# rtqichen/torchdiffeq

Measured on NVIDIA H100. Metric: trajectories/sec (dopri5, batch=65536 dim=128), higher is better.
Workload: dtype f32

## Files before the change

include/tdq.h:

```cpp
#ifndef TDQ_H_
#define TDQ_H_

#include <stddef.h>
#include <stdint.h>

#ifdef __cplusplus
extern "C" {
#endif

#define TDQ_ABI_VERSION 2

#define TDQ_MAX_STAGES 16
#define TDQ_MAX_K      (TDQ_MAX_STAGES + 1)
#define TDQ_MAX_SEGS   64
#define TDQ_MAX_RANKS  16

typedef enum {
    TDQ_OK = 0,
    TDQ_ERR_INVALID = 1,
    TDQ_ERR_CUDA = 2,
    TDQ_ERR_UNSUPPORTED = 3
} tdq_status;

typedef enum { TDQ_F32 = 0, TDQ_F64 = 1 } tdq_dtype;

typedef enum {
    TDQ_RUN_OK = 0,
    TDQ_RUN_DT_UNDERFLOW = 1,
    TDQ_RUN_NONFINITE = 2,
    TDQ_RUN_MAX_STEPS = 3,
    TDQ_RUN_EXCHANGE_TIMEOUT = 4
} tdq_run_status;

typedef struct {
    int32_t n_stages;
    int32_t order;
    int32_t fsal;
    int32_t reserved;
    double alpha[TDQ_MAX_STAGES];
    double beta[TDQ_MAX_STAGES][TDQ_MAX_K];
    double c_sol[TDQ_MAX_K];
    double c_err[TDQ_MAX_K];
    double c_mid[TDQ_MAX_K];
} tdq_tableau;

typedef struct {
    int32_t dtype;
    int32_t ratio_f64;
    double rtol, atol;
    double min_step, max_step;
    double safety, ifactor, dfactor;
    double t_sign;
    int64_t max_num_steps;
    int64_t n_global;
    void *ybuf[2];
    void *kbuf[2];
    int32_t always_fit;
    int32_t reserved;
    uint64_t loop_handle;
} tdq_options;

typedef struct {
    volatile uint64_t seq;
    volatile int32_t status;
    volatile int32_t accept;
    volatile int32_t done;
    volatile int32_t out_cursor;
    volatile int64_t n_accept, n_reject;
    volatile double t0, t1, dt;
    volatile double ratio;
    volatile double att_t0, att_dt;
    volatile double next_t0, next_dt;
    volatile int32_t on_jump_t;
    volatile int32_t par;
} tdq_mailbox;

int tdq_abi_version(void);
size_t tdq_sizeof(int32_t which);
const char *tdq_last_error(void);
int tdq_device_sm_count(int *out);

int tdq_tableau_get(const char *name, tdq_tableau *out);

int tdq_mailbox_create(tdq_mailbox **host_ptr, void **dev_ptr);
int tdq_mailbox_destroy(tdq_mailbox *host_ptr);

size_t tdq_ctrl_size(void);
size_t tdq_ctrl_tstage_offset(void);
size_t tdq_ctrl_taux_offset(void);

int tdq_ctrl_init(void *ctrl_dev, const tdq_tableau *tab, const tdq_options *opt, const double *t_out_dev,
                  double t_start, int32_t n_out, void *mailbox_dev, void *stream);

int tdq_ctrl_set_step_t(void *ctrl_dev, const double *step_t_dev, int32_t n, void *stream);
int tdq_ctrl_set_jump_t(void *ctrl_dev, const double *jump_t_dev, int32_t n, void *stream);

int64_t tdq_norm_table_fill(const int64_t *seg_offsets, const int64_t *seg_lens, int32_t n_seg, int64_t n,
                            int32_t dtype, int64_t *table_host, int64_t capacity_words);
size_t tdq_norm_partials_len(size_t n, int64_t n_chunks);

int tdq_scaled_sumsq(void *ctrl_dev, int32_t dtype, const void *x, const void *x2, const void *y0,
                     const double *rtol_vec, const double *atol_vec, const int64_t *table_dev, int64_t n_chunks,
                     int32_t table_aligned, int32_t n_seg, size_t n, double *partials, double *out, void *stream);
int tdq_initial_step_h0(void *ctrl_dev, int32_t dtype, const double *d0_sumsq, const double *d1_sumsq,
                        const int64_t *seg_counts_dev, int32_t n_seg, void *stream);
int tdq_initial_step_probe(void *ctrl_dev, int32_t dtype, void *y_probe, const void *y0, const void *f0,
                           size_t n, void *stream);
int tdq_initial_step_finish(void *ctrl_dev, int32_t dtype, const double *d2_sumsq,
                            const int64_t *seg_counts_dev, int32_t n_seg, void *stream);
int tdq_set_first_step(void *ctrl_dev, double first_step, void *stream);

int tdq_prepare_attempt(void *ctrl_dev, int32_t dtype, const double *y0_nonfinite_count_dev, void *stream);

int tdq_stage_combine(void *ctrl_dev, const tdq_tableau *tab, int32_t dtype, int32_t row, void *y_out,
                      const void *y0, const void *const *k, size_t n, void *stream);

int tdq_stage_combine_final(void *ctrl_dev, const tdq_tableau *tab, int32_t dtype, void *y1_out, void *err_out,
                            const void *y0, const void *const *k, size_t n, void *stream);

int tdq_error_norm_commit(void *ctrl_dev, int32_t dtype, const void *err_pre, const void *k_last, const void *y0,
                          const void *y1, const double *rtol_vec, const double *atol_vec, const int64_t *table_dev,
                          int64_t n_chunks, int32_t table_aligned, int32_t n_seg, size_t n, double *partials,
                          double *out, void *err_over_tol_out, void *stream);
int tdq_commit_candidates(void *ctrl_dev, int32_t dtype, const void *y1, const void *k_last, size_t n, void *stream);

int tdq_controller(void *ctrl_dev, int32_t dtype, const double *norm_in, const int64_t *seg_counts_dev,
                   int32_t n_seg, const void *ratio_dev, void *stream);

int tdq_interp_fit_eval(void *ctrl_dev, const tdq_tableau *tab, int32_t dtype, const void *y1, const void *const *k,
                        void *const *coeff, void *solution, size_t n, void *stream);
int tdq_interp_eval_at(void *ctrl_dev, int32_t dtype, const void *const *coeff, const double *t_dev, void *out,
                       size_t n, void *stream);
int tdq_poly_eval(int32_t dtype, const void *const *coeff, double x, void *out, size_t n, void *stream);
int tdq_ctrl_reset_interval(void *ctrl_dev, void *stream);

int tdq_loop_create(void *body_graph, void **loop_out, uint64_t *handle_out);
int tdq_loop_launch(void *loop, void *stream);
int tdq_loop_destroy(void *loop);
int tdq_ctrl_set_loop(void *ctrl_dev, uint64_t loop_handle, void *stream);

int tdq_rk4_stage(int32_t dtype, int32_t which, void *y_out, const void *y0, const void *k1,
                  const void *k2, const void *k3, const void *k4, const void *dt_dev,
                  const int64_t *step_dev, size_t n, void *stream);
int tdq_fixed_emit(int32_t dtype, void *y0, const void *y1, void *solution,
                   const int32_t *rec_begin_dev, const int32_t *out_idx_dev, const int32_t *mode_dev,
                   const void *slope_dev, int64_t *step_dev, const void *tstage_all_dev,
                   void *tstage_cur_dev, int64_t n_steps, size_t n, void *stream);

int tdq_fixed_final_emit(int32_t dtype, int32_t which, void *y0, const void *k1, const void *k2, const void *k3,
                         const void *k4, const void *dt_dev, void *solution, const int32_t *rec_begin_dev,
                         const int32_t *out_idx_dev, const int32_t *mode_dev, const void *slope_dev, int64_t *step_dev,
                         const void *tstage_all_dev, void *tstage_cur_dev, int64_t n_steps, size_t n, void *stream);

int tdq_lincomb(int32_t dtype, void *out, const void *base, const void *const *x, const double *coefs, int32_t n_terms,
                size_t n, void *stream);

int tdq_linear_supported(int32_t dtype, int32_t width);
size_t tdq_linear_weights_bytes(int32_t width);
int tdq_linear_prepare(int32_t dtype, const void *weight, int32_t width, void *planes, void *stream);
int tdq_linear_apply(int32_t dtype, const void *y, const void *planes, int32_t width, size_t n_rows, void *k_out,
                     void *stream);
int tdq_linear_stage(void *ctrl_dev, const tdq_tableau *tab, int32_t dtype, int32_t row, void *k_out, void *y1_out,
                     void *err_out, const void *y0, const void *const *k, const void *planes, int32_t width, size_t n,
                     void *stream);

int tdq_linear_attempt_supported(const tdq_tableau *tab, int32_t dtype, int32_t width);
int tdq_linear_attempt(void *ctrl_dev, const tdq_tableau *tab, int32_t dtype, void *const *k_out, void *y1_out, void *err_out,
                       const void *y0, const void *k0, const void *planes, int32_t width, size_t n, double *partials,
                       double *norm_out, const int64_t *seg_counts_dev, int32_t store_always, void *stream);

int tdq_fixed_emit_cubic(int32_t dtype, const void *y0, const void *y1, const void *f0, const void *f1, void *solution,
                         const int32_t *out_idx_dev, const void *coef_dev, int32_t rec_lo, int32_t rec_hi, size_t n,
                         void *stream);

#define TDQ_IMPL_MAX_STAGES 4
#define TDQ_IMPL_MAX_CHUNKS 64
typedef enum {
    TDQ_IMPL_CONTINUE = 0, TDQ_IMPL_CONVERGED = 1, TDQ_IMPL_SINGULAR = 2, TDQ_IMPL_EXHAUSTED = 3
} tdq_impl_status;
size_t tdq_implicit_partials_len(int32_t max_vectors);
size_t tdq_implicit_state_len(int32_t max_iters);
int tdq_implicit_residual(int32_t dtype, const void *x, const void *const *f, int32_t n_stages, size_t n,
                          const void *const *u_chunks, const void *const *s_chunks, int32_t n_chunks, int64_t per_chunk,
                          int32_t slot, int32_t n_dots, double *partials, double *out, void *stream);
int tdq_implicit_solve(int32_t dtype, const double *res_out, const double *upd_out, double *state, int32_t *status,
                       int32_t m, int32_t max_iters, double tol, void *stream);
int tdq_implicit_update(int32_t dtype, void *x, int32_t n_stages, size_t n, const void *const *u_chunks,
                        const void *const *s_chunks, int32_t n_chunks, int64_t per_chunk, int32_t m, const double *w_dev,
                        const void *f0, void *y_out, const void *y0, const void *const *k, const double *coefs,
                        int32_t n_terms, double *partials, double *out, void *stream);

typedef struct { unsigned char bytes[64]; } tdq_ipc_handle;
int tdq_xchg_create(void **dev_ptr, tdq_ipc_handle *handle_out);
int tdq_xchg_open(const tdq_ipc_handle *handle, void **peer_ptr);
int tdq_xchg_close(void *peer_ptr);
int tdq_xchg_destroy(void *dev_ptr);
int tdq_ctrl_set_exchange(void *ctrl_dev, const void *const *peer_ptrs, int32_t rank, int32_t world,
                          uint64_t epoch, void *stream);

typedef enum {
    TDQ_ROWS_T0 = 0, TDQ_ROWS_T1, TDQ_ROWS_DT, TDQ_ROWS_RATIO,
    TDQ_ROWS_ATT_T0, TDQ_ROWS_ATT_DT, TDQ_ROWS_ATT_T1, TDQ_ROWS_FIT_DT,
    TDQ_ROWS_H0, TDQ_ROWS_D1,
    TDQ_ROWS_PAR, TDQ_ROWS_ACCEPT, TDQ_ROWS_FIT, TDQ_ROWS_DONE,
    TDQ_ROWS_STATUS, TDQ_ROWS_CURSOR, TDQ_ROWS_EMIT_LO, TDQ_ROWS_EMIT_HI,
    TDQ_ROWS_N_STEPS, TDQ_ROWS_N_ACCEPT, TDQ_ROWS_N_REJECT,
    TDQ_ROWS_T_FIRST, TDQ_ROWS_T_PROBE, TDQ_ROWS_T_STAGE,
    TDQ_ROWS_N_FIELDS = TDQ_ROWS_T_STAGE + TDQ_MAX_STAGES,
    TDQ_ROWS_HEADER = 255
} tdq_rows_field;
size_t tdq_rows_size(size_t n_rows);
size_t tdq_rows_offset(int32_t field, size_t n_rows);
size_t tdq_rows_partials_len(size_t n_rows, size_t row_len);
int tdq_rows_init(void *ctrl_dev, void *rows_dev, int32_t dtype, size_t n_rows, double t_start, void *stream);
int tdq_rows_init_grid(void *ctrl_dev, void *rows_dev, int32_t dtype, size_t n_rows, const double *t_grid, int32_t n_out,
                       void *stream);
int tdq_rows_sumsq(void *ctrl_dev, void *rows_dev, int32_t dtype, const void *x, const void *x2, const double *rtol_vec,
                   const double *atol_vec, size_t n_rows, size_t row_len, double *partials, double *out, void *stream);
int tdq_rows_initial_h0(void *ctrl_dev, void *rows_dev, int32_t dtype, const double *d0_sumsq, const double *d1_sumsq,
                        size_t n_rows, size_t row_len, void *stream);
int tdq_rows_initial_probe(void *ctrl_dev, void *rows_dev, int32_t dtype, void *y_probe, size_t n_rows, size_t row_len,
                           void *stream);
int tdq_rows_initial_finish(void *ctrl_dev, void *rows_dev, int32_t dtype, const double *d2_sumsq, size_t n_rows,
                            size_t row_len, void *stream);
int tdq_rows_set_first_step(void *rows_dev, size_t n_rows, double first_step, void *stream);
int tdq_rows_prepare(void *ctrl_dev, void *rows_dev, int32_t dtype, const double *y0_nonfinite_dev, size_t n_rows,
                     void *stream);
int tdq_rows_combine(void *ctrl_dev, void *rows_dev, const tdq_tableau *tab, int32_t dtype, int32_t row, void *y_out,
                     const void *const *k, size_t n_rows, size_t row_len, void *stream);
int tdq_rows_combine_final(void *ctrl_dev, void *rows_dev, const tdq_tableau *tab, int32_t dtype, void *y1_out,
                           void *err_out, const void *const *k, size_t n_rows, size_t row_len, void *stream);
int tdq_rows_error_norm_commit(void *ctrl_dev, void *rows_dev, int32_t dtype, const void *err_pre, const void *k_last,
                               const void *y1, const double *rtol_vec, const double *atol_vec, size_t n_rows,
                               size_t row_len, double *partials, double *out, void *stream);
int tdq_rows_controller(void *ctrl_dev, void *rows_dev, int32_t dtype, const double *norm_in, size_t n_rows,
                        size_t row_len, void *stream);
int tdq_rows_fit_eval(void *ctrl_dev, void *rows_dev, const tdq_tableau *tab, int32_t dtype, const void *y1,
                      const void *const *k, void *solution, size_t n_rows, size_t row_len, void *stream);
int tdq_rows_controller_grid(void *ctrl_dev, void *rows_dev, int32_t dtype, const double *norm_in, size_t n_rows,
                             size_t row_len, void *stream);
int tdq_rows_fit_eval_grid(void *ctrl_dev, void *rows_dev, const tdq_tableau *tab, int32_t dtype, const void *y1,
                           const void *const *k, void *solution, size_t n_rows, size_t row_len, void *stream);

int tdq_rows_event_init(void *rows_dev, const double *ev_val, double *init_sign, double *sign0, int32_t *flag,
                        size_t n_rows, int32_t K, void *stream);
int tdq_rows_controller_event(void *ctrl_dev, void *rows_dev, int32_t dtype, const double *norm_in, const double *ev_val,
                              const double *init_sign, const double *sign0, int32_t *flag, size_t n_rows, size_t row_len,
                              int32_t K, void *stream);
int tdq_rows_controller_event_grid(void *ctrl_dev, void *rows_dev, int32_t dtype, const double *norm_in,
                                   const double *ev_val, const double *init_sign, const double *sign0, int32_t *flag,
                                   size_t n_rows, size_t row_len, int32_t K, void *stream);
int tdq_rows_fit_store(void *ctrl_dev, void *rows_dev, const tdq_tableau *tab, int32_t dtype, const void *y1,
                       const void *const *k, const int32_t *flag, void *coeff, size_t n_rows, size_t row_len,
                       void *stream);
int tdq_rows_event_bisect(void *ctrl_dev, void *rows_dev, int32_t dtype, int32_t iter, const double *ev_val,
                          const double *init_sign, const double *sign0, const int32_t *nitrs, double *lo, double *hi,
                          const void *coeff, const void *y_start, void *y_mid, double *t_ev, double *event_t,
                          void *y_event, size_t n_rows, size_t row_len, int32_t K, void *stream);

int tdq_pack_segments(int32_t dtype, void *dst, const void *const *src, const int64_t *offsets,
                      const int64_t *lens, const double *scales, int32_t n_src, void *stream);

#ifdef __cplusplus
}
#endif
#endif
```

torchdiffeq_b200/_engine.py:

```python
import ctypes as C
import math
import time

import torch

from . import _lib

_DTYPES = {torch.float32: _lib.TDQ_F32, torch.float64: _lib.TDQ_F64}


def _stream():
    return torch.cuda.current_stream().cuda_stream


_SOLVER_STREAMS = {}


def solver_stream(device):
    idx = device.index if device.index is not None else torch.cuda.current_device()
    st = _SOLVER_STREAMS.get(idx)
    if st is None:
        st = _SOLVER_STREAMS[idx] = torch.cuda.Stream(device=idx)
    return st


class on_solver_stream:

    def __init__(self, device):
        self.device = device

    def __enter__(self):
        self.cur = torch.cuda.current_stream(self.device)
        self.s = solver_stream(self.device)
        if self.cur == self.s:
            self.ctx = None
            return self
        self.s.wait_stream(self.cur)
        self.ctx = torch.cuda.stream(self.s)
        self.ctx.__enter__()
        return self

    def __exit__(self, *exc):
        if self.ctx is not None:
            self.ctx.__exit__(*exc)
            self.cur.wait_stream(self.s)
        return False

    def publish(self, *tensors):
        if self.ctx is not None:
            for t in tensors:
                if isinstance(t, torch.Tensor) and t.is_cuda:
                    t.record_stream(self.cur)


class _RetryWithCopies(Exception):
    """func handed back a buffer it had already returned for an earlier stage of the same attempt."""


class SolverFailure(AssertionError):
    """Raised for the reference's in-loop assertions (rk_common.py:247, :286, :287)."""


class Layout:

    def __init__(self, shapes, dtype):
        self.shapes = [torch.Size(s) for s in shapes]
        self.dtype = dtype
        vec = 16 // torch.empty((), dtype=dtype).element_size()
        self.offsets, self.lens = [], []
        off = 0
        for s in self.shapes:
            n = s.numel()
            self.offsets.append(off)
            self.lens.append(n)
            off += (n + vec - 1) // vec * vec
        self.n = off
        self.n_real = sum(self.lens)

    def flatten(self, tensors, out=None):
        flat = out if out is not None else torch.zeros(self.n, dtype=self.dtype, device=tensors[0].device)
        for t, o, l in zip(tensors, self.offsets, self.lens):
            flat[o:o + l].copy_(t.reshape(-1))
        return flat

    def views(self, flat, lead=()):
        return tuple(flat[..., o:o + l].view((*lead, *s)) for o, l, s in zip(self.offsets, self.lens, self.shapes))


def pack_pieces(lib, dt_code, dtype, buf, f, pieces):
    offs, lens, scales = pieces
    srcs, keep = [], []
    for p_, l in zip(f, lens):
        if p_ is None:
            srcs.append(None)
            continue
        if p_.dtype != dtype:
            p_ = p_.to(dtype)
        p_ = p_.reshape(-1)
        if not p_.is_contiguous():
            p_ = p_.contiguous()
        if p_.numel() != l:
            raise ValueError("func returned a piece of %d elements, expected %d" % (p_.numel(), l))
        keep.append(p_)
        srcs.append(p_.data_ptr())
    n_launch = 0
    for lo in range(0, len(srcs), _lib.TDQ_MAX_SEGS):
        hi = min(lo + _lib.TDQ_MAX_SEGS, len(srcs))
        _lib.check(lib.tdq_pack_segments(
            dt_code, buf.data_ptr(), _lib.ptr_array(srcs[lo:hi]), _lib.i64_array(offs[lo:hi]),
            _lib.i64_array(lens[lo:hi]), _lib.dbl_array(scales[lo:hi]), hi - lo, _stream()))
        n_launch += 1
    return n_launch


def find_event(interp_fn, sign0, t0, t1, event_fn, tol):
    nitrs = torch.ceil(torch.log((t1 - t0) / tol) / math.log(2.0))
    for _ in range(int(nitrs.long())):
        t_mid = (t1 + t0) / 2.0
        if bool(sign0 == torch.sign(event_fn(t_mid, interp_fn(t_mid)))):
            t0 = t_mid
        else:
            t1 = t_mid
    event_t = (t0 + t1) / 2.0
    return event_t, interp_fn(event_t)


class AdaptiveEngine:

    def __init__(self, fn, n, dtype, device, method, *, rtol, atol, segs=None, t_sign=1.0,
                 pieces=None, min_step=0.0, max_step=float("inf"), first_step=None, step_t=None, jump_t=None,
                 safety=0.9, ifactor=10.0, dfactor=0.2, max_num_steps=2 ** 31 - 1,
                 rtol_vec=None, atol_vec=None, norm_fn=None, q_view=None,
                 graph="auto", run_ahead=2, reduce_fn=None, n_global=None, seg_counts_global=None,
                 agree_fn=None, exchange=None, callbacks=None, keep_interp=False, device_loop="auto", post_fn=None):
        if device.type != "cuda":
            raise _lib.TdqError("torchdiffeq_b200 runs on CUDA devices only (got %s); there is no CPU path" % device)
        if dtype not in _DTYPES:
            raise _lib.TdqError("unsupported state dtype %s (float32 and float64 are implemented)" % dtype)
        self.lib = _lib.load()
        self.fn = fn
        self.n = int(n)
        self.dtype = dtype
        self.device = device
        self.dt_code = _DTYPES[dtype]
        self.tab = _lib.tableau(method)
        self.S = self.tab.n_stages
        self.fsal = bool(self.tab.fsal)
        self.pieces = pieces
        self.first_step = first_step
        self.norm_fn = norm_fn
        self.q_view = q_view
        self.reduce_fn = reduce_fn
        self.agree_fn = agree_fn
        self.exchange = exchange
        self.post_fn = post_fn
        if exchange is not None and post_fn is None:
            self.agree_fn = None
        self.callbacks = callbacks or {}
        self.graph_opt = graph
        self.run_ahead = int(run_ahead)
        self.device_loop = device_loop
        self.keep_interp = bool(keep_interp)
        self.jump_t = jump_t
        if self.callbacks or (jump_t is not None and jump_t.numel() > 0):
            self.graph_opt = False
            self.run_ahead = 0

        segs = segs if segs is not None else [(0, self.n)]
        self.n_seg = len(segs)
        n_real = sum(int(l) for _, l in segs)
        counts = seg_counts_global if seg_counts_global is not None else [int(l) for _, l in segs]
        self.seg_counts = torch.tensor(counts, dtype=torch.int64, device=device)
        if len(segs) == 1 and int(segs[0][0]) == 0 and int(segs[0][1]) == self.n:
            self.norm_table, self.n_chunks, self.table_aligned = None, 0, 0
        else:
            words = _lib.norm_table(segs, self.n, _DTYPES[dtype])
            self.norm_table = torch.tensor(words, dtype=torch.int64, device=device)
            self.n_chunks, self.table_aligned = int(words[1]), int(words[3])

        if (rtol_vec is None) != (atol_vec is None):
            if rtol_vec is None:
                rtol_vec = torch.full_like(atol_vec, rtol)
            else:
                atol_vec = torch.full_like(rtol_vec, atol)
        self.rtol_vec = rtol_vec
        self.atol_vec = atol_vec
        vtol = rtol_vec is not None
        self.ratio_f64 = vtol or dtype == torch.float64
        self.opt = _lib.Options(
            dtype=self.dt_code, ratio_f64=1 if vtol else 0,
            rtol=float(rtol) if not vtol else 0.0, atol=float(atol) if not vtol else 0.0,
            min_step=float(min_step), max_step=float(max_step), safety=float(safety),
            ifactor=float(ifactor), dfactor=float(dfactor), t_sign=float(t_sign),
            max_num_steps=int(max_num_steps), n_global=int(n_global if n_global is not None else n_real))
        self.step_t = step_t

        kw = dict(dtype=dtype, device=device)
        self.ctrl = torch.zeros(self.lib.tdq_ctrl_size(), dtype=torch.uint8, device=device)
        o = self.lib.tdq_ctrl_tstage_offset()
        self.tstage = self.ctrl[o:o + 8 * _lib.TDQ_MAX_K].view(dtype)
        o = self.lib.tdq_ctrl_taux_offset()
        self.taux = self.ctrl[o:o + 32].view(dtype)
        self.ybuf = [torch.zeros(self.n, **kw) for _ in range(2)]
        self.kbuf = [torch.zeros(self.n, **kw) for _ in range(2)]
        self.opt.ybuf[0], self.opt.ybuf[1] = self.ybuf[0].data_ptr(), self.ybuf[1].data_ptr()
        self.opt.kbuf[0], self.opt.kbuf[1] = self.kbuf[0].data_ptr(), self.kbuf[1].data_ptr()
        self.opt.always_fit = 1 if self.keep_interp else 0
        self.ytmp = torch.zeros(self.n, **kw)
        self.y1 = torch.zeros(self.n, **kw)
        self.errp = torch.zeros(self.n, **kw)
        if self.keep_interp:
            self.coeff = [torch.zeros(self.n, **kw) for _ in range(5)]
            self.coeff_ptrs = _lib.ptr_array([c.data_ptr() for c in self.coeff])
        else:
            self.coeff, self.coeff_ptrs = [], None
        self.partials = torch.zeros(self.lib.tdq_norm_partials_len(self.n, self.n_chunks), dtype=torch.float64,
                                    device=device)
        self.norm_out = torch.zeros(self.n_seg + 1, dtype=torch.float64, device=device)
        self.dsum = [torch.zeros(self.n_seg + 1, dtype=torch.float64, device=device) for _ in range(3)]
        self.kslots = {}
        self.qbuf = None
        self.ratio_buf = None
        if norm_fn is not None:
            self.qbuf = torch.zeros(self.n, dtype=torch.float64 if vtol else dtype, device=device)
            self.ratio_buf = torch.zeros((), dtype=torch.float64 if self.ratio_f64 else dtype, device=device)
        self._own_ptrs = None
        self.mbox_host = C.POINTER(_lib.Mailbox)()
        mdev = C.c_void_p()
        _lib.check(self.lib.tdq_mailbox_create(C.byref(self.mbox_host), C.byref(mdev)))
        self.mbox_dev = mdev.value
        self.solution = None
        self._graph = None
        self._graph_failed = False
        self._graph_keep = None
        self._loop = None
        self._loop_handle = 0
        self._loop_failed = False
        self._always_copy = False
        self.linear = None
        self.capture_in_solve = True
        self.n_attempts = 0
        self.nfe = 0
        self.nfe_total = 0
        self.launches = 0
        self._graph_launches = 0

    def __del__(self):
        try:
            if self.mbox_host:
                torch.cuda.synchronize(self.device)
                self._drop_graph()
                self.lib.tdq_mailbox_destroy(self.mbox_host)
                self.mbox_host = None
        except Exception:
            pass

    def _call_fn(self, t, y, slot, taken=(), dst=None):
        self.nfe += 1
        f = self.fn(t, y)
        if isinstance(f, torch.Tensor):
            if f.dtype != self.dtype:
                f = f.to(self.dtype)
            f = f.reshape(-1)
            if f.numel() != self.n:
                raise ValueError("func returned %d elements for a state of %d" % (f.numel(), self.n))
            if f.data_ptr() in taken and not self._always_copy:
                self._always_copy = True
                raise _RetryWithCopies()
            if (self._always_copy or not f.is_contiguous() or (f.data_ptr() % 16) != 0 or self._aliases(f)
                    or f.data_ptr() in taken):
                buf = self._slot(slot)
                buf.copy_(f)
                f = buf
            return f
        buf = dst if dst is not None else self._slot(slot)
        self.launches += pack_pieces(self.lib, self.dt_code, self.dtype, buf, f, self.pieces)
        if self.post_fn is not None:
            self.post_fn(buf)
        return buf

    def set_linear(self, weight, whole_attempt=True):
        width, S = int(weight.shape[0]), self.S
        if self.pieces is not None or self.post_fn is not None or self.n % width:
            return False
        beta, c_err = self.tab.beta, self.tab.c_err
        for i in range(S):
            used = {j for j in range(i + 1) if beta[i][j] != 0.0}
            if self.fsal and i == S - 1:
                used |= {j for j in range(S) if c_err[j] != 0.0}
            if not 1 <= len(used) <= 8:
                return False
        planes = torch.empty(int(self.lib.tdq_linear_weights_bytes(width)), dtype=torch.uint8, device=self.device)
        whole = bool(whole_attempt) and bool(self.lib.tdq_linear_attempt_supported(C.byref(self.tab), self.dt_code, width))
        fold = (whole and self.norm_table is None and self.n_seg == 1 and self.rtol_vec is None and self.norm_fn is None)
        self.linear = dict(weight=weight, width=width, planes=planes, whole=whole, fold=fold,
                           k=[torch.zeros(self.n, dtype=self.dtype, device=self.device) for _ in range(S)])
        self._drop_graph()
        return True

    def _eval(self, t, y, slot, dst=None):
        if self.linear is None:
            return self._call_fn(t, y, slot, dst=dst)
        self.nfe += 1
        out = dst if dst is not None else self._slot(slot)
        L = self.linear
        self._launch(self.lib.tdq_linear_apply(self.dt_code, y.data_ptr(), L["planes"].data_ptr(), L["width"],
                                               self.n // L["width"], out.data_ptr(), _stream()))
        return out

    @property
    def y0w(self):
        return self.ybuf[self.mbox_host.contents.par & 1]

    @property
    def k0(self):
        return self.kbuf[self.mbox_host.contents.par & 1]

    def _drop_graph(self):
        if self._loop is not None:
            try:
                self.lib.tdq_loop_destroy(self._loop)
            except Exception:
                pass
        self._loop, self._loop_handle = None, 0
        self._graph, self._graph_keep = None, None

    def _launch(self, rc):
        _lib.check(rc)
        self.launches += 1

    def _slot(self, i):
        if i not in self.kslots:
            self.kslots[i] = torch.zeros(self.n, dtype=self.dtype, device=self.device)
        return self.kslots[i]

    def _aliases(self, f):
        if self._own_ptrs is None:
            own = self.ybuf + self.kbuf + [self.ytmp, self.y1, self.errp, self.solution] + self.coeff
            self._own_ptrs = {t.untyped_storage().data_ptr() for t in own}
        return f.untyped_storage().data_ptr() in self._own_ptrs

    def _reduce(self, buf):
        if self.reduce_fn is not None:
            self.reduce_fn(buf)

    def _sumsq(self, x, x2, out):
        self._launch(self.lib.tdq_scaled_sumsq(
            self.ctrl.data_ptr(), self.dt_code, x.data_ptr(), x2.data_ptr() if x2 is not None else None,
            None,
            self.rtol_vec.data_ptr() if self.rtol_vec is not None else None,
            self.atol_vec.data_ptr() if self.atol_vec is not None else None,
            self.norm_table.data_ptr() if self.norm_table is not None else None, self.n_chunks, self.table_aligned,
            self.n_seg, self.n, self.partials.data_ptr(), out.data_ptr(), _stream()))
        self._reduce(out)

    def _attempt_front(self):
        try:
            return self._attempt_front_once()
        except _RetryWithCopies:
            return self._attempt_front_once()

    def _attempt_front_once(self):
        lib, ctrl, tab, dc, st = self.lib, self.ctrl.data_ptr(), C.byref(self.tab), self.dt_code, _stream()
        S = self.S
        k = [None] * (S + 1)
        keep = []
        folded = False
        if self.linear is not None and self.linear["whole"]:
            L = self.linear
            for i in range(S):
                k[i + 1] = L["k"][i].data_ptr()
            folded = L["fold"]
            self._launch(lib.tdq_linear_attempt(ctrl, tab, dc, _lib.ptr_array(k), self.y1.data_ptr(), self.errp.data_ptr(),
                                                None, None, L["planes"].data_ptr(), L["width"], self.n,
                                                self.partials.data_ptr() if folded else None,
                                                self.norm_out.data_ptr() if folded else None,
                                                None, 0 if folded else 1, st))
            self.nfe += S
        elif self.linear is not None:
            L = self.linear
            for i in range(S):
                last = i == S - 1 and self.fsal
                out = L["k"][i]
                self._launch(lib.tdq_linear_stage(ctrl, tab, dc, i, out.data_ptr(),
                                                  self.y1.data_ptr() if last else None,
                                                  self.errp.data_ptr() if last else None, None, _lib.ptr_array(k),
                                                  L["planes"].data_ptr(), L["width"], self.n, st))
                self.nfe += 1
                k[i + 1] = out.data_ptr()
        for i in range(S if self.linear is None else 0):
            if i == S - 1 and self.fsal:
                out = self.y1
                self._launch(lib.tdq_stage_combine_final(ctrl, tab, dc, out.data_ptr(), self.errp.data_ptr(), None,
                                                         _lib.ptr_array(k), self.n, st))
            else:
                out = self.ytmp
                self._launch(lib.tdq_stage_combine(ctrl, tab, dc, i, out.data_ptr(), None, _lib.ptr_array(k), self.n,
                                                   st))
            f = self._call_fn(self.tstage[i], out, i + 1, taken=k)
            keep.append(f)
            k[i + 1] = f.data_ptr()
        if not self.fsal:
            self._launch(lib.tdq_stage_combine_final(ctrl, tab, dc, self.y1.data_ptr(), self.errp.data_ptr(), None,
                                                     _lib.ptr_array(k), self.n, st))
        kp = _lib.ptr_array(k)
        if not folded:
            self._launch(lib.tdq_error_norm_commit(
                ctrl, dc, self.errp.data_ptr(), k[S], None, self.y1.data_ptr(),
                self.rtol_vec.data_ptr() if self.rtol_vec is not None else None,
                self.atol_vec.data_ptr() if self.atol_vec is not None else None,
                self.norm_table.data_ptr() if self.norm_table is not None else None, self.n_chunks, self.table_aligned,
                self.n_seg, self.n, self.partials.data_ptr(), self.norm_out.data_ptr(),
                self.qbuf.data_ptr() if self.qbuf is not None else None, st))
        ratio_ptr = None
        if self.norm_fn is not None:
            r = self.norm_fn(self.q_view(self.qbuf))
            r = torch.as_tensor(r, device=self.device)
            self.ratio_buf.copy_(r.to(self.ratio_buf.dtype).reshape(()))
            ratio_ptr = self.ratio_buf.data_ptr()
        elif self.exchange is None:
            self._reduce(self.norm_out)
        self._launch(lib.tdq_controller(ctrl, dc, self.norm_out.data_ptr(), self.seg_counts.data_ptr(), self.n_seg,
                                      ratio_ptr, st))
        return k, kp, keep

    def _attempt_back(self, kp):
        self._launch(self.lib.tdq_interp_fit_eval(self.ctrl.data_ptr(), C.byref(self.tab), self.dt_code,
                                                  self.y1.data_ptr(), kp, self.coeff_ptrs, self.solution.data_ptr(),
                                                  self.n, _stream()))

    def _attempt(self):
        k, kp, keep = self._attempt_front()
        self._attempt_back(kp)
        return keep

    def _wait_seq(self, target):
        mb = self.mbox_host.contents
        spins = 0
        while mb.seq < target:
            spins += 1
            if spins > 2000:
                time.sleep(0)
                if spins % 20000 == 0 and torch.cuda.current_stream().query() and mb.seq < target:
                    raise _lib.TdqError("the device finished the queued attempts without reporting attempt %d (mailbox at %d)"
                                        % (target, mb.seq))
        return mb

    def _raise_if_failed(self, mb):
        if mb.status != _lib.RUN_OK:
            torch.cuda.current_stream().synchronize()
            self._raise_status(mb.status, mb.next_dt, self.y0w)

    def _raise_status(self, s, dt, y, where=""):
        if s == _lib.RUN_DT_UNDERFLOW:
            raise SolverFailure("underflow in dt {}".format(dt) + where)
        if s == _lib.RUN_NONFINITE:
            raise SolverFailure("non-finite values in state `y`: {}".format(y) + where)
        if s == _lib.RUN_EXCHANGE_TIMEOUT:
            raise _lib.TdqError("a peer rank did not deliver its norm partials within 10 s (sharded solve)")
        if s == _lib.RUN_MAX_STEPS:
            m = self.opt.max_num_steps
            raise SolverFailure("max_num_steps exceeded ({}>={})".format(m, m) + where)
        raise SolverFailure("solver failed with status %d" % s + where)

    def _lockstep_mode(self):
        return bool(self.callbacks) or self.run_ahead == 0

    def _use_loop(self):
        return (self._loop is not None and not self._lockstep_mode() and self.agree_fn is None
                and self.norm_fn is None)

    def solve(self, y0_flat, t64, t_start=None):
        try:
            if self._lockstep_mode():
                for _ in self._lockstep(y0_flat, t64, t_start):
                    pass
            else:
                if self._begin(y0_flat, t64, t_start, loop=self._use_loop()) > 1:
                    self._loop_run_ahead()
                self._read_counters()
        except BaseException:
            self.poisoned = True
            try:
                torch.cuda.current_stream().synchronize()
            except Exception:
                pass
            raise
        return self.solution

    def _read_counters(self):
        mb = self.mbox_host.contents
        self.n_accept, self.n_reject = int(mb.n_accept), int(mb.n_reject)
        self.n_attempts = self.n_accept + self.n_reject

    def prime(self, y0_flat, t64, t_start=None):
        if self.graph_opt not in (True, "auto") or self._lockstep_mode():
            return False
        n_out = self._begin(y0_flat, t64, t_start)
        if n_out <= 1:
            return False
        self._warm_attempt()
        self._capture()
        torch.cuda.current_stream().synchronize()
        return self._graph is not None

    def _begin(self, y0_flat, t64, t_start=None, loop=False):
        lib = self.lib
        self.nfe_total += self.nfe
        self.nfe, self.launches = 0, 0
        n_out = int(t64.numel())
        self.t_out = t64.contiguous()
        if getattr(self, "solution", None) is None or self.solution.shape[0] != n_out:
            self.solution = torch.empty(n_out, self.n, dtype=self.dtype, device=self.device)
            self._drop_graph()
            self._own_ptrs = None
            loop = False
        self.solution[0].copy_(y0_flat)
        self.ybuf[0].copy_(y0_flat)
        st = _stream()
        mb = self.mbox_host.contents
        mb.seq, mb.status, mb.done, mb.par, mb.accept = 0, 0, 0, 0, 0
        mb.n_accept, mb.n_reject = 0, 0
        if t_start is None:
            t_start = float(t64[0])
        self.opt.loop_handle = self._loop_handle if loop else 0
        _lib.check(lib.tdq_ctrl_init(self.ctrl.data_ptr(), C.byref(self.tab), C.byref(self.opt),
                                     self.t_out.data_ptr(), float(t_start), n_out, self.mbox_dev, st))
        self._start(float(t_start), n_out)
        return n_out

    def _start(self, t_start, n_out):
        lib = self.lib
        st = _stream()
        if self.exchange is not None:
            self.exchange.arm(self.ctrl.data_ptr(), st)
        if self.jump_t is not None and self.jump_t.numel() > 0:
            self._launch(lib.tdq_ctrl_set_jump_t(self.ctrl.data_ptr(), self.jump_t.data_ptr(),
                                                 int(self.jump_t.numel()), st))
        if self.step_t is not None and self.step_t.numel() > 0:
            self._launch(lib.tdq_ctrl_set_step_t(self.ctrl.data_ptr(), self.step_t.data_ptr(),
                                               int(self.step_t.numel()), st))
        dc, ctrl = self.dt_code, self.ctrl.data_ptr()
        if self.linear is not None:
            L = self.linear
            self._launch(lib.tdq_linear_prepare(dc, L["weight"].data_ptr(), L["width"], L["planes"].data_ptr(), st))

        f0 = self._eval(self.taux[0], self.ybuf[0], 0, dst=self.kbuf[0])
        if f0.data_ptr() != self.kbuf[0].data_ptr():
            self.kbuf[0].copy_(f0)
        del f0
        self._sumsq(self.ybuf[0], None, self.dsum[0])
        if self.first_step is None:
            if self.norm_fn is not None:
                self._initial_step_custom_norm()
            else:
                self._sumsq(self.kbuf[0], None, self.dsum[1])
                self._launch(lib.tdq_initial_step_h0(ctrl, dc, self.dsum[0].data_ptr(), self.dsum[1].data_ptr(),
                                                   self.seg_counts.data_ptr(), self.n_seg, st))
                self._launch(lib.tdq_initial_step_probe(ctrl, dc, self.ytmp.data_ptr(), None, None, self.n, st))
                f1 = self._eval(self.taux[1], self.ytmp, 1)
                self._sumsq(f1, self.kbuf[0], self.dsum[2])
                del f1
                self._launch(lib.tdq_initial_step_finish(ctrl, dc, self.dsum[2].data_ptr(),
                                                       self.seg_counts.data_ptr(), self.n_seg, st))
        else:
            self._launch(lib.tdq_set_first_step(ctrl, float(self.first_step), st))
        bad_ptr = self.dsum[0].data_ptr() + 8 * self.n_seg if n_out > 1 else None
        self._launch(lib.tdq_prepare_attempt(ctrl, dc, bad_ptr, st))

    def _lockstep_attempt(self, issued, mb):
        cb = self.callbacks
        if cb.get("callback_step") is not None:
            cb["callback_step"](*self._with_y(mb.next_t0, mb.next_dt))
        k, kp, keep = self._attempt_front()
        issued += 1
        mb = self._wait_seq(issued)
        self._raise_if_failed(mb)
        if cb:
            name = "callback_accept_step" if mb.accept else "callback_reject_step"
            if cb.get(name) is not None:
                cb[name](*self._with_y(mb.att_t0, mb.att_dt))
        jumped = bool(mb.accept) and bool(mb.on_jump_t)
        self._attempt_back(kp)
        del k, kp, keep
        if jumped:
            k0 = self.k0
            f = self._call_fn(self.taux[2], self.y0w, 0, dst=k0)
            if f.data_ptr() != k0.data_ptr():
                k0.copy_(f)
            del f
        return issued, mb

    def _lockstep(self, y0_flat, t64, t_start=None):
        n_out = self._begin(y0_flat, t64, t_start)
        torch.cuda.current_stream().synchronize()
        mb = self.mbox_host.contents
        self._raise_if_failed(mb)
        issued = 0
        yield mb
        try:
            while n_out > 1:
                issued, mb = self._lockstep_attempt(issued, mb)
                yield mb
                if mb.done:
                    break
        except GeneratorExit:
            pass
        torch.cuda.current_stream().synchronize()
        self._read_counters()

    def solve_dense(self, y0_flat, t64):
        steps = self._lockstep(y0_flat, t64)
        next(steps)
        times, coeffs = [float(t64[0])], []
        for mb in steps:
            if mb.accept:
                times.append(float(mb.t1))
                coeffs.append([c.clone() for c in self.coeff])
        return self.solution, times, coeffs

    def solve_taped(self, y0_flat, t64, t_start=None):
        steps = self._lockstep(y0_flat, t64, t_start)
        next(steps)
        tape, cursor, first, jumped = [], 1, True, None
        for mb in steps:
            if mb.accept:
                prev = (mb.par ^ 1) & 1
                k0 = self.kbuf[prev]
                tape.append(dict(t0=float(mb.att_t0), dt=float(mb.att_dt), y0=self.ybuf[prev].clone(), k0=k0.clone(),
                                 out_lo=cursor, out_hi=int(mb.out_cursor), first=first, jumped_into=jumped))
                cursor, first = int(mb.out_cursor), False
                jumped = True if mb.on_jump_t else None
        return self.solution, tape

    def solve_until_event(self, y0_flat, t0, event_fn, tol):
        t64 = torch.tensor([float(t0), float("inf")], dtype=torch.float64, device=self.device)
        steps = self._lockstep(y0_flat, t64, float(t0))
        mb = next(steps)
        tt = lambda v: torch.tensor(v, dtype=torch.float64, device=self.device)
        t_cur = float(t0)
        if bool(event_fn(tt(t_cur), self.y0w) == 0):
            return t_cur, self.y0w.clone()
        sign0 = torch.sign(event_fn(tt(t_cur), self.y0w))
        while bool(sign0 == torch.sign(event_fn(tt(t_cur), self.y0w))):
            mb = next(steps)
            t_cur = mb.t1
        steps.close()
        y_mid = torch.empty(self.n, dtype=self.dtype, device=self.device)

        def interp(t_eval):
            self._launch(self.lib.tdq_interp_eval_at(self.ctrl.data_ptr(), self.dt_code, self.coeff_ptrs,
                                                     t_eval.to(self.device).data_ptr(), y_mid.data_ptr(), self.n,
                                                     _stream()))
            return y_mid
        bound = lambda v: torch.tensor(float(v), dtype=torch.float64)
        event_t, y_event = find_event(interp, sign0, bound(mb.t0), bound(mb.t1),
                                      lambda t_, y_: event_fn(t_.to(self.device), y_), tol)
        return float(event_t), y_event.clone()

    def _with_y(self, t0, dt):
        t0, dt = self._scalars(t0, dt)
        return t0, self.y0w, dt

    def _scalars(self, t0, dt):
        kw = dict(dtype=torch.float64, device=self.device)
        return torch.tensor(t0, **kw), torch.tensor(dt, **kw)

    def _loop_run_ahead(self):
        D = max(1, self.run_ahead)
        mb = self.mbox_host.contents
        issued = 0
        use_graph = self.graph_opt in (True, "auto") and not self._graph_failed and self.capture_in_solve
        if self._use_loop() and self.opt.loop_handle != 0:
            self._launch_loop()
            return
        if self._graph is None:
            if use_graph:
                self._warm_attempt()
                self._capture()
            else:
                self._attempt()
            issued += 1
            if self._use_loop():
                _lib.check(self.lib.tdq_ctrl_set_loop(self.ctrl.data_ptr(), self._loop_handle, _stream()))
                self._launch_loop(first=1)
                return
        while True:
            seen = mb.seq
            if mb.status != _lib.RUN_OK or mb.done:
                break
            if issued - seen > D:
                time.sleep(0)
                continue
            if self._graph is not None:
                self._graph.replay()
                self.nfe += self.S
                self.launches += self._graph_launches
            else:
                self._attempt()
            issued += 1
        if self.agree_fn is not None:
            target = self.agree_fn(issued)
            while issued < target:
                if self._graph is not None:
                    self._graph.replay()
                    self.nfe += self.S
                    self.launches += self._graph_launches
                else:
                    self._attempt()
                issued += 1
        mb = self._wait_seq(issued)
        self._raise_if_failed(mb)
        torch.cuda.current_stream().synchronize()

    def _launch_loop(self, first=0):
        _lib.check(self.lib.tdq_loop_launch(self._loop, _stream()))
        torch.cuda.current_stream().synchronize()
        mb = self.mbox_host.contents
        ran = int(mb.seq) - first
        self.nfe += self.S * ran
        self.launches += self._graph_launches * ran
        self._raise_if_failed(mb)

    def _warm_attempt(self):
        self._attempt()

    def _capture(self):
        last = None
        for _try in range(2):
            try:
                want_loop = (self.device_loop in (True, "auto") and not self._loop_failed and self.agree_fn is None
                             and self.norm_fn is None)
                g = torch.cuda.CUDAGraph(keep_graph=True) if want_loop else torch.cuda.CUDAGraph()
                nfe, launches = self.nfe, self.launches
                try:
                    with torch.cuda.graph(g, stream=solver_stream(self.device)):
                        keep = self._attempt()
                finally:
                    self._graph_launches = self.launches - launches
                    self.nfe, self.launches = nfe, launches
                self._graph, self._graph_keep = g, keep
                if want_loop:
                    self._make_loop(g)
                return
            except Exception as e:
                last = e
                self._graph = None
                torch.cuda.synchronize(self.device)
        self._graph_failed = True
        if self.graph_opt is True:
            raise last
        import warnings
        warnings.warn("torchdiffeq_b200: CUDA graph capture of the step body failed (%s: %s); "
                      "continuing with eager launches" % (type(last).__name__, last))

    def _make_loop(self, g):
        loop, handle = C.c_void_p(), C.c_uint64()
        try:
            _lib.check(self.lib.tdq_loop_create(C.c_void_p(g.raw_cuda_graph()), C.byref(loop), C.byref(handle)))
            self._loop, self._loop_handle = loop.value, int(handle.value)
        except Exception as e:
            self._loop, self._loop_handle, self._loop_failed = None, 0, True
            if self.device_loop is True:
                raise
            import warnings
            warnings.warn("torchdiffeq_b200: the captured step could not be wrapped into a device-side loop "
                          "(%s: %s); the host replays it instead" % (type(e).__name__, e))

    def _initial_step_custom_norm(self):
        T = self.dtype
        y0, f0 = self.ybuf[0], self.kbuf[0] * self.opt.t_sign
        if self.rtol_vec is not None:
            scale = self.atol_vec + torch.abs(y0) * self.rtol_vec
        else:
            scale = float(self.opt.atol) + torch.abs(y0) * float(self.opt.rtol)
        nf = lambda v: torch.as_tensor(self.norm_fn(self.q_view(v)), device=self.device).abs()
        d0, d1 = nf(y0 / scale), nf(f0 / scale)
        if d0 < 1e-5 or d1 < 1e-5:
            h0 = torch.tensor(1e-6, dtype=T, device=self.device)
        else:
            h0 = 0.01 * d0 / d1
        h0 = h0.abs()
        self.ytmp.copy_(y0 + h0 * f0)
        t0 = float(self.t_out[0])
        self.taux[1] = (torch.tensor(t0, dtype=torch.float64, device=self.device) + h0.double()).to(T) * self.opt.t_sign
        f1 = self._call_fn(self.taux[1], self.ytmp, 1) * self.opt.t_sign
        d2 = torch.abs(nf((f1 - f0) / scale) / h0)
        order = self.tab.order - 1
        if d1 <= 1e-15 and d2 <= 1e-15:
            h1 = torch.max(torch.tensor(1e-6, dtype=T, device=self.device), h0 * 1e-3)
        else:
            h1 = (0.01 / max(d1, d2)) ** (1. / float(order + 1))
        h1 = h1.abs()
        dt = float(torch.min(100 * h0, h1).to(torch.float64))
        self._launch(self.lib.tdq_set_first_step(self.ctrl.data_ptr(), dt, _stream()))


def bisect_iterations(lo, hi, tol):
    v = torch.log((hi - lo) / tol) / math.log(2.0)
    for r in ((v - v.round()).abs() < 1e-6).nonzero().view(-1).tolist():
        v[r] = torch.log((hi[r] - lo[r]) / tol[r]) / math.log(2.0)
    n = torch.ceil(v)
    return torch.where(torch.isfinite(n) & (n > 0), n, torch.zeros_like(n)).to(torch.int32)


class RowsEngine(AdaptiveEngine):

    def __init__(self, fn, shape, dtype, device, method, **kw):
        shape = torch.Size(shape)
        self.B = int(shape[0])
        self.D = int(shape[1:].numel())
        self.row_shape = shape[1:]
        super().__init__(fn, self.B * self.D, dtype, device, method, **kw)
        lib, B = self.lib, self.B
        self.rows = torch.zeros(lib.tdq_rows_size(B), dtype=torch.uint8, device=device)
        es = torch.empty((), dtype=dtype).element_size()
        tshape = (B,) + (1,) * (len(shape) - 1)

        def field(which, dt, size):
            o = lib.tdq_rows_offset(which, B)
            return self.rows[o:o + B * size].view(dt)
        self._field = field
        self.t_first = field(_lib.ROWS_T_FIRST, dtype, es).view(tshape)
        self.t_probe = field(_lib.ROWS_T_PROBE, dtype, es).view(tshape)
        self.t_stage = [field(_lib.ROWS_T_STAGE + i, dtype, es).view(tshape) for i in range(self.S)]
        f64 = dict(dtype=torch.float64, device=device)
        self.row_partials = torch.zeros(lib.tdq_rows_partials_len(B, self.D), **f64)
        self.row_norm = torch.zeros(2 * B, **f64)
        self.row_dsum = [torch.zeros(2 * B, **f64) for _ in range(3)]
        self.row_n_accept = self.row_n_reject = None
        self.ev_fn = None
        self.grid = None
        self._next_grid = None
        self._graph_grid = False

    def solve(self, y0_flat, t64, t_start=None, grid=None):
        if grid is not None:
            if grid.dim() != 2 or grid.shape[0] != self.B or grid.dtype != torch.float64 or grid.device != self.device:
                raise ValueError("grid must be a float64 [%d, T] tensor on %s, got %s %s on %s"
                                 % (self.B, self.device, grid.dtype, tuple(grid.shape), grid.device))
            grid = grid.contiguous()
            t64 = grid[0]
        self._next_grid = grid
        try:
            return super().solve(y0_flat, t64, t_start)
        finally:
            self._next_grid = None

    def _begin(self, y0_flat, t64, t_start=None, loop=False):
        self.grid = self._next_grid
        if (self.grid is not None) != self._graph_grid:
            self._drop_graph()
            self._graph_grid = self.grid is not None
            loop = False
        return super()._begin(y0_flat, t64, t_start, loop)

    def _rows_sumsq(self, x, x2, out):
        self._launch(self.lib.tdq_rows_sumsq(
            self.ctrl.data_ptr(), self.rows.data_ptr(), self.dt_code, x.data_ptr(),
            x2.data_ptr() if x2 is not None else None,
            self.rtol_vec.data_ptr() if self.rtol_vec is not None else None,
            self.atol_vec.data_ptr() if self.atol_vec is not None else None,
            self.B, self.D, self.row_partials.data_ptr(), out.data_ptr(), _stream()))

    def _attempt_front_once(self):
        lib, ctrl, rows, tab, dc, st = (self.lib, self.ctrl.data_ptr(), self.rows.data_ptr(), C.byref(self.tab),
                                        self.dt_code, _stream())
        S, B, D = self.S, self.B, self.D
        k = [None] * (S + 1)
        keep = []
        for i in range(S):
            if i == S - 1 and self.fsal:
                out = self.y1
                self._launch(lib.tdq_rows_combine_final(ctrl, rows, tab, dc, out.data_ptr(), self.errp.data_ptr(),
                                                        _lib.ptr_array(k), B, D, st))
            else:
                out = self.ytmp
                self._launch(lib.tdq_rows_combine(ctrl, rows, tab, dc, i, out.data_ptr(), _lib.ptr_array(k), B, D, st))
            f = self._call_fn(self.t_stage[i], out, i + 1, taken=k)
            keep.append(f)
            k[i + 1] = f.data_ptr()
        if not self.fsal:
            self._launch(lib.tdq_rows_combine_final(ctrl, rows, tab, dc, self.y1.data_ptr(), self.errp.data_ptr(),
                                                    _lib.ptr_array(k), B, D, st))
        kp = _lib.ptr_array(k)
        self._launch(lib.tdq_rows_error_norm_commit(
            ctrl, rows, dc, self.errp.data_ptr(), k[S], self.y1.data_ptr(),
            self.rtol_vec.data_ptr() if self.rtol_vec is not None else None,
            self.atol_vec.data_ptr() if self.atol_vec is not None else None,
            B, D, self.row_partials.data_ptr(), self.row_norm.data_ptr(), st))
        grid = self.grid is not None
        if self.ev_fn is None:
            controller = lib.tdq_rows_controller_grid if grid else lib.tdq_rows_controller
            self._launch(controller(ctrl, rows, dc, self.row_norm.data_ptr(), B, D, st))
        else:
            torch.mul(self.row_field(_lib.ROWS_ATT_T1, torch.float64), self.opt.t_sign, out=self.ev_t)
            self._ev_call(self.y1)
            controller = lib.tdq_rows_controller_event_grid if grid else lib.tdq_rows_controller_event
            self._launch(controller(ctrl, rows, dc, self.row_norm.data_ptr(), self.ev_val.data_ptr(),
                                    self.ev_init.data_ptr(), self.ev_sign0.data_ptr(), self.ev_flag.data_ptr(), B, D,
                                    self.K, st))
        return k, kp, keep

    def _attempt_back(self, kp):
        if self.ev_fn is not None:
            self._launch(self.lib.tdq_rows_fit_store(self.ctrl.data_ptr(), self.rows.data_ptr(), C.byref(self.tab),
                                                     self.dt_code, self.y1.data_ptr(), kp, self.ev_flag.data_ptr(),
                                                     self.ev_coeff.data_ptr(), self.B, self.D, _stream()))
            return
        fit_eval = self.lib.tdq_rows_fit_eval_grid if self.grid is not None else self.lib.tdq_rows_fit_eval
        self._launch(fit_eval(self.ctrl.data_ptr(), self.rows.data_ptr(), C.byref(self.tab), self.dt_code,
                              self.y1.data_ptr(), kp, self.solution.data_ptr(), self.B, self.D, _stream()))

    def _ev_call(self, y_flat):
        self.n_ev += 1
        v = self.ev_fn(self.ev_t_view, y_flat.view(self.B, *self.row_shape))
        if not isinstance(v, torch.Tensor) or v.dim() == 0 or v.shape[0] != self.B or v.numel() != self.B * self.K:
            raise ValueError("event_fn returned %s; with independent rows it must keep the shape of its first result, "
                             "[B, K...] with B = %d and K = %d" % (tuple(getattr(v, "shape", ())), self.B, self.K))
        self.ev_val.copy_(v.reshape(self.B, self.K))

    def solve_until_event(self, y0_flat, t_start, ev, ev0, tol, t_starts=None):
        B, dev = self.B, self.device
        K = int(ev0.numel()) // B
        f64 = dict(dtype=torch.float64, device=dev)
        self.ev_fn, self.K = ev, K
        self.ev_val = torch.zeros(B, K, **f64)
        self.ev_init = torch.zeros(B, K, **f64)
        self.ev_sign0 = torch.zeros(B, **f64)
        self.ev_flag = torch.zeros(B, dtype=torch.int32, device=dev)
        self.ev_lo = torch.zeros(2 * B, **f64)
        self.ev_hi = torch.zeros(2 * B, **f64)
        self.ev_nitrs = torch.zeros(B, dtype=torch.int32, device=dev)
        self.ev_coeff = torch.zeros(5, self.n, dtype=self.dtype, device=dev)
        sign = self.opt.t_sign
        self.ev_t = torch.full((B,), t_start * sign, **f64) if t_starts is None else t_starts * sign
        self.ev_t_view = self.ev_t.view(B, *([1] * len(self.row_shape)))
        self.ev_event_t = torch.zeros(B, **f64)
        self.ev_val.copy_(ev0.reshape(B, K))
        self.n_ev = 1
        t64 = torch.tensor([t_start, float("inf")], **f64)
        grid = None if t_starts is None else torch.stack([t_starts, torch.full_like(t_starts, float("inf"))], dim=1)
        self.solve(y0_flat, t64, t_start, grid=grid)
        o0, o1 = self.lib.tdq_rows_offset(_lib.ROWS_T0, B), self.lib.tdq_rows_offset(_lib.ROWS_T1, B)
        tt = self.rows[o0:o1 + 8 * B].view(torch.float64).cpu()
        nitrs = bisect_iterations(tt[:B], tt[(o1 - o0) // 8:], tol)
        self.ev_nitrs.copy_(nitrs)
        self.bisect_iters = int(nitrs.max())
        lib, ctrl, rows, dc, st = self.lib, self.ctrl.data_ptr(), self.rows.data_ptr(), self.dt_code, _stream()
        for it in range(self.bisect_iters + 1):
            self._launch(lib.tdq_rows_event_bisect(
                ctrl, rows, dc, it, self.ev_val.data_ptr(), self.ev_init.data_ptr(), self.ev_sign0.data_ptr(),
                self.ev_nitrs.data_ptr(), self.ev_lo.data_ptr(), self.ev_hi.data_ptr(), self.ev_coeff.data_ptr(),
                self.solution[0].data_ptr(), self.ytmp.data_ptr(), self.ev_t.data_ptr(), self.ev_event_t.data_ptr(),
                self.solution[1].data_ptr(), B, self.D, K, st))
            if it < self.bisect_iters:
                self._ev_call(self.ytmp)
        return self.ev_event_t, self.solution

    def _start(self, t_start, n_out):
        lib, st = self.lib, _stream()
        ctrl, rows, dc, B, D = self.ctrl.data_ptr(), self.rows.data_ptr(), self.dt_code, self.B, self.D
        if self.grid is not None:
            self._launch(lib.tdq_rows_init_grid(ctrl, rows, dc, B, self.grid.data_ptr(), n_out, st))
        else:
            self._launch(lib.tdq_rows_init(ctrl, rows, dc, B, t_start, st))
        f0 = self._call_fn(self.t_first, self.ybuf[0], 0, dst=self.kbuf[0])
        if f0.data_ptr() != self.kbuf[0].data_ptr():
            self.kbuf[0].copy_(f0)
        del f0
        d = self.row_dsum
        self._rows_sumsq(self.ybuf[0], None, d[0])
        if self.first_step is None:
            self._rows_sumsq(self.kbuf[0], None, d[1])
            self._launch(lib.tdq_rows_initial_h0(ctrl, rows, dc, d[0].data_ptr(), d[1].data_ptr(), B, D, st))
            self._launch(lib.tdq_rows_initial_probe(ctrl, rows, dc, self.ytmp.data_ptr(), B, D, st))
            f1 = self._call_fn(self.t_probe, self.ytmp, 1)
            self._rows_sumsq(f1, self.kbuf[0], d[2])
            del f1
            self._launch(lib.tdq_rows_initial_finish(ctrl, rows, dc, d[2].data_ptr(), B, D, st))
        else:
            self._launch(lib.tdq_rows_set_first_step(rows, B, float(self.first_step), st))
        if self.ev_fn is not None:
            self._launch(lib.tdq_rows_event_init(rows, self.ev_val.data_ptr(), self.ev_init.data_ptr(),
                                                 self.ev_sign0.data_ptr(), self.ev_flag.data_ptr(), B, self.K, st))
        self._launch(lib.tdq_rows_prepare(ctrl, rows, dc, d[0].data_ptr() if n_out > 1 else None, B, st))

    def row_field(self, which, dtype):
        return self._field(which, dtype, torch.empty((), dtype=dtype).element_size())

    def _raise_if_failed(self, mb):
        if mb.status == _lib.RUN_OK:
            return
        torch.cuda.current_stream().synchronize()
        r = int(self.rows[:16].view(torch.int32)[3])
        par = int(self.row_field(_lib.ROWS_PAR, torch.int32)[r])
        y = self.ybuf[par][r * self.D:(r + 1) * self.D].view(1, *self.row_shape)
        self._raise_status(mb.status, float(self.row_field(_lib.ROWS_ATT_DT, torch.float64)[r]), y, " (row %d)" % r)

    def _read_counters(self):
        self.row_n_accept = self.row_field(_lib.ROWS_N_ACCEPT, torch.int64).cpu()
        self.row_n_reject = self.row_field(_lib.ROWS_N_REJECT, torch.int64).cpu()
        self.n_accept, self.n_reject = int(self.row_n_accept.sum()), int(self.row_n_reject.sum())
        self.n_attempts = int((self.row_n_accept + self.row_n_reject).max())
```

torchdiffeq_b200/_lib.py:

```python
import ctypes as C
import os

_HERE = os.path.dirname(os.path.abspath(__file__))
LIB_PATH = os.path.join(_HERE, "csrc", "libtdq.so")

TDQ_MAX_STAGES = 16
TDQ_MAX_K = TDQ_MAX_STAGES + 1
TDQ_MAX_SEGS = 64
TDQ_F32, TDQ_F64 = 0, 1
RUN_OK, RUN_DT_UNDERFLOW, RUN_NONFINITE, RUN_MAX_STEPS, RUN_EXCHANGE_TIMEOUT = 0, 1, 2, 3, 4
TDQ_MAX_RANKS = 16
(ROWS_T0, ROWS_T1, ROWS_DT, ROWS_RATIO, ROWS_ATT_T0, ROWS_ATT_DT, ROWS_ATT_T1, ROWS_FIT_DT, ROWS_H0, ROWS_D1, ROWS_PAR,
 ROWS_ACCEPT, ROWS_FIT, ROWS_DONE, ROWS_STATUS, ROWS_CURSOR, ROWS_EMIT_LO, ROWS_EMIT_HI, ROWS_N_STEPS, ROWS_N_ACCEPT,
 ROWS_N_REJECT, ROWS_T_FIRST, ROWS_T_PROBE, ROWS_T_STAGE) = range(24)
ROWS_HEADER = 255
ABI_VERSION = 2


class IpcHandle(C.Structure):
    _fields_ = [("bytes", C.c_ubyte * 64)]


class Tableau(C.Structure):
    _fields_ = [
        ("n_stages", C.c_int32), ("order", C.c_int32), ("fsal", C.c_int32), ("reserved", C.c_int32),
        ("alpha", C.c_double * TDQ_MAX_STAGES),
        ("beta", (C.c_double * TDQ_MAX_K) * TDQ_MAX_STAGES),
        ("c_sol", C.c_double * TDQ_MAX_K),
        ("c_err", C.c_double * TDQ_MAX_K),
        ("c_mid", C.c_double * TDQ_MAX_K),
    ]


class Options(C.Structure):
    _fields_ = [
        ("dtype", C.c_int32), ("ratio_f64", C.c_int32),
        ("rtol", C.c_double), ("atol", C.c_double),
        ("min_step", C.c_double), ("max_step", C.c_double),
        ("safety", C.c_double), ("ifactor", C.c_double), ("dfactor", C.c_double),
        ("t_sign", C.c_double),
        ("max_num_steps", C.c_int64), ("n_global", C.c_int64),
        ("ybuf", C.c_void_p * 2), ("kbuf", C.c_void_p * 2),
        ("always_fit", C.c_int32), ("reserved", C.c_int32),
        ("loop_handle", C.c_uint64),
    ]


class Mailbox(C.Structure):
    _fields_ = [
        ("seq", C.c_uint64),
        ("status", C.c_int32), ("accept", C.c_int32), ("done", C.c_int32), ("out_cursor", C.c_int32),
        ("n_accept", C.c_int64), ("n_reject", C.c_int64),
        ("t0", C.c_double), ("t1", C.c_double), ("dt", C.c_double),
        ("ratio", C.c_double), ("att_t0", C.c_double), ("att_dt", C.c_double),
        ("next_t0", C.c_double), ("next_dt", C.c_double),
        ("on_jump_t", C.c_int32), ("par", C.c_int32),
    ]


class TdqError(RuntimeError):
    pass


_vp, _i32, _i64, _sz, _dbl = C.c_void_p, C.c_int32, C.c_int64, C.c_size_t, C.c_double
_pp = C.POINTER(C.c_void_p)
_pi64 = C.POINTER(C.c_int64)
_pdbl = C.POINTER(C.c_double)
_ptab = C.POINTER(Tableau)

_SIGNATURES = {
    "tdq_abi_version": (C.c_int, []),
    "tdq_sizeof": (_sz, [_i32]),
    "tdq_last_error": (C.c_char_p, []),
    "tdq_device_sm_count": (C.c_int, [C.POINTER(C.c_int)]),
    "tdq_tableau_get": (C.c_int, [C.c_char_p, _ptab]),
    "tdq_mailbox_create": (C.c_int, [C.POINTER(C.POINTER(Mailbox)), _pp]),
    "tdq_mailbox_destroy": (C.c_int, [C.POINTER(Mailbox)]),
    "tdq_ctrl_size": (_sz, []),
    "tdq_ctrl_tstage_offset": (_sz, []),
    "tdq_ctrl_taux_offset": (_sz, []),
    "tdq_ctrl_init": (C.c_int, [_vp, _ptab, C.POINTER(Options), _vp, _dbl, _i32, _vp, _vp]),
    "tdq_ctrl_set_step_t": (C.c_int, [_vp, _vp, _i32, _vp]),
    "tdq_ctrl_set_jump_t": (C.c_int, [_vp, _vp, _i32, _vp]),
    "tdq_norm_table_fill": (_i64, [_pi64, _pi64, _i32, _i64, _i32, _pi64, _i64]),
    "tdq_norm_partials_len": (_sz, [_sz, _i64]),
    "tdq_scaled_sumsq": (C.c_int, [_vp, _i32, _vp, _vp, _vp, _vp, _vp, _vp, _i64, _i32, _i32, _sz, _vp, _vp, _vp]),
    "tdq_initial_step_h0": (C.c_int, [_vp, _i32, _vp, _vp, _vp, _i32, _vp]),
    "tdq_initial_step_probe": (C.c_int, [_vp, _i32, _vp, _vp, _vp, _sz, _vp]),
    "tdq_initial_step_finish": (C.c_int, [_vp, _i32, _vp, _vp, _i32, _vp]),
    "tdq_set_first_step": (C.c_int, [_vp, _dbl, _vp]),
    "tdq_prepare_attempt": (C.c_int, [_vp, _i32, _vp, _vp]),
    "tdq_stage_combine": (C.c_int, [_vp, _ptab, _i32, _i32, _vp, _vp, _pp, _sz, _vp]),
    "tdq_stage_combine_final": (C.c_int, [_vp, _ptab, _i32, _vp, _vp, _vp, _pp, _sz, _vp]),
    "tdq_error_norm_commit": (C.c_int, [_vp, _i32, _vp, _vp, _vp, _vp, _vp, _vp, _vp, _i64, _i32, _i32, _sz, _vp, _vp,
                                        _vp, _vp]),
    "tdq_commit_candidates": (C.c_int, [_vp, _i32, _vp, _vp, _sz, _vp]),
    "tdq_controller": (C.c_int, [_vp, _i32, _vp, _vp, _i32, _vp, _vp]),
    "tdq_interp_fit_eval": (C.c_int, [_vp, _ptab, _i32, _vp, _pp, _pp, _vp, _sz, _vp]),
    "tdq_interp_eval_at": (C.c_int, [_vp, _i32, _pp, _vp, _vp, _sz, _vp]),
    "tdq_poly_eval": (C.c_int, [_i32, _pp, _dbl, _vp, _sz, _vp]),
    "tdq_ctrl_reset_interval": (C.c_int, [_vp, _vp]),
    "tdq_loop_create": (C.c_int, [_vp, _pp, C.POINTER(C.c_uint64)]),
    "tdq_loop_launch": (C.c_int, [_vp, _vp]),
    "tdq_loop_destroy": (C.c_int, [_vp]),
    "tdq_ctrl_set_loop": (C.c_int, [_vp, C.c_uint64, _vp]),
    "tdq_rk4_stage": (C.c_int, [_i32, _i32, _vp, _vp, _vp, _vp, _vp, _vp, _vp, _vp, _sz, _vp]),
    "tdq_fixed_emit": (C.c_int, [_i32, _vp, _vp, _vp, _vp, _vp, _vp, _vp, _vp, _vp, _vp, _i64, _sz, _vp]),
    "tdq_fixed_final_emit": (C.c_int, [_i32, _i32, _vp, _vp, _vp, _vp, _vp, _vp, _vp, _vp, _vp, _vp, _vp, _vp, _vp, _vp,
                                       _i64, _sz, _vp]),
    "tdq_lincomb": (C.c_int, [_i32, _vp, _vp, _pp, _pdbl, _i32, _sz, _vp]),
    "tdq_linear_supported": (C.c_int, [_i32, _i32]),
    "tdq_linear_weights_bytes": (_sz, [_i32]),
    "tdq_linear_prepare": (C.c_int, [_i32, _vp, _i32, _vp, _vp]),
    "tdq_linear_apply": (C.c_int, [_i32, _vp, _vp, _i32, _sz, _vp, _vp]),
    "tdq_linear_stage": (C.c_int, [_vp, _ptab, _i32, _i32, _vp, _vp, _vp, _vp, _pp, _vp, _i32, _sz, _vp]),
    "tdq_linear_attempt_supported": (C.c_int, [_ptab, _i32, _i32]),
    "tdq_linear_attempt": (C.c_int, [_vp, _ptab, _i32, _pp, _vp, _vp, _vp, _vp, _vp, _i32, _sz, _vp, _vp, _vp, _i32, _vp]),
    "tdq_fixed_emit_cubic": (C.c_int, [_i32, _vp, _vp, _vp, _vp, _vp, _vp, _vp, _i32, _i32, _sz, _vp]),
    "tdq_pack_segments": (C.c_int, [_i32, _vp, _pp, _pi64, _pi64, _pdbl, _i32, _vp]),
    "tdq_implicit_partials_len": (_sz, [_i32]),
    "tdq_implicit_state_len": (_sz, [_i32]),
    "tdq_implicit_residual": (C.c_int, [_i32, _vp, _pp, _i32, _sz, _pp, _pp, _i32, _i64, _i32, _i32, _vp, _vp, _vp]),
    "tdq_implicit_solve": (C.c_int, [_i32, _vp, _vp, _vp, _vp, _i32, _i32, _dbl, _vp]),
    "tdq_implicit_update": (C.c_int, [_i32, _vp, _i32, _sz, _pp, _pp, _i32, _i64, _i32, _vp, _vp, _vp, _vp, _pp, _pdbl,
                                      _i32, _vp, _vp, _vp]),
    "tdq_rows_size": (_sz, [_sz]),
    "tdq_rows_offset": (_sz, [_i32, _sz]),
    "tdq_rows_partials_len": (_sz, [_sz, _sz]),
    "tdq_rows_init": (C.c_int, [_vp, _vp, _i32, _sz, _dbl, _vp]),
    "tdq_rows_init_grid": (C.c_int, [_vp, _vp, _i32, _sz, _vp, _i32, _vp]),
    "tdq_rows_sumsq": (C.c_int, [_vp, _vp, _i32, _vp, _vp, _vp, _vp, _sz, _sz, _vp, _vp, _vp]),
    "tdq_rows_initial_h0": (C.c_int, [_vp, _vp, _i32, _vp, _vp, _sz, _sz, _vp]),
    "tdq_rows_initial_probe": (C.c_int, [_vp, _vp, _i32, _vp, _sz, _sz, _vp]),
    "tdq_rows_initial_finish": (C.c_int, [_vp, _vp, _i32, _vp, _sz, _sz, _vp]),
    "tdq_rows_set_first_step": (C.c_int, [_vp, _sz, _dbl, _vp]),
    "tdq_rows_prepare": (C.c_int, [_vp, _vp, _i32, _vp, _sz, _vp]),
    "tdq_rows_combine": (C.c_int, [_vp, _vp, _ptab, _i32, _i32, _vp, _pp, _sz, _sz, _vp]),
    "tdq_rows_combine_final": (C.c_int, [_vp, _vp, _ptab, _i32, _vp, _vp, _pp, _sz, _sz, _vp]),
    "tdq_rows_error_norm_commit": (C.c_int, [_vp, _vp, _i32, _vp, _vp, _vp, _vp, _vp, _sz, _sz, _vp, _vp, _vp]),
    "tdq_rows_controller": (C.c_int, [_vp, _vp, _i32, _vp, _sz, _sz, _vp]),
    "tdq_rows_controller_grid": (C.c_int, [_vp, _vp, _i32, _vp, _sz, _sz, _vp]),
    "tdq_rows_fit_eval": (C.c_int, [_vp, _vp, _ptab, _i32, _vp, _pp, _vp, _sz, _sz, _vp]),
    "tdq_rows_fit_eval_grid": (C.c_int, [_vp, _vp, _ptab, _i32, _vp, _pp, _vp, _sz, _sz, _vp]),
    "tdq_rows_event_init": (C.c_int, [_vp, _vp, _vp, _vp, _vp, _sz, _i32, _vp]),
    "tdq_rows_controller_event": (C.c_int, [_vp, _vp, _i32, _vp, _vp, _vp, _vp, _vp, _sz, _sz, _i32, _vp]),
    "tdq_rows_controller_event_grid": (C.c_int, [_vp, _vp, _i32, _vp, _vp, _vp, _vp, _vp, _sz, _sz, _i32, _vp]),
    "tdq_rows_fit_store": (C.c_int, [_vp, _vp, _ptab, _i32, _vp, _pp, _vp, _vp, _sz, _sz, _vp]),
    "tdq_rows_event_bisect": (C.c_int, [_vp, _vp, _i32, _i32, _vp, _vp, _vp, _vp, _vp, _vp, _vp, _vp, _vp, _vp, _vp, _vp,
                                        _sz, _sz, _i32, _vp]),
    "tdq_xchg_create": (C.c_int, [_pp, C.POINTER(IpcHandle)]),
    "tdq_xchg_open": (C.c_int, [C.POINTER(IpcHandle), _pp]),
    "tdq_xchg_close": (C.c_int, [_vp]),
    "tdq_xchg_destroy": (C.c_int, [_vp]),
    "tdq_ctrl_set_exchange": (C.c_int, [_vp, _pp, _i32, _i32, C.c_uint64, _vp]),
}

EXPORTED_SYMBOLS = tuple(_SIGNATURES)

_lib = None


def load():
    global _lib
    if _lib is not None:
        return _lib
    if not os.path.exists(LIB_PATH):
        raise TdqError(
            "libtdq.so is not built (%s). Run `python -m torchdiffeq_b200.csrc.build` "
            "(or __graft_entry__.build()); there is no fallback path." % LIB_PATH)
    lib = C.CDLL(LIB_PATH)
    for name, (res, args) in _SIGNATURES.items():
        try:
            fn = getattr(lib, name)
        except AttributeError as e:
            raise TdqError("libtdq.so does not export %s; rebuild it" % name) from e
        fn.restype = res
        fn.argtypes = args
    if lib.tdq_abi_version() != ABI_VERSION:
        raise TdqError("libtdq.so ABI version mismatch")
    for which, st in ((0, Tableau), (1, Options), (2, Mailbox)):
        if lib.tdq_sizeof(which) != C.sizeof(st):
            raise TdqError("libtdq.so struct layout mismatch for %s; rebuild it" % st.__name__)
    _lib = lib
    return lib


def check(rc):
    if rc != 0:
        msg = load().tdq_last_error()
        raise TdqError("libtdq call failed (%d): %s" % (rc, msg.decode() if msg else "?"))


def tableau(name):
    t = Tableau()
    check(load().tdq_tableau_get(name.encode(), C.byref(t)))
    return t


def tableau_as_dict(name):
    t = tableau(name)
    S = t.n_stages
    return {
        "n_stages": S, "order": t.order, "fsal": bool(t.fsal),
        "alpha": [t.alpha[i] for i in range(S)],
        "beta": [[t.beta[i][j] for j in range(i + 1)] for i in range(S)],
        "c_sol": [t.c_sol[j] for j in range(S + 1)],
        "c_err": [t.c_err[j] for j in range(S + 1)],
        "c_mid": [t.c_mid[j] for j in range(S + 1)],
    }


def norm_table(segs, n, dt_code):
    lib = load()
    offs = i64_array([int(o) for o, _ in segs])
    lens = i64_array([int(l) for _, l in segs])
    words = lib.tdq_norm_table_fill(offs, lens, len(segs), int(n), dt_code, None, 0)
    if words < 0:
        check(1)
    buf = (C.c_int64 * words)()
    if lib.tdq_norm_table_fill(offs, lens, len(segs), int(n), dt_code, buf, words) != words:
        check(1)
    return list(buf)


def ptr_array(ptrs):
    arr = (C.c_void_p * len(ptrs))()
    for i, p in enumerate(ptrs):
        arr[i] = p
    return arr


def i64_array(vals):
    return (C.c_int64 * len(vals))(*vals)


def dbl_array(vals):
    return (C.c_double * len(vals))(*vals)
```

torchdiffeq_b200/csrc/build.py:

```python
import hashlib
import os
import shutil
import subprocess
import sys

HERE = os.path.dirname(os.path.abspath(__file__))
ROOT = os.path.dirname(os.path.dirname(HERE))
INCLUDE = os.path.join(ROOT, "include")
SOURCES = ["tdq_api.cu", "tdq_ctrl.cu", "tdq_stream.cu", "tdq_norm.cu", "tdq_interp.cu", "tdq_fixed.cu", "tdq_graph.cu", "tdq_linear.cu", "tdq_attempt.cu", "tdq_implicit.cu", "tdq_rows.cu"]
HEADERS = [os.path.join(HERE, "tdq_common.cuh"), os.path.join(HERE, "tdq_shape.cuh"), os.path.join(HERE, "tdq_step.cuh"), os.path.join(HERE, "tdq_tc.cuh"), os.path.join(HERE, "tdq_tableau_tsit5.inc"), os.path.join(INCLUDE, "tdq.h")]
LIB = os.path.join(HERE, "libtdq.so")
STAMP = os.path.join(HERE, "libtdq.stamp")

NVCC_FLAGS = [
    "-gencode", "arch=compute_90a,code=sm_90a",
    "-O3", "-lineinfo", "-std=c++17",
    "--fmad=false",
    "-Xcompiler", "-fPIC,-O2,-ffp-contract=off,-fvisibility=default",
    "-I", INCLUDE, "-I", HERE,
]


def _nvcc():
    exe = shutil.which("nvcc") or "/usr/local/cuda/bin/nvcc"
    if not os.path.exists(exe):
        raise RuntimeError("nvcc not found; libtdq cannot be built")
    return exe


def _digest():
    h = hashlib.sha256()
    for p in [os.path.join(HERE, s) for s in SOURCES] + HEADERS + [os.path.abspath(__file__)]:
        with open(p, "rb") as f:
            h.update(f.read())
    return h.hexdigest()


def build(force=False, verbose=False):
    want = _digest()
    if not force and os.path.exists(LIB) and os.path.exists(STAMP):
        with open(STAMP) as f:
            if f.read().strip() == want:
                return LIB
    nvcc = _nvcc()
    objs = []
    procs = []
    for src in SOURCES:
        obj = os.path.join(HERE, src.replace(".cu", ".o"))
        cmd = [nvcc] + NVCC_FLAGS + (["-Xptxas", "-v"] if verbose else []) + ["-c", os.path.join(HERE, src), "-o", obj]
        procs.append((src, subprocess.Popen(cmd, stdout=subprocess.PIPE, stderr=subprocess.STDOUT, text=True)))
        objs.append(obj)
    failed = False
    for src, p in procs:
        out, _ = p.communicate()
        if p.returncode != 0:
            failed = True
            sys.stderr.write("nvcc failed on %s:\n%s\n" % (src, out))
        elif verbose:
            sys.stderr.write(out)
    if failed:
        raise RuntimeError("libtdq build failed")
    cmd = [nvcc, "-shared", "-o", LIB] + objs + ["-gencode", "arch=compute_90a,code=sm_90a", "-lcudart_static",
                                                 "-Xcompiler", "-fPIC"]
    subprocess.run(cmd, check=True)
    with open(STAMP, "w") as f:
        f.write(want)
    return LIB


if __name__ == "__main__":
    print(build(force="--force" in sys.argv, verbose="--verbose" in sys.argv))
```

torchdiffeq_b200/csrc/tdq_attempt.cu:

```cuda
#include "tdq_shape.cuh"
#include "tdq_tc.cuh"

#include <cstddef>
#include <type_traits>

namespace {

using namespace tdq_tc;

constexpr int AT_ROWS = 32;
constexpr int AT_THREADS = 256;
constexpr int AT_STAGE = 3 * y_plane<AT_ROWS>();
constexpr int AT_Y0 = AT_ROWS * LD * 4;
constexpr int AT_AUX = 2048;
constexpr int AT_SMEM = W_BYTES + AT_STAGE + AT_Y0 + AT_AUX + 128;
constexpr int AT_MAX_S = 7;

__device__ __forceinline__ void sts_f32(uint32_t addr, float v) { asm volatile("st.shared.f32 [%0], %1;" :: "r"(addr), "f"(v) : "memory"); }
__device__ __forceinline__ float lds_f32(uint32_t addr) {
    float v;
    asm volatile("ld.shared.f32 %0, [%1];" : "=f"(v) : "r"(addr) : "memory");
    return v;
}

__device__ __forceinline__ uint64_t lds_u64(uint32_t addr) {
    uint64_t v;
    asm volatile("ld.shared.u64 %0, [%1];" : "=l"(v) : "r"(addr) : "memory");
    return v;
}
__device__ __forceinline__ float lds_pinned_f32(uint32_t addr) {
    float v;
    asm volatile("ld.volatile.shared.f32 %0, [%1];" : "=f"(v) : "r"(addr) : "memory");
    return v;
}

struct AttOut {
    float *k[AT_MAX_S + 1];
    float *y1, *err;
};

template <int S, unsigned long long RM, unsigned EM>
__global__ void __launch_bounds__(AT_THREADS, 1)
k_linear_attempt(TdqCtrl *c, const float *y0, const float *k0, AttOut out, const uint32_t *__restrict__ wt,
                 double *partials, double *norm_out, int store_always, size_t n_rows_sz) {
    if (c->halt) return;
    extern __shared__ uint8_t smem_raw[];
    uint8_t *smem = reinterpret_cast<uint8_t *>((reinterpret_cast<uintptr_t>(smem_raw) + 127) & ~(uintptr_t)127);
    uint8_t *aux = smem + W_BYTES + AT_STAGE + AT_Y0;
    int *s_flag = reinterpret_cast<int *>(aux);
    struct Scalars {
        const float *y0, *k0;
        float *ycand, *kcand;
        AttOut out;
        float rtol, atol;
    };
    Scalars *s_sc = reinterpret_cast<Scalars *>(aux + 320);
    static_assert(320 + sizeof(Scalars) <= 512, "aux layout");
    float *s_cr = reinterpret_cast<float *>(aux + 64);
    float *s_ce = s_cr + AT_MAX_S * 8;
    double *s_red = reinterpret_cast<double *>(aux + 512);
    const int tid = threadIdx.x, lane = tid & 31;
    const int warp = __shfl_sync(0xffffffffu, tid >> 5, 0);
    const int n_rows = (int)n_rows_sz;

    if (tid < AT_MAX_S * 8) {
        const int i = tid >> 3, j = tid & 7;
        const unsigned mask = i < S ? (unsigned)((RM >> (8 * i)) & 0xffull) : 0u, below = (1u << j) - 1u;
        s_cr[i * 8 + j] = ((mask >> j) & 1u) ? (float)c->coef[i][__popc(mask & below)] : 0.f;
        if (i == 0) s_ce[j] = j == S ? (float)c->ecoef[__popc(EM)] : ((EM >> j) & 1u) ? (float)c->ecoef[__popc(EM & below)] : 0.f;
    }
    const bool fold = partials != nullptr;
    if (tid == 0) {
        Scalars sc;
        sc.y0 = tdq_detach(y0 != nullptr ? y0 : reinterpret_cast<const float *>(c->y0_cur), n_rows_sz);
        sc.k0 = tdq_detach(k0 != nullptr ? k0 : reinterpret_cast<const float *>(c->k0_cur), n_rows_sz);
        sc.ycand = sc.kcand = nullptr;
        if (fold && c->ybuf[0] != nullptr) {
            sc.ycand = tdq_detach(reinterpret_cast<float *>(c->ybuf[c->par ^ 1]), n_rows_sz);
            sc.kcand = tdq_detach(reinterpret_cast<float *>(c->kbuf[c->par ^ 1]), n_rows_sz);
        }
        sc.out = out;
        sc.rtol = (float)c->rtol;
        sc.atol = (float)c->atol;
        *s_sc = sc;
    }
    load_weights(smem, wt, tid, AT_THREADS);
    fence_async_smem();
    __syncthreads();

    bool store = store_always != 0 || c->always_fit != 0;
    if (!store) {
        const int cur = c->out_cursor;
        store = cur < c->n_out && !(c->t_out[cur] > c->att_t1);
    }
    const int h = warp >> 2, w = warp & 3;
    const uint32_t wsm = smem_u32(smem);
    const uint32_t ssc = wsm + (uint32_t)(reinterpret_cast<uint8_t *>(s_sc) - smem);
    const uint32_t scoef = wsm + (uint32_t)(reinterpret_cast<uint8_t *>(s_cr) - smem);
    auto coef = [scoef](int i, int j) { return lds_pinned_f32(scoef + 4 * (8 * i + j)); };
    const uint32_t wsm_h = wsm + h * 8 * SBO;
    const uint32_t stage = wsm + W_BYTES;
    const uint32_t sy0 = stage + AT_STAGE + tid * 4;
    const uint64_t dw = make_desc(wsm_h), dy = make_desc(stage);
    uint32_t ahi[LD / 16][4];
#pragma unroll
    for (int ks = 0; ks < LD / 16; ++ks) {
#pragma unroll
        for (int r = 0; r < 4; ++r) {
            const int f = 16 * w + (lane >> 2) + 8 * (r & 1), k = 16 * ks + 2 * (lane & 3) + 8 * (r >> 1);
            asm volatile("ld.shared.b32 %0, [%1];" : "=r"(ahi[ks][r])
                         : "r"(wsm_h + (f >> 3) * SBO + (k >> 3) * LBO + (f & 7) * 16 + (k & 7) * 2));
        }
    }
    const int toff = thread_offset(w, lane) + 64 * h;

    const int tiles = (n_rows + AT_ROWS - 1) / AT_ROWS;
    double acc = 0.0;
    int nbad = 0;

    constexpr int KEEP = S < 4 ? S : 4;
    constexpr int NACC = S - KEEP;
    auto row_mask = [](int i) -> unsigned { return (unsigned)((RM >> (8 * i)) & 0xffull); };
    auto do_tile = [&](auto full_tag, const int t) {
        constexpr bool FULL = decltype(full_tag)::value;
        const int row0 = t * AT_ROWS;
        const int rows_here = n_rows - row0;
        const size_t base = (size_t)row0 * LD + toff;
        float K[KEEP][16];
        float A[NACC > 0 ? NACC : 1][16];
        float AE[16], PRE[16], KN[16], Y1[16];
        {
            const float *y0 = reinterpret_cast<const float *>(lds_u64(ssc + offsetof(Scalars, y0)));
            const float *k0 = reinterpret_cast<const float *>(lds_u64(ssc + offsetof(Scalars, k0)));
            float Y0[16];
#pragma unroll
            for (int e = 0; e < 16; ++e) {
                Y0[e] = 0.f;
                KN[e] = 0.f;
                if (FULL || elem_row<AT_ROWS>(e, lane) < rows_here) {
                    Y0[e] = __ldcs(y0 + base + elem_offset<AT_ROWS>(e));
                    KN[e] = __ldcs(k0 + base + elem_offset<AT_ROWS>(e));
                }
            }
#pragma unroll
            for (int e = 0; e < 16; ++e) sts_f32(sy0 + e * 1024, Y0[e]);
        }
#pragma unroll
        for (int i = 0; i < S; ++i) {
            const unsigned mask = row_mask(i);
            const bool last = i == S - 1;
            const bool has_prefix = (mask & ((1u << i) - 1u)) != 0u, has_new = ((mask >> i) & 1u) != 0u;
            const float c_new = has_new ? coef(i, i) : 0.f;
            if (i < KEEP) {
#pragma unroll
                for (int e = 0; e < 16; ++e) K[i < KEEP ? i : 0][e] = KN[e];
            }
            {
                float yv[16];
#pragma unroll
                for (int e = 0; e < 16; ++e) {
                    const float pre = i < KEEP ? PRE[e] : A[i >= KEEP ? i - KEEP : 0][e];
                    float sum;
                    if (has_prefix && has_new) sum = pre + KN[e] * c_new;
                    else if (has_prefix) sum = pre;
                    else sum = KN[e] * c_new;
                    yv[e] = lds_f32(sy0 + e * 1024) + sum;
                    if (last) Y1[e] = yv[e];
                }
                __syncthreads();
                store_planes<AT_ROWS>(stage, yv, h, w, lane);
            }
            fence_async_smem();
            __syncthreads();
            TileAcc<AT_ROWS> tacc;
            tile_product(dw, dy, tacc, ahi);
            if (i + 1 < KEEP && i + 1 < S) {
                const unsigned mn = row_mask(i + 1);
                bool first = true;
#pragma unroll
                for (int j = 0; j <= i; ++j) {
                    if ((mn >> j) & 1u) {
                        const float cj = coef(i + 1, j);
#pragma unroll
                        for (int e = 0; e < 16; ++e) {
                            const float p = K[j < KEEP ? j : 0][e] * cj;
                            PRE[e] = first ? p : PRE[e] + p;
                        }
                        first = false;
                    }
                }
                reg_fence(PRE);
            }
            if (i == KEEP - 1) {
                float cq[NACC > 0 ? NACC : 1][KEEP], ce[KEEP];
#pragma unroll
                for (int j = 0; j < KEEP; ++j) {
#pragma unroll
                    for (int qrow = KEEP; qrow < S; ++qrow)
                        if ((row_mask(qrow) >> j) & 1u) cq[qrow - KEEP][j] = coef(qrow, j);
                    if ((EM >> j) & 1u) ce[j] = coef(AT_MAX_S, j);
                }
#pragma unroll
                for (int e = 0; e < 16; ++e) {
#pragma unroll
                    for (int qrow = KEEP; qrow < S; ++qrow) {
                        const unsigned mq = row_mask(qrow);
                        float a_ = 0.f;
                        bool first = true;
#pragma unroll
                        for (int j = 0; j <= i; ++j) {
                            if ((mq >> j) & 1u) {
                                const float p = K[j < KEEP ? j : 0][e] * cq[qrow - KEEP][j];
                                a_ = first ? p : a_ + p;
                                first = false;
                            }
                        }
                        A[qrow - KEEP][e] = a_;
                    }
                    float e_ = 0.f;
                    bool first = true;
#pragma unroll
                    for (int j = 0; j <= i; ++j) {
                        if ((EM >> j) & 1u) {
                            const float p = K[j < KEEP ? j : 0][e] * ce[j];
                            e_ = first ? p : e_ + p;
                            first = false;
                        }
                    }
                    AE[e] = e_;
                }
#pragma unroll
                for (int qrow = KEEP; qrow < S; ++qrow) reg_fence(A[qrow - KEEP]);
                reg_fence(AE);
            }
            if (i >= KEEP) {
#pragma unroll
                for (int qrow = i + 1; qrow < S; ++qrow) {
                    const unsigned mq = row_mask(qrow);
                    if ((mq >> i) & 1u) {
                        const float cj = coef(qrow, i);
                        const bool started = (mq & ((1u << i) - 1u)) != 0u;
#pragma unroll
                        for (int e = 0; e < 16; ++e) {
                            const float p = KN[e] * cj;
                            A[qrow - KEEP][e] = started ? A[qrow - KEEP][e] + p : p;
                        }
                    }
                }
                if ((EM >> i) & 1u) {
                    const float cj = coef(AT_MAX_S, i);
                    const bool started = (EM & ((1u << i) - 1u)) != 0u;
#pragma unroll
                    for (int e = 0; e < 16; ++e) {
                        const float p = KN[e] * cj;
                        AE[e] = started ? AE[e] + p : p;
                    }
                }
#pragma unroll
                for (int qrow = i + 1; qrow < S; ++qrow) reg_fence(A[qrow - KEEP]);
                reg_fence(AE);
            }
            if (last) {
                float *ycand = reinterpret_cast<float *>(lds_u64(ssc + offsetof(Scalars, ycand)));
                const float rtolT = lds_f32(ssc + offsetof(Scalars, rtol)), atolT = lds_f32(ssc + offsetof(Scalars, atol));
#pragma unroll
                for (int e = 0; e < 16; ++e) {
                    const float y1v = Y1[e];
                    if (FULL || elem_row<AT_ROWS>(e, lane) < rows_here) {
                        if (!isfinite(y1v)) nbad += 1;
                        const size_t o = base + elem_offset<AT_ROWS>(e);
                        if (ycand) ycand[o] = y1v;
                        if (store) {
                            reinterpret_cast<float *>(lds_u64(ssc + offsetof(Scalars, out.y1)))[o] = y1v;
                            reinterpret_cast<float *>(lds_u64(ssc + offsetof(Scalars, out.err)))[o] = AE[e];
                        }
                    }
                    Y1[e] = Ar<float>::add(atolT, Ar<float>::mul(rtolT, Ar<float>::max_nan(fabsf(lds_f32(sy0 + e * 1024)), fabsf(y1v))));
                }
                reg_fence(Y1);
            }
            wgmma_wait();
            tile_result(tacc, KN);
            if (store) {
                float *ko = reinterpret_cast<float *>(lds_u64(ssc + offsetof(Scalars, out.k) + 8 * (i + 1)));
#pragma unroll
                for (int e = 0; e < 16; ++e)
                    if (FULL || elem_row<AT_ROWS>(e, lane) < rows_here) ko[base + elem_offset<AT_ROWS>(e)] = KN[e];
            }
            if (last) {
                float *kcand = reinterpret_cast<float *>(lds_u64(ssc + offsetof(Scalars, kcand)));
                const float ecS = coef(AT_MAX_S, S);
#pragma unroll
                for (int e = 0; e < 16; ++e) {
                    if (FULL || elem_row<AT_ROWS>(e, lane) < rows_here) {
                        if (kcand) kcand[base + elem_offset<AT_ROWS>(e)] = KN[e];
                        if (fold) {
                            const float num = Ar<float>::add(AE[e], Ar<float>::mul(KN[e], ecS));
                            const float q = Ar<float>::div(num, Y1[e]);
                            acc += (double)Ar<float>::mul(q, q);
                        }
                    }
                }
            }
        }
    };
#pragma unroll 1
    for (int t = (int)blockIdx.x; t < tiles; t += (int)gridDim.x) {
        {
            const int tn = t + (int)gridDim.x;
            const long long prow = (long long)tn * AT_ROWS + lane;
            if (tn < tiles && prow < (long long)n_rows) {
                const float *y0 = reinterpret_cast<const float *>(lds_u64(ssc + offsetof(Scalars, y0)));
                const float *k0 = reinterpret_cast<const float *>(lds_u64(ssc + offsetof(Scalars, k0)));
                const size_t o = (size_t)prow * LD + 64 * h + 16 * w;
                asm volatile("prefetch.global.L2 [%0];" :: "l"(y0 + o));
                asm volatile("prefetch.global.L2 [%0];" :: "l"(k0 + o));
            }
        }
        if (n_rows - t * AT_ROWS >= AT_ROWS) do_tile(std::true_type{}, t);
        else do_tile(std::false_type{}, t);
    }
    const double bad = (double)nbad;

    if (!fold) return;
    {
        const double wa = warp_sum(acc), wb = warp_sum(bad);
        if (lane == 0) {
            s_red[warp] = wa;
            s_red[32 + warp] = wb;
        }
    }
    __syncthreads();
    const int P = (int)gridDim.x;
    double *p_sum = partials + 2, *p_bad = p_sum + P;
    unsigned int *ticket = reinterpret_cast<unsigned int *>(partials);
    if (tid == 0) {
        double a = 0.0, b = 0.0;
        for (int w_ = 0; w_ < AT_THREADS / 32; ++w_) {
            a += s_red[w_];
            b += s_red[32 + w_];
        }
        p_sum[blockIdx.x] = a;
        p_bad[blockIdx.x] = b;
        __threadfence();
        const unsigned int tk = atomicAdd(ticket, 1u);
        *s_flag = (tk == gridDim.x - 1) ? 1 : 0;
    }
    __syncthreads();
    if (!*s_flag) return;
    __threadfence();
    if (warp == 0) {
        double a = 0.0, b = 0.0;
        for (int i = lane; i < P; i += 32) {
            a += __ldcg(&p_sum[i]);
            b += __ldcg(&p_bad[i]);
        }
        a = warp_sum(a);
        b = warp_sum(b);
        if (lane == 0) {
            norm_out[0] = a;
            norm_out[1] = b;
            *ticket = 0;
        }
    }
}

constexpr unsigned long long RM_DOPRI5 = 0x01ull | (0x03ull << 8) | (0x07ull << 16) | (0x0full << 24) | (0x1full << 32) | (0x3dull << 40);
constexpr unsigned long long RM_BOSH3 = 0x01ull | (0x02ull << 8) | (0x07ull << 16);

template <int S, unsigned long long RM, unsigned EM>
int launch_attempt(TdqCtrl *c, const float *y0, const float *k0, const AttOut &out, const uint32_t *wt, double *partials,
                   double *norm_out, int store_always, size_t n_rows, cudaStream_t st) {
    auto kern = k_linear_attempt<S, RM, EM>;
    if (cudaFuncSetAttribute(kern, cudaFuncAttributeMaxDynamicSharedMemorySize, AT_SMEM) != cudaSuccess) return -2;
    kern<<<tdq_grid(n_rows, AT_ROWS, 1), AT_THREADS, AT_SMEM, st>>>(c, y0, k0, out, wt, partials, norm_out, store_always, n_rows);
    return 0;
}

bool attempt_masks(const TdqHostShape &hs, unsigned long long *rm, unsigned *em) {
    const int S = hs.n_stages;
    if (!hs.fsal || S < 2 || S > AT_MAX_S) return false;
    *rm = 0;
    *em = 0;
    for (int i = 0; i < S; ++i) {
        unsigned m = 0;
        for (int q = 0; q < hs.row_nnz[i]; ++q) {
            if (hs.row_idx[i][q] > i) return false;
            m |= 1u << hs.row_idx[i][q];
        }
        if (m == 0) return false;
        *rm |= (unsigned long long)m << (8 * i);
    }
    bool has_S = false;
    for (int q = 0; q < hs.err_nnz; ++q) {
        if (hs.err_idx[q] == S) has_S = true;
        else *em |= 1u << hs.err_idx[q];
    }
    return has_S && hs.err_idx[hs.err_nnz - 1] == S;
}

}

extern "C" {

int tdq_linear_attempt_supported(const tdq_tableau *tab, int32_t dtype, int32_t width) {
    if (!tab || dtype != TDQ_F32 || width != LD) return 0;
    TdqHostShape hs;
    tdq_shape_from_tableau(tab, &hs);
    unsigned long long rm;
    unsigned em;
    if (!attempt_masks(hs, &rm, &em)) return 0;
    const int S = hs.n_stages;
    return ((S == 6 && rm == RM_DOPRI5 && em == 0x3du) || (S == 3 && rm == RM_BOSH3 && em == 0x07u)) ? 1 : 0;
}

int tdq_linear_attempt(void *ctrl_dev, const tdq_tableau *tab, int32_t dtype, void *const *k_out, void *y1_out, void *err_out,
                       const void *y0, const void *k0, const void *planes, int32_t width, size_t n, double *partials,
                       double *norm_out, const int64_t *seg_counts_dev, int32_t store_always, void *stream) {
    TDQ_REQUIRE(ctrl_dev && tab && k_out && y1_out && err_out && planes, "null argument");
    TDQ_REQUIRE(dtype == TDQ_F32 && width == LD, "the fused linear field is float32, width 128");
    TDQ_REQUIRE(n % (size_t)width == 0, "state size is not a multiple of the field width");
    TDQ_REQUIRE((partials == nullptr) == (norm_out == nullptr), "partials and norm_out go together");
    TDQ_REQUIRE(seg_counts_dev == nullptr, "seg_counts_dev is reserved and must be NULL");
    const size_t n_rows = n / (size_t)width;
    TDQ_REQUIRE(n_rows < ((size_t)1 << 31) - 64, "too many rows");
    TdqHostShape hs;
    tdq_shape_from_tableau(tab, &hs);
    unsigned long long rm = 0;
    unsigned em = 0;
    TDQ_REQUIRE(attempt_masks(hs, &rm, &em), "the whole-attempt kernel takes FSAL tableaus of at most 7 stages");
    const int S = hs.n_stages;
    AttOut out;
    memset(&out, 0, sizeof(out));
    for (int i = 1; i <= S; ++i) {
        TDQ_REQUIRE(k_out[i] != nullptr, "missing stage slot");
        out.k[i] = (float *)k_out[i];
    }
    out.y1 = (float *)y1_out;
    out.err = (float *)err_out;
    if (n_rows == 0) return TDQ_OK;
    TdqCtrl *c = (TdqCtrl *)ctrl_dev;
    const uint32_t *wt = (const uint32_t *)planes;
    cudaStream_t st = (cudaStream_t)stream;
    int rc = -1;
    if (S == 6 && rm == RM_DOPRI5 && em == 0x3du)
        rc = launch_attempt<6, RM_DOPRI5, 0x3du>(c, (const float *)y0, (const float *)k0, out, wt, partials, norm_out, store_always, n_rows, st);
    else if (S == 3 && rm == RM_BOSH3 && em == 0x07u)
        rc = launch_attempt<3, RM_BOSH3, 0x07u>(c, (const float *)y0, (const float *)k0, out, wt, partials, norm_out, store_always, n_rows, st);
    TDQ_REQUIRE(rc != -1, "no whole-attempt kernel for this tableau (tdq_linear_attempt_supported)");
    TDQ_REQUIRE(rc == 0, "launch configuration failed");
    TDQ_CHECK_CUDA(cudaGetLastError());
    return TDQ_OK;
}

}
```

torchdiffeq_b200/csrc/tdq_ctrl.cu:

```cuda
#include "tdq_common.cuh"
#include "tdq_shape.cuh"
#include "tdq_step.cuh"

namespace {

template <typename T> __device__ __forceinline__ void store_T(unsigned char *raw, int i, T v) {
    reinterpret_cast<T *>(raw)[i] = v;
}

template <typename T> __device__ void prepare_scalar(TdqCtrl &c) {
    if (c.halt) return;
    if (c.n_steps_interval >= c.max_num_steps) {
        c.status = TDQ_RUN_MAX_STEPS;
        c.halt = 1;
        return;
    }
    double dt = tdq_clamp_dt(c.dt, c.min_step, c.max_step);
    const double t0 = c.t1;
    double t1 = t0 + dt;
    c.att_t0 = t0;
    c.att_dt = dt;
    if (!(t0 + dt > t0)) {
        c.status = TDQ_RUN_DT_UNDERFLOW;
        c.halt = 1;
        return;
    }
    if (c.y0_bad) {
        c.status = TDQ_RUN_NONFINITE;
        c.halt = 1;
        return;
    }
    c.on_step_t = 0;
    if (c.n_step_t > 0) {
        const double nxt = c.step_t[c.next_step_index];
        if (t0 < nxt && nxt < t0 + dt) {
            c.on_step_t = 1;
            t1 = nxt;
            dt = t1 - t0;
        }
    }
    c.on_jump_t = 0;
    if (c.n_jump_t > 0) {
        const double nxt = c.jump_t[c.next_jump_index];
        if (t0 < nxt && nxt < t0 + dt) {
            c.on_jump_t = 1;
            c.on_step_t = 0;
            t1 = nxt;
            dt = t1 - t0;
        }
    }
    c.att_dt = dt;
    c.att_t1 = t1;
    c.att_dtT = (double)(T)dt;
}

template <typename T> __device__ void prepare_tables(TdqCtrl &c, int tid, int nthreads) {
    if (c.halt) return;
    const T t0T = (T)c.att_t0, dtT = (T)c.att_dt, t1T = (T)c.att_t1;
    const T sgn = (T)c.t_sign;
    const int S = c.n_stages;
    for (int i = tid; i < S; i += nthreads)
        store_T<T>(c.tstage, i, tdq_stage_time<T>((T)c.alpha[i], t0T, dtT, t1T, sgn));
    const int rows = c.fsal ? S : S + 1;
    for (int e = tid; e < rows * TDQ_MAX_K; e += nthreads) {
        const int r = e / TDQ_MAX_K, m = e % TDQ_MAX_K;
        if (m < c.row_nnz[r]) c.coef[r][m] = (double)tdq_coef<T>(sgn, (T)c.beta[r][m], dtT);
    }
    for (int m = tid; m < c.err_nnz; m += nthreads)
        c.ecoef[m] = (double)tdq_coef<T>(sgn, (T)c.c_err[m], dtT);
}

template <typename T> __device__ void prepare_attempt(TdqCtrl &c) {
    prepare_scalar<T>(c);
    prepare_tables<T>(c, 0, 1);
}

template <typename T, int THREADS>
__device__ double block_norm_from_sums(const TdqCtrl &c, const double *sums, const int64_t *counts, int n_seg,
                                       double *smem ) {
    double best = 0.0;
    int nan = 0;
    for (int s = threadIdx.x; s < n_seg; s += THREADS) {
        const double cnt = counts ? (double)counts[s] : (double)c.n_global;
        if (cnt <= 0.0) continue;
        const double r = tdq_rms<T>(sums[s], cnt, c.ratio_f64);
        if (r != r) nan = 1;
        if (r > best) best = r;
    }
#pragma unroll
    for (int o = 16; o > 0; o >>= 1) {
        const double ob = __shfl_down_sync(0xffffffffu, best, o);
        const int on = __shfl_down_sync(0xffffffffu, nan, o);
        if (ob > best) best = ob;
        nan |= on;
    }
    const int lane = threadIdx.x & 31, w = threadIdx.x >> 5;
    __syncthreads();
    if (lane == 0) smem[w] = nan ? CUDART_NAN : best;
    __syncthreads();
    if (threadIdx.x == 0) {
        double b = 0.0;
        bool bn = false;
        for (int i = 0; i < THREADS / 32; ++i) {
            const double v = smem[i];
            if (v != v) bn = true;
            else if (v > b) b = v;
        }
        smem[THREADS / 32] = bn ? CUDART_NAN : b;
    }
    __syncthreads();
    return smem[THREADS / 32];
}

static __device__ void write_mailbox(TdqCtrl &c, double fin_t0, double fin_dt, int jumped = 0) {
    c.seq += 1;
    tdq_mailbox *m = c.mbox;
    if (!m) return;
    if (c.loop_handle != 0ull && !c.halt) return;
    m->status = c.status;
    m->accept = c.accept;
    m->done = c.done;
    m->out_cursor = c.out_cursor;
    m->n_accept = c.n_accept;
    m->n_reject = c.n_reject;
    m->t0 = c.t0;
    m->t1 = c.t1;
    m->dt = c.dt;
    m->ratio = c.ratio;
    m->att_t0 = fin_t0;
    m->att_dt = fin_dt;
    m->next_t0 = c.att_t0;
    m->next_dt = c.att_dt;
    m->on_jump_t = jumped;
    m->par = c.par;
    __threadfence_system();
    m->seq = c.seq;
}

template <typename T>
__device__ void controller(TdqCtrl &c, const double *norm_in, int n_seg, const void *ratio_dev, double ratio_pre) {
    if (c.halt) {
        c.accept = 0;
        c.fit_now = 0;
        c.emit_lo = c.emit_hi;
        write_mailbox(c, c.att_t0, c.att_dt);
        return;
    }
    using A = Ar<T>;
    double ratio;
    if (ratio_dev) {
        ratio = c.ratio_f64 ? *reinterpret_cast<const double *>(ratio_dev)
                            : (double)*reinterpret_cast<const T *>(ratio_dev);
        ratio = fabs(ratio);
    } else {
        ratio = ratio_pre;
    }
    const bool y1_nonfinite = norm_in && norm_in[n_seg] > 0.0;
    if (y1_nonfinite && !ratio_dev) ratio = CUDART_NAN;
    c.ratio = ratio;

    const double dt = c.att_dt;
    const bool accept = tdq_accept(ratio, dt, c.min_step, c.max_step);
    c.accept = accept ? 1 : 0;

    if (accept) {
        c.t0 = c.att_t0;
        c.t1 = c.att_t1;
        c.n_accept += 1;
        c.y0_prev = c.y0_cur;
        c.k0_prev = c.k0_cur;
        c.par ^= 1;
        c.y0_cur = c.ybuf[c.par];
        c.k0_cur = c.kbuf[c.par];
        if (c.on_step_t && c.next_step_index != c.n_step_t - 1) c.next_step_index += 1;
        if (c.on_jump_t) {
            if (c.next_jump_index != c.n_jump_t - 1) c.next_jump_index += 1;
            store_T<T>(c.taux, 2, A::mul((T)c.t_sign, next_repr<T>((T)c.att_t1)));
        }
        const T dtT = (T)c.att_dtT, sgn = (T)c.t_sign;
        c.fit_sdt = (double)A::mul(sgn, dtT);
        for (int m = 0; m < c.mid_nnz; ++m)
            c.fit_mcoef[m] = (double)tdq_coef<T>(sgn, (T)c.c_mid[m], dtT);
        if (y1_nonfinite) {
            c.status = TDQ_RUN_NONFINITE;
            c.halt = 1;
        }
    } else {
        c.t0 = c.att_t0;
        c.t1 = c.att_t0;
        c.n_reject += 1;
    }

    const double dt_next = tdq_next_dt(ratio, dt, c.safety, c.ifactor, c.dfactor, c.order, c.min_step, c.max_step);
    c.dt = dt_next;

    c.emit_lo = c.out_cursor;
    c.n_steps_interval += 1;
    if (accept) {
        const int cur = tdq_cursor_after(c.t_out, c.n_out, c.out_cursor, c.t1);
        if (cur != c.out_cursor) c.n_steps_interval = 0;
        c.out_cursor = cur;
    }
    c.emit_hi = c.out_cursor;
    c.fit_now = (accept && (c.always_fit || c.emit_hi > c.emit_lo)) ? 1 : 0;
    if (c.out_cursor >= c.n_out) {
        c.done = 1;
        c.halt = 1;
    }
    const double fin_t0 = c.att_t0, fin_dt = c.att_dt;
    const int jumped = (accept && c.on_jump_t) ? 1 : 0;
    prepare_scalar<T>(c);
    write_mailbox(c, fin_t0, fin_dt, jumped);
}

constexpr int kCtrlThreads = 256;
static_assert(sizeof(TdqCtrl) % 8 == 0, "control block must be a whole number of 8-byte words");
static_assert(sizeof(TdqCtrl) <= 40 * 1024, "control block must fit static shared memory");

template <typename T>
__global__ void __launch_bounds__(kCtrlThreads)
k_controller(TdqCtrl *c, const double *norm_in, const int64_t *cnt, int n_seg, const void *ratio_dev) {
    __shared__ __align__(16) unsigned char raw[sizeof(TdqCtrl)];
    constexpr int kWords = (int)(sizeof(TdqCtrl) / 8);
    unsigned long long *sw = reinterpret_cast<unsigned long long *>(raw);
    const unsigned long long *gw = reinterpret_cast<const unsigned long long *>(c);
    for (int i = threadIdx.x; i < kWords; i += kCtrlThreads) sw[i] = gw[i];
    __syncthreads();
    TdqCtrl &sc = *reinterpret_cast<TdqCtrl *>(raw);
    __shared__ double xsum[TDQ_MAX_SEGS + 2];
    __shared__ int xfail;
    if (sc.xworld > 1 && !sc.halt && norm_in != nullptr && ratio_dev == nullptr && n_seg <= TDQ_MAX_SEGS) {
        const int R = sc.xworld, me = sc.xrank, nv = n_seg + 1;
        const int par = (int)(((sc.xepoch & 1ull) << 1) | (sc.seq & 1ull));
        const unsigned long long want = (sc.xepoch << 32) | (sc.seq + 1ull);
        if (threadIdx.x == 0) xfail = 0;
        __syncthreads();
        if ((int)threadIdx.x < R) {
            const int t = threadIdx.x;
            TdqXBuf *peer = reinterpret_cast<TdqXBuf *>(sc.xpeer[t]);
            for (int i = 0; i < nv; ++i) peer->vals[par][me][i] = norm_in[i];
            __threadfence_system();
            asm volatile("st.release.sys.global.u64 [%0], %1;" :: "l"(&peer->flags[par][me]), "l"(want) : "memory");
            TdqXBuf *mine = reinterpret_cast<TdqXBuf *>(sc.xpeer[me]);
            unsigned long long seen = 0, t0 = 0, now = 0;
            asm volatile("mov.u64 %0, %%globaltimer;" : "=l"(t0));
            do {
                asm volatile("ld.acquire.sys.global.u64 %0, [%1];" : "=l"(seen) : "l"(&mine->flags[par][t]) : "memory");
                if (seen == want) break;
                asm volatile("mov.u64 %0, %%globaltimer;" : "=l"(now));
            } while (now - t0 < 10000000000ull);
            if (seen != want) atomicExch(&xfail, 1);
        }
        __syncthreads();
        if (threadIdx.x == 0) {
            if (xfail) {
                sc.status = TDQ_RUN_EXCHANGE_TIMEOUT;
                sc.halt = 1;
            } else {
                const TdqXBuf *mine = reinterpret_cast<const TdqXBuf *>(sc.xpeer[me]);
                for (int i = 0; i < nv; ++i) {
                    double a = 0.0;
                    for (int r = 0; r < R; ++r) a += __ldcg(&mine->vals[par][r][i]);
                    xsum[i] = a;
                }
            }
        }
        __syncthreads();
        norm_in = xsum;
    }
    __shared__ double nsm[kCtrlThreads / 32 + 1];
    double ratio_pre = 0.0;
    if (!sc.halt && ratio_dev == nullptr)
        ratio_pre = block_norm_from_sums<T, kCtrlThreads>(sc, norm_in, cnt, n_seg, nsm);
    __shared__ int was_halted;
    if (threadIdx.x == 0) {
        was_halted = sc.halt;
        controller<T>(sc, norm_in, n_seg, ratio_dev, ratio_pre);
    }
    __syncthreads();
    if (!was_halted) prepare_tables<T>(sc, threadIdx.x, kCtrlThreads);
    __syncthreads();
    unsigned long long *go = reinterpret_cast<unsigned long long *>(c);
    for (int i = threadIdx.x; i < kWords; i += kCtrlThreads) go[i] = sw[i];
    if (threadIdx.x == 0 && sc.loop_handle != 0ull)
        cudaGraphSetConditional((cudaGraphConditionalHandle)sc.loop_handle, sc.halt ? 0u : 1u);
}

template <typename T>
__device__ void initial_h0(TdqCtrl &c, double d0d, double d1d) {
    using A = Ar<T>;
    const double h0 = tdq_initial_h0<T>(c.ratio_f64 != 0, d0d, d1d);
    c.h0 = h0;
    c.ratio = d1d;
    const T tp = (T)(c.t1 + h0);
    store_T<T>(c.taux, 1, A::mul((T)c.t_sign, tp));
}

template <typename T>
__device__ void initial_finish(TdqCtrl &c, double nd) {
    const double dt = tdq_initial_finish<T>(c.ratio_f64 != 0, c.order, c.ratio, c.h0, nd);
    c.dt = dt;
}

template <typename T> __global__ void k_prepare(TdqCtrl *c, const double *y0_bad) {
    if (y0_bad && *y0_bad > 0.0) c->y0_bad = 1;
    prepare_attempt<T>(*c);
    c->y0_bad = 0;
    if (c->mbox) {
        c->mbox->status = c->status;
        c->mbox->next_t0 = c->att_t0;
        c->mbox->next_dt = c->att_dt;
        __threadfence_system();
    }
}
constexpr int kInitThreads = 128;
template <typename T>
__global__ void __launch_bounds__(kInitThreads)
k_initial_h0(TdqCtrl *c, const double *s0, const double *s1, const int64_t *cnt, int n_seg) {
    __shared__ double nsm[kInitThreads / 32 + 1];
    const double d0 = block_norm_from_sums<T, kInitThreads>(*c, s0, cnt, n_seg, nsm);
    const double d1 = block_norm_from_sums<T, kInitThreads>(*c, s1, cnt, n_seg, nsm);
    if (threadIdx.x == 0) initial_h0<T>(*c, d0, d1);
}
template <typename T>
__global__ void __launch_bounds__(kInitThreads)
k_initial_finish(TdqCtrl *c, const double *s2, const int64_t *cnt, int n_seg) {
    __shared__ double nsm[kInitThreads / 32 + 1];
    const double nd = block_norm_from_sums<T, kInitThreads>(*c, s2, cnt, n_seg, nsm);
    if (threadIdx.x == 0) initial_finish<T>(*c, nd);
}
__global__ void k_set_loop(TdqCtrl *c, unsigned long long h) { c->loop_handle = h; }
__global__ void k_set_first_step(TdqCtrl *c, double dt) { c->dt = dt; }
struct XPtrs { const void *p[TDQ_MAX_RANKS]; };
__global__ void k_set_exchange(TdqCtrl *c, XPtrs xp, int rank, int world, unsigned long long epoch) {
    for (int r = 0; r < TDQ_MAX_RANKS; ++r) c->xpeer[r] = const_cast<void *>(xp.p[r]);
    c->xrank = rank;
    c->xworld = world;
    c->xepoch = epoch;
}
__global__ void k_reset_interval(TdqCtrl *c) { c->n_steps_interval = 0; }
__global__ void k_set_jump_t(TdqCtrl *c, const double *jt, int n) {
    c->jump_t = jt;
    c->n_jump_t = n;
    int idx = 0;
    while (idx < n && !(jt[idx] > c->t1)) ++idx;
    c->next_jump_index = (idx < n - 1) ? idx : (n - 1);
    if (n <= 0) c->next_jump_index = 0;
}
__global__ void k_set_step_t(TdqCtrl *c, const double *st, int n) {
    c->step_t = st;
    c->n_step_t = n;
    int idx = 0;
    while (idx < n && !(st[idx] > c->t1)) ++idx;
    c->next_step_index = (idx < n - 1) ? idx : (n - 1);
    if (n <= 0) c->next_step_index = 0;
}

}

extern "C" {

size_t tdq_ctrl_size(void) { return (sizeof(TdqCtrl) + 255) & ~size_t(255); }
size_t tdq_ctrl_tstage_offset(void) { return offsetof(TdqCtrl, tstage); }
size_t tdq_ctrl_taux_offset(void) { return offsetof(TdqCtrl, taux); }

static float round_f32(double x) { return (float)x; }

int tdq_ctrl_init(void *ctrl_dev, const tdq_tableau *tab, const tdq_options *opt, const double *t_out_dev,
                  double t_start, int32_t n_out, void *mailbox_dev, void *stream) {
    TDQ_REQUIRE(ctrl_dev && tab && opt, "null argument");
    TDQ_REQUIRE(tab->n_stages >= 1 && tab->n_stages <= TDQ_MAX_STAGES, "n_stages out of range");
    TDQ_REQUIRE(opt->dtype == TDQ_F32 || opt->dtype == TDQ_F64, "unsupported dtype");
    TDQ_REQUIRE(n_out >= 1, "need at least one output time");
    static thread_local TdqCtrl h;
    memset(&h, 0, sizeof(h));
    const bool f32 = opt->dtype == TDQ_F32;
    auto rT = [&](double x) { return f32 ? (double)round_f32(x) : x; };
    const int S = tab->n_stages;
    h.dtype = opt->dtype;
    h.n_stages = S;
    h.order = tab->order;
    h.fsal = tab->fsal ? 1 : 0;
    h.ratio_f64 = (opt->ratio_f64 || !f32) ? 1 : 0;
    h.n_out = n_out;
    TdqHostShape hs;
    tdq_shape_from_tableau(tab, &hs);
    static_assert(sizeof(h.row_idx) == sizeof(hs.row_idx) && sizeof(h.err_idx) == sizeof(hs.err_idx), "index layouts");
    memcpy(h.row_nnz, hs.row_nnz, sizeof(h.row_nnz));
    memcpy(h.row_idx, hs.row_idx, sizeof(h.row_idx));
    memcpy(h.err_idx, hs.err_idx, sizeof(h.err_idx));
    memcpy(h.mid_idx, hs.mid_idx, sizeof(h.mid_idx));
    h.err_nnz = hs.err_nnz;
    h.mid_nnz = hs.mid_nnz;
    for (int i = 0; i < S; ++i) h.alpha[i] = rT(tab->alpha[i]);
    for (int i = 0; i <= S; ++i) {
        const double *w = i < S ? tab->beta[i] : tab->c_sol;
        for (int m = 0; m < hs.row_nnz[i]; ++m) h.beta[i][m] = rT(w[hs.row_idx[i][m]]);
    }
    for (int m = 0; m < hs.err_nnz; ++m) h.c_err[m] = rT(tab->c_err[hs.err_idx[m]]);
    for (int m = 0; m < hs.mid_nnz; ++m) h.c_mid[m] = rT(tab->c_mid[hs.mid_idx[m]]);
    h.rtol = opt->rtol;
    h.atol = opt->atol;
    h.min_step = opt->min_step;
    h.max_step = opt->max_step;
    h.safety = opt->safety;
    h.ifactor = opt->ifactor;
    h.dfactor = opt->dfactor;
    h.t_sign = (opt->t_sign < 0) ? -1.0 : 1.0;
    h.max_num_steps = opt->max_num_steps;
    h.n_global = opt->n_global;
    h.t_out = t_out_dev;
    h.mbox = reinterpret_cast<tdq_mailbox *>(mailbox_dev);
    h.t0 = h.t1 = t_start;
    h.dt = 0.0;
    TDQ_REQUIRE((opt->ybuf[0] == nullptr) == (opt->ybuf[1] == nullptr) &&
                    (opt->ybuf[0] == nullptr) == (opt->kbuf[0] == nullptr) &&
                    (opt->ybuf[0] == nullptr) == (opt->kbuf[1] == nullptr),
                "ybuf/kbuf: give all four state buffers or none");
    for (int i = 0; i < 2; ++i) {
        TDQ_REQUIRE(tdq_aligned16(opt->ybuf[i]) && tdq_aligned16(opt->kbuf[i]), "state buffers must be 16-byte aligned");
        h.ybuf[i] = opt->ybuf[i];
        h.kbuf[i] = opt->kbuf[i];
    }
    h.par = 0;
    h.y0_cur = h.y0_prev = h.ybuf[0];
    h.k0_cur = h.k0_prev = h.kbuf[0];
    h.always_fit = opt->always_fit ? 1 : 0;
    h.loop_handle = opt->loop_handle;
    h.out_cursor = 1;
    h.emit_lo = h.emit_hi = 1;
    if (n_out <= 1) { h.done = 1; h.halt = 1; }
    if (f32) {
        float v = (float)h.t_sign * (float)t_start;
        memcpy(h.taux, &v, sizeof(v));
    } else {
        double v = h.t_sign * t_start;
        memcpy(h.taux, &v, sizeof(v));
    }
    TDQ_CHECK_CUDA(cudaMemcpyAsync(ctrl_dev, &h, sizeof(h), cudaMemcpyHostToDevice, (cudaStream_t)stream));
    return TDQ_OK;
}

int tdq_ctrl_set_step_t(void *ctrl_dev, const double *step_t_dev, int32_t n, void *stream) {
    TDQ_REQUIRE(ctrl_dev, "null ctrl");
    k_set_step_t<<<1, 1, 0, (cudaStream_t)stream>>>((TdqCtrl *)ctrl_dev, step_t_dev, n);
    TDQ_CHECK_CUDA(cudaGetLastError());
    return TDQ_OK;
}

int tdq_ctrl_set_jump_t(void *ctrl_dev, const double *jump_t_dev, int32_t n, void *stream) {
    TDQ_REQUIRE(ctrl_dev, "null ctrl");
    k_set_jump_t<<<1, 1, 0, (cudaStream_t)stream>>>((TdqCtrl *)ctrl_dev, jump_t_dev, n);
    TDQ_CHECK_CUDA(cudaGetLastError());
    return TDQ_OK;
}

int tdq_prepare_attempt(void *ctrl_dev, int32_t dtype, const double *y0_nonfinite_count_dev, void *stream) {
    TDQ_REQUIRE(ctrl_dev, "null ctrl");
    TDQ_DISPATCH_T(dtype, (k_prepare<T><<<1, 1, 0, (cudaStream_t)stream>>>((TdqCtrl *)ctrl_dev, y0_nonfinite_count_dev)));
    TDQ_CHECK_CUDA(cudaGetLastError());
    return TDQ_OK;
}

int tdq_controller(void *ctrl_dev, int32_t dtype, const double *norm_in, const int64_t *seg_counts_dev,
                   int32_t n_seg, const void *ratio_dev, void *stream) {
    TDQ_REQUIRE(ctrl_dev, "null ctrl");
    TDQ_REQUIRE(norm_in || ratio_dev, "need norm sums or an explicit ratio");
    TDQ_REQUIRE(n_seg >= 1, "n_seg out of range");
    TDQ_DISPATCH_T(dtype, (k_controller<T><<<1, kCtrlThreads, 0, (cudaStream_t)stream>>>(
                               (TdqCtrl *)ctrl_dev, norm_in, seg_counts_dev, n_seg, ratio_dev)));
    TDQ_CHECK_CUDA(cudaGetLastError());
    return TDQ_OK;
}

int tdq_initial_step_h0(void *ctrl_dev, int32_t dtype, const double *d0_sumsq, const double *d1_sumsq,
                        const int64_t *seg_counts_dev, int32_t n_seg, void *stream) {
    TDQ_REQUIRE(ctrl_dev && d0_sumsq && d1_sumsq, "null argument");
    TDQ_DISPATCH_T(dtype, (k_initial_h0<T><<<1, kInitThreads, 0, (cudaStream_t)stream>>>(
                               (TdqCtrl *)ctrl_dev, d0_sumsq, d1_sumsq, seg_counts_dev, n_seg)));
    TDQ_CHECK_CUDA(cudaGetLastError());
    return TDQ_OK;
}

int tdq_initial_step_finish(void *ctrl_dev, int32_t dtype, const double *d2_sumsq,
                            const int64_t *seg_counts_dev, int32_t n_seg, void *stream) {
    TDQ_REQUIRE(ctrl_dev && d2_sumsq, "null argument");
    TDQ_DISPATCH_T(dtype, (k_initial_finish<T><<<1, kInitThreads, 0, (cudaStream_t)stream>>>(
                               (TdqCtrl *)ctrl_dev, d2_sumsq, seg_counts_dev, n_seg)));
    TDQ_CHECK_CUDA(cudaGetLastError());
    return TDQ_OK;
}

int tdq_set_first_step(void *ctrl_dev, double first_step, void *stream) {
    TDQ_REQUIRE(ctrl_dev, "null ctrl");
    k_set_first_step<<<1, 1, 0, (cudaStream_t)stream>>>((TdqCtrl *)ctrl_dev, first_step);
    TDQ_CHECK_CUDA(cudaGetLastError());
    return TDQ_OK;
}

int tdq_ctrl_set_exchange(void *ctrl_dev, const void *const *peer_ptrs, int32_t rank, int32_t world, uint64_t epoch,
                          void *stream) {
    TDQ_REQUIRE(ctrl_dev && peer_ptrs, "null argument");
    TDQ_REQUIRE(world >= 1 && world <= TDQ_MAX_RANKS && rank >= 0 && rank < world, "rank/world out of range");
    XPtrs xp;
    memset(&xp, 0, sizeof(xp));
    for (int r = 0; r < world; ++r) {
        TDQ_REQUIRE(peer_ptrs[r] != nullptr, "missing peer buffer");
        xp.p[r] = peer_ptrs[r];
    }
    k_set_exchange<<<1, 1, 0, (cudaStream_t)stream>>>((TdqCtrl *)ctrl_dev, xp, rank, world, (unsigned long long)epoch);
    TDQ_CHECK_CUDA(cudaGetLastError());
    return TDQ_OK;
}

int tdq_xchg_create(void **dev_ptr, tdq_ipc_handle *handle_out) {
    TDQ_REQUIRE(dev_ptr && handle_out, "null argument");
    static_assert(sizeof(cudaIpcMemHandle_t) <= sizeof(tdq_ipc_handle), "IPC handle does not fit");
    void *p = nullptr;
    TDQ_CHECK_CUDA(cudaMalloc(&p, sizeof(TdqXBuf)));
    TDQ_CHECK_CUDA(cudaMemset(p, 0, sizeof(TdqXBuf)));
    TDQ_CHECK_CUDA(cudaDeviceSynchronize());
    cudaIpcMemHandle_t h;
    cudaError_t e = cudaIpcGetMemHandle(&h, p);
    if (e != cudaSuccess) {
        cudaFree(p);
        tdq_set_error("cudaIpcGetMemHandle failed: %s", cudaGetErrorString(e));
        return TDQ_ERR_CUDA;
    }
    memset(handle_out, 0, sizeof(*handle_out));
    memcpy(handle_out->bytes, &h, sizeof(h));
    *dev_ptr = p;
    return TDQ_OK;
}

int tdq_xchg_open(const tdq_ipc_handle *handle, void **peer_ptr) {
    TDQ_REQUIRE(handle && peer_ptr, "null argument");
    cudaIpcMemHandle_t h;
    memcpy(&h, handle->bytes, sizeof(h));
    TDQ_CHECK_CUDA(cudaIpcOpenMemHandle(peer_ptr, h, cudaIpcMemLazyEnablePeerAccess));
    return TDQ_OK;
}

int tdq_xchg_close(void *peer_ptr) {
    if (peer_ptr) TDQ_CHECK_CUDA(cudaIpcCloseMemHandle(peer_ptr));
    return TDQ_OK;
}

int tdq_xchg_destroy(void *dev_ptr) {
    if (dev_ptr) TDQ_CHECK_CUDA(cudaFree(dev_ptr));
    return TDQ_OK;
}

int tdq_ctrl_set_loop(void *ctrl_dev, uint64_t loop_handle, void *stream) {
    TDQ_REQUIRE(ctrl_dev, "null ctrl");
    k_set_loop<<<1, 1, 0, (cudaStream_t)stream>>>((TdqCtrl *)ctrl_dev, (unsigned long long)loop_handle);
    TDQ_CHECK_CUDA(cudaGetLastError());
    return TDQ_OK;
}

int tdq_ctrl_reset_interval(void *ctrl_dev, void *stream) {
    TDQ_REQUIRE(ctrl_dev, "null ctrl");
    k_reset_interval<<<1, 1, 0, (cudaStream_t)stream>>>((TdqCtrl *)ctrl_dev);
    TDQ_CHECK_CUDA(cudaGetLastError());
    return TDQ_OK;
}

}
```

torchdiffeq_b200/csrc/tdq_interp.cu:

```cuda
#include "tdq_common.cuh"
#include "tdq_shape.cuh"
#include "tdq_step.cuh"

namespace {

constexpr int kThreads = 256;

template <typename T, int NK, bool VECTOR, bool STORE>
__global__ void __launch_bounds__(kThreads)
k_fit_eval(const TdqCtrl *__restrict__ c, const T *__restrict__ y1p, const T *__restrict__ kSp, KPtrs kmid,
           T *__restrict__ ce, T *__restrict__ cd, T *__restrict__ cc, T *__restrict__ cb, T *__restrict__ ca,
           T *__restrict__ solution, size_t n) {
    if (!c->fit_now) return;
    using A = Ar<T>;
    const T *y0p = reinterpret_cast<const T *>(c->y0_prev);
    const T *k0p = reinterpret_cast<const T *>(c->k0_prev);
    T mf[NK];
    const T *km[NK];
#pragma unroll
    for (int m = 0; m < NK; ++m) {
        mf[m] = (T)c->fit_mcoef[m];
        km[m] = reinterpret_cast<const T *>(kmid.p[m] ? kmid.p[m] : (const void *)k0p);
    }
    const T sdt = (T)c->fit_sdt;
    const T two_sdt = A::mul((T)2, sdt);
    const int lo = c->emit_lo, hi = c->emit_hi;
    const double t0 = c->t0, t1 = c->t1;

    auto fit = [&](T y0v, T y1v, T f0, T f1, const T *kv, T &e, T &d, T &cq, T &b, T &a) {
        tdq_quartic<T>(y0v, y1v, f0, f1, tdq_combine<T, NK>(y0v, kv, mf), sdt, two_sdt, e, d, cq, b, a);
    };
    auto xof = [&](int j) -> T { return (T)((c->t_out[j] - t0) / (t1 - t0)); };

    if (VECTOR) {
        using V = Vec<T>;
        const size_t nvec = n / V::N;
        for (size_t v = (size_t)blockIdx.x * kThreads + threadIdx.x; v < nvec; v += (size_t)gridDim.x * kThreads) {
            const size_t i0 = v * V::N;
            V a0 = ld_stream<T>(y0p + i0), a1 = ld_stream<T>(y1p + i0);
            V f0 = ld_stream<T>(k0p + i0), f1 = ld_stream<T>(kSp + i0);
            V kv[NK];
#pragma unroll
            for (int m = 0; m < NK; ++m) kv[m] = ld_stream<T>(km[m] + i0);
            V re, rd, rc, rb, ra;
#pragma unroll
            for (int e = 0; e < V::N; ++e) {
                T ke[NK];
#pragma unroll
                for (int m = 0; m < NK; ++m) ke[m] = kv[m].v[e];
                fit(a0.v[e], a1.v[e], f0.v[e], f1.v[e], ke, re.v[e], rd.v[e], rc.v[e], rb.v[e], ra.v[e]);
            }
            if (STORE) {
                st_vec<T>(ce + i0, re); st_vec<T>(cd + i0, rd); st_vec<T>(cc + i0, rc);
                st_vec<T>(cb + i0, rb); st_vec<T>(ca + i0, ra);
            }
            for (int j = lo; j < hi; ++j) {
                const T x = xof(j);
                V r;
#pragma unroll
                for (int l = 0; l < V::N; ++l) r.v[l] = tdq_eval_poly<T>(re.v[l], rd.v[l], rc.v[l], rb.v[l], ra.v[l], x);
                st_vec<T>(solution + (size_t)j * n + i0, r);
            }
        }
        if (blockIdx.x == gridDim.x - 1) {
            const size_t i = nvec * V::N + threadIdx.x;
            if (i < n) {
                T ke[NK];
#pragma unroll
                for (int m = 0; m < NK; ++m) ke[m] = km[m][i];
                T e, d, cq, b, a;
                fit(y0p[i], y1p[i], k0p[i], kSp[i], ke, e, d, cq, b, a);
                if (STORE) { ce[i] = e; cd[i] = d; cc[i] = cq; cb[i] = b; ca[i] = a; }
                for (int j = lo; j < hi; ++j) solution[(size_t)j * n + i] = tdq_eval_poly<T>(e, d, cq, b, a, xof(j));
            }
        }
    } else {
        for (size_t i = (size_t)blockIdx.x * kThreads + threadIdx.x; i < n; i += (size_t)gridDim.x * kThreads) {
            T ke[NK];
#pragma unroll
            for (int m = 0; m < NK; ++m) ke[m] = km[m][i];
            T e, d, cq, b, a;
            fit(y0p[i], y1p[i], k0p[i], kSp[i], ke, e, d, cq, b, a);
            if (STORE) { ce[i] = e; cd[i] = d; cc[i] = cq; cb[i] = b; ca[i] = a; }
            for (int j = lo; j < hi; ++j) solution[(size_t)j * n + i] = tdq_eval_poly<T>(e, d, cq, b, a, xof(j));
        }
    }
}

template <typename T, int NK>
int launch_fit(const TdqCtrl *c, const void *y1, const void *kS, const KPtrs &kmid, void *const *coeff, void *solution,
               size_t n, bool vec, cudaStream_t st) {
    const unsigned blocks = tdq_grid(vec ? n / Vec<T>::N : n, kThreads, 2);
    T *co[5] = {nullptr, nullptr, nullptr, nullptr, nullptr};
    if (coeff) for (int i = 0; i < 5; ++i) co[i] = (T *)coeff[i];
    return tdq_dispatch(TdqBool{}, vec, [&](auto V) {
        return tdq_dispatch(TdqBool{}, coeff != nullptr, [&](auto S) {
            k_fit_eval<T, NK, V, S><<<blocks, kThreads, 0, st>>>(c, (const T *)y1, (const T *)kS, kmid, co[0], co[1], co[2],
                                                                 co[3], co[4], (T *)solution, n);
            return 0;
        });
    });
}

template <typename T>
__global__ void __launch_bounds__(kThreads)
k_poly_eval(const T *__restrict__ ce, const T *__restrict__ cd, const T *__restrict__ cc, const T *__restrict__ cb,
            const T *__restrict__ ca, T *__restrict__ out, double x64, size_t n) {
    const T x = (T)x64;
    for (size_t i = (size_t)blockIdx.x * kThreads + threadIdx.x; i < n; i += (size_t)gridDim.x * kThreads)
        out[i] = tdq_eval_poly<T>(ce[i], cd[i], cc[i], cb[i], ca[i], x);
}

template <typename T>
__global__ void __launch_bounds__(kThreads)
k_interp_eval_at(const TdqCtrl *__restrict__ c, const T *__restrict__ ce, const T *__restrict__ cd,
                 const T *__restrict__ cc, const T *__restrict__ cb, const T *__restrict__ ca, T *__restrict__ out,
                 const double *__restrict__ t_at, size_t n) {
    const double t0 = c->t0, t1 = c->t1;
    const T x = (T)((*t_at - t0) / (t1 - t0));
    for (size_t i = (size_t)blockIdx.x * kThreads + threadIdx.x; i < n; i += (size_t)gridDim.x * kThreads)
        out[i] = tdq_eval_poly<T>(ce[i], cd[i], cc[i], cb[i], ca[i], x);
}

template <typename T>
__global__ void __launch_bounds__(kThreads)
k_probe(const TdqCtrl *__restrict__ c, T *__restrict__ out, const T *y0, const T *f0, size_t n) {
    if (y0 == nullptr) y0 = reinterpret_cast<const T *>(c->y0_cur);
    if (f0 == nullptr) f0 = reinterpret_cast<const T *>(c->k0_cur);
    const T h = tdq_probe_h<T>(c->t_sign, c->h0);
    for (size_t i = (size_t)blockIdx.x * kThreads + threadIdx.x; i < n; i += (size_t)gridDim.x * kThreads)
        out[i] = tdq_probe<T>(y0[i], h, f0[i]);
}

}

extern "C" {

int tdq_initial_step_probe(void *ctrl_dev, int32_t dtype, void *y_probe, const void *y0, const void *f0, size_t n,
                           void *stream) {
    TDQ_REQUIRE(ctrl_dev && y_probe, "null argument");
    if (n == 0) return TDQ_OK;
    const unsigned blocks = tdq_grid(n, kThreads, 16);
    TDQ_DISPATCH_T(dtype, (k_probe<T><<<blocks, kThreads, 0, (cudaStream_t)stream>>>(
                               (const TdqCtrl *)ctrl_dev, (T *)y_probe, (const T *)y0, (const T *)f0, n)));
    TDQ_CHECK_CUDA(cudaGetLastError());
    return TDQ_OK;
}

int tdq_interp_fit_eval(void *ctrl_dev, const tdq_tableau *tab, int32_t dtype, const void *y1, const void *const *k,
                        void *const *coeff, void *solution, size_t n, void *stream) {
    TDQ_REQUIRE(ctrl_dev && tab && y1 && k && solution, "null argument");
    TdqHostShape hs;
    tdq_shape_from_tableau(tab, &hs);
    const int S = hs.n_stages;
    const int nk = hs.mid_nnz;
    TDQ_REQUIRE(nk >= 1, "tableau has no mid-point weights");
    TDQ_REQUIRE(k[S] != nullptr, "k_S is required");
    KPtrs kmid;
    bool vec = tdq_aligned16(y1) && tdq_aligned16(k[S]) && tdq_aligned16(solution) &&
               ((n * (dtype == TDQ_F32 ? 4 : 8)) % 16 == 0);
    TDQ_REQUIRE(tdq_plan_terms(hs.mid_idx, nk, k, kmid.p, vec) == TDQ_PLAN_OK,
                "missing stage slot for a non-zero mid-point weight");
    if (coeff)
        for (int i = 0; i < 5; ++i) {
            TDQ_REQUIRE(coeff[i] != nullptr, "five coefficient buffers are required");
            vec = vec && tdq_aligned16(coeff[i]);
        }
    if (n == 0) return TDQ_OK;
    int rc = -1;
    TDQ_DISPATCH_T(dtype, rc = tdq_dispatch(TdqRange<1, TDQ_MAX_K>{}, nk, [&](auto NK) {
                       return launch_fit<T, NK>((const TdqCtrl *)ctrl_dev, y1, k[S], kmid, coeff, solution, n, vec,
                                                (cudaStream_t)stream);
                   }));
    TDQ_REQUIRE(rc == 0, "unsupported number of mid-point terms");
    TDQ_CHECK_CUDA(cudaGetLastError());
    return TDQ_OK;
}

int tdq_poly_eval(int32_t dtype, const void *const *coeff, double x, void *out, size_t n, void *stream) {
    TDQ_REQUIRE(coeff && out, "null argument");
    for (int i = 0; i < 5; ++i) TDQ_REQUIRE(coeff[i] != nullptr, "five coefficient buffers are required");
    if (n == 0) return TDQ_OK;
    const unsigned blocks = tdq_grid(n, kThreads, 8);
    TDQ_DISPATCH_T(dtype, (k_poly_eval<T><<<blocks, kThreads, 0, (cudaStream_t)stream>>>(
                               (const T *)coeff[0], (const T *)coeff[1], (const T *)coeff[2], (const T *)coeff[3],
                               (const T *)coeff[4], (T *)out, x, n)));
    TDQ_CHECK_CUDA(cudaGetLastError());
    return TDQ_OK;
}

int tdq_interp_eval_at(void *ctrl_dev, int32_t dtype, const void *const *coeff, const double *t_dev, void *out,
                       size_t n, void *stream) {
    TDQ_REQUIRE(ctrl_dev && coeff && out && t_dev, "null argument");
    for (int i = 0; i < 5; ++i) TDQ_REQUIRE(coeff[i] != nullptr, "five coefficient buffers are required");
    if (n == 0) return TDQ_OK;
    const unsigned blocks = tdq_grid(n, kThreads, 8);
    TDQ_DISPATCH_T(dtype, (k_interp_eval_at<T><<<blocks, kThreads, 0, (cudaStream_t)stream>>>(
                               (const TdqCtrl *)ctrl_dev, (const T *)coeff[0], (const T *)coeff[1], (const T *)coeff[2],
                               (const T *)coeff[3], (const T *)coeff[4], (T *)out, t_dev, n)));
    TDQ_CHECK_CUDA(cudaGetLastError());
    return TDQ_OK;
}

}
```

Measured before the change: 3.426 million.

## Run whole linear-ODE solve in one persistent kernel with grid barriers

Adds a persistent cooperative kernel that runs the whole adaptive dopri5 loop for linear vector fields on the device. Stage attempts, the norm reduction, the step controller and dense-output fitting all run inside it, separated by software grid barriers. This removes per-attempt kernel launches, graph or loop dispatch and host mailbox polling. The cost is grid-wide barrier synchronization, a timeout error path, and reliance on all blocks being co-resident.

```diff
diff --git a/include/tdq.h b/include/tdq.h
--- a/include/tdq.h
+++ b/include/tdq.h
@@ -29,7 +29,8 @@
     TDQ_RUN_DT_UNDERFLOW = 1,
     TDQ_RUN_NONFINITE = 2,
     TDQ_RUN_MAX_STEPS = 3,
-    TDQ_RUN_EXCHANGE_TIMEOUT = 4
+    TDQ_RUN_EXCHANGE_TIMEOUT = 4,
+    TDQ_RUN_BARRIER_TIMEOUT = 5
 } tdq_run_status;
 
 typedef struct {
@@ -168,6 +169,11 @@
 int tdq_linear_attempt(void *ctrl_dev, const tdq_tableau *tab, int32_t dtype, void *const *k_out, void *y1_out, void *err_out,
                        const void *y0, const void *k0, const void *planes, int32_t width, size_t n, double *partials,
                        double *norm_out, const int64_t *seg_counts_dev, int32_t store_always, void *stream);
+
+size_t tdq_linear_solve_scratch_len(void);
+int tdq_linear_solve(void *ctrl_dev, const tdq_tableau *tab, int32_t dtype, void *const *k_out, void *y1_out, void *err_out,
+                     const void *planes, int32_t width, size_t n, double *scratch, size_t scratch_len,
+                     const int64_t *seg_counts_dev, void *solution, void *stream);
 
 int tdq_fixed_emit_cubic(int32_t dtype, const void *y0, const void *y1, const void *f0, const void *f1, void *solution,
                          const int32_t *out_idx_dev, const void *coef_dev, int32_t rec_lo, int32_t rec_hi, size_t n,
diff --git a/torchdiffeq_b200/_engine.py b/torchdiffeq_b200/_engine.py
--- a/torchdiffeq_b200/_engine.py
+++ b/torchdiffeq_b200/_engine.py
@@ -236,6 +236,8 @@
         self._loop = None
         self._loop_handle = 0
         self._loop_failed = False
+        self._solve_scratch = None
+        self._solve_refused = False
         self._always_copy = False
         self.linear = None
         self.capture_in_solve = True
@@ -458,6 +460,8 @@
             raise SolverFailure("non-finite values in state `y`: {}".format(y) + where)
         if s == _lib.RUN_EXCHANGE_TIMEOUT:
             raise _lib.TdqError("a peer rank did not deliver its norm partials within 10 s (sharded solve)")
+        if s == _lib.RUN_BARRIER_TIMEOUT:
+            raise _lib.TdqError("a block of the persistent linear solve missed a grid barrier by 10 s")
         if s == _lib.RUN_MAX_STEPS:
             m = self.opt.max_num_steps
             raise SolverFailure("max_num_steps exceeded ({}>={})".format(m, m) + where)
@@ -667,6 +671,8 @@
         return torch.tensor(t0, **kw), torch.tensor(dt, **kw)
 
     def _loop_run_ahead(self):
+        if self._linear_solve_ready() and self._linear_solve():
+            return
         D = max(1, self.run_ahead)
         mb = self.mbox_host.contents
         issued = 0
@@ -713,6 +719,34 @@
         self._raise_if_failed(mb)
         torch.cuda.current_stream().synchronize()
 
+    persistent_linear = True
+
+    def _linear_solve_ready(self):
+        L = self.linear
+        return (L is not None and L["whole"] and L["fold"] and self.persistent_linear and not self._solve_refused
+                and self.device_loop in (True, "auto") and not self._lockstep_mode() and self.agree_fn is None
+                and self.norm_fn is None and self.exchange is None and not self.keep_interp)
+
+    def _linear_solve(self):
+        lib, L = self.lib, self.linear
+        if self._solve_scratch is None:
+            self._solve_scratch = torch.zeros(int(lib.tdq_linear_solve_scratch_len()), dtype=torch.float64,
+                                              device=self.device)
+        k = [None] + [L["k"][i].data_ptr() for i in range(self.S)]
+        rc = lib.tdq_linear_solve(self.ctrl.data_ptr(), C.byref(self.tab), self.dt_code, _lib.ptr_array(k),
+                                  self.y1.data_ptr(), self.errp.data_ptr(), L["planes"].data_ptr(), L["width"], self.n,
+                                  self._solve_scratch.data_ptr(), self._solve_scratch.numel(), self.seg_counts.data_ptr(),
+                                  self.solution.data_ptr(), _stream())
+        if rc == _lib.TDQ_ERR_UNSUPPORTED:
+            self._solve_refused = True
+            return False
+        self._launch(rc)
+        torch.cuda.current_stream().synchronize()
+        mb = self.mbox_host.contents
+        self.nfe += self.S * int(mb.seq)
+        self._raise_if_failed(mb)
+        return True
+
     def _launch_loop(self, first=0):
         _lib.check(self.lib.tdq_loop_launch(self._loop, _stream()))
         torch.cuda.current_stream().synchronize()
@@ -805,6 +839,8 @@
 
 
 class RowsEngine(AdaptiveEngine):
+
+    persistent_linear = False
 
     def __init__(self, fn, shape, dtype, device, method, **kw):
         shape = torch.Size(shape)
diff --git a/torchdiffeq_b200/_lib.py b/torchdiffeq_b200/_lib.py
--- a/torchdiffeq_b200/_lib.py
+++ b/torchdiffeq_b200/_lib.py
@@ -8,7 +8,8 @@
 TDQ_MAX_K = TDQ_MAX_STAGES + 1
 TDQ_MAX_SEGS = 64
 TDQ_F32, TDQ_F64 = 0, 1
-RUN_OK, RUN_DT_UNDERFLOW, RUN_NONFINITE, RUN_MAX_STEPS, RUN_EXCHANGE_TIMEOUT = 0, 1, 2, 3, 4
+TDQ_ERR_UNSUPPORTED = 3
+RUN_OK, RUN_DT_UNDERFLOW, RUN_NONFINITE, RUN_MAX_STEPS, RUN_EXCHANGE_TIMEOUT, RUN_BARRIER_TIMEOUT = 0, 1, 2, 3, 4, 5
 TDQ_MAX_RANKS = 16
 (ROWS_T0, ROWS_T1, ROWS_DT, ROWS_RATIO, ROWS_ATT_T0, ROWS_ATT_DT, ROWS_ATT_T1, ROWS_FIT_DT, ROWS_H0, ROWS_D1, ROWS_PAR,
  ROWS_ACCEPT, ROWS_FIT, ROWS_DONE, ROWS_STATUS, ROWS_CURSOR, ROWS_EMIT_LO, ROWS_EMIT_HI, ROWS_N_STEPS, ROWS_N_ACCEPT,
@@ -116,6 +117,8 @@
     "tdq_linear_stage": (C.c_int, [_vp, _ptab, _i32, _i32, _vp, _vp, _vp, _vp, _pp, _vp, _i32, _sz, _vp]),
     "tdq_linear_attempt_supported": (C.c_int, [_ptab, _i32, _i32]),
     "tdq_linear_attempt": (C.c_int, [_vp, _ptab, _i32, _pp, _vp, _vp, _vp, _vp, _vp, _i32, _sz, _vp, _vp, _vp, _i32, _vp]),
+    "tdq_linear_solve_scratch_len": (_sz, []),
+    "tdq_linear_solve": (C.c_int, [_vp, _ptab, _i32, _pp, _vp, _vp, _vp, _i32, _sz, _vp, _sz, _vp, _vp, _vp]),
     "tdq_fixed_emit_cubic": (C.c_int, [_i32, _vp, _vp, _vp, _vp, _vp, _vp, _vp, _i32, _i32, _sz, _vp]),
     "tdq_pack_segments": (C.c_int, [_i32, _vp, _pp, _pi64, _pi64, _pdbl, _i32, _vp]),
     "tdq_implicit_partials_len": (_sz, [_i32]),
diff --git a/torchdiffeq_b200/csrc/build.py b/torchdiffeq_b200/csrc/build.py
--- a/torchdiffeq_b200/csrc/build.py
+++ b/torchdiffeq_b200/csrc/build.py
@@ -8,7 +8,7 @@
 ROOT = os.path.dirname(os.path.dirname(HERE))
 INCLUDE = os.path.join(ROOT, "include")
 SOURCES = ["tdq_api.cu", "tdq_ctrl.cu", "tdq_stream.cu", "tdq_norm.cu", "tdq_interp.cu", "tdq_fixed.cu", "tdq_graph.cu", "tdq_linear.cu", "tdq_attempt.cu", "tdq_implicit.cu", "tdq_rows.cu"]
-HEADERS = [os.path.join(HERE, "tdq_common.cuh"), os.path.join(HERE, "tdq_shape.cuh"), os.path.join(HERE, "tdq_step.cuh"), os.path.join(HERE, "tdq_tc.cuh"), os.path.join(HERE, "tdq_tableau_tsit5.inc"), os.path.join(INCLUDE, "tdq.h")]
+HEADERS = [os.path.join(HERE, "tdq_common.cuh"), os.path.join(HERE, "tdq_shape.cuh"), os.path.join(HERE, "tdq_step.cuh"), os.path.join(HERE, "tdq_tc.cuh"), os.path.join(HERE, "tdq_ctrl_step.cuh"), os.path.join(HERE, "tdq_fit.cuh"), os.path.join(HERE, "tdq_tableau_tsit5.inc"), os.path.join(INCLUDE, "tdq.h")]
 LIB = os.path.join(HERE, "libtdq.so")
 STAMP = os.path.join(HERE, "libtdq.stamp")
 
diff --git a/torchdiffeq_b200/csrc/tdq_attempt.cu b/torchdiffeq_b200/csrc/tdq_attempt.cu
--- a/torchdiffeq_b200/csrc/tdq_attempt.cu
+++ b/torchdiffeq_b200/csrc/tdq_attempt.cu
@@ -1,5 +1,7 @@
 #include "tdq_shape.cuh"
 #include "tdq_tc.cuh"
+#include "tdq_ctrl_step.cuh"
+#include "tdq_fit.cuh"
 
 #include <cstddef>
 #include <type_traits>
@@ -39,37 +41,36 @@
     float *y1, *err;
 };
 
+struct Scalars {
+    const float *y0, *k0;
+    float *ycand, *kcand;
+    AttOut out;
+    float rtol, atol;
+};
+
+constexpr int AUX_CR = 64;
+constexpr int AUX_SC = 320;
+constexpr int AUX_RED = 512;
+constexpr int AUX_SOLVE = 1024;
+static_assert(AUX_SC + sizeof(Scalars) <= AUX_RED, "aux layout");
+
+__device__ __forceinline__ uint8_t *at_smem() {
+    extern __shared__ uint8_t smem_raw[];
+    return reinterpret_cast<uint8_t *>((reinterpret_cast<uintptr_t>(smem_raw) + 127) & ~(uintptr_t)127);
+}
+__device__ __forceinline__ uint8_t *at_aux(uint8_t *smem) { return smem + W_BYTES + AT_STAGE + AT_Y0; }
+
 template <int S, unsigned long long RM, unsigned EM>
-__global__ void __launch_bounds__(AT_THREADS, 1)
-k_linear_attempt(TdqCtrl *c, const float *y0, const float *k0, AttOut out, const uint32_t *__restrict__ wt,
-                 double *partials, double *norm_out, int store_always, size_t n_rows_sz) {
-    if (c->halt) return;
-    extern __shared__ uint8_t smem_raw[];
-    uint8_t *smem = reinterpret_cast<uint8_t *>((reinterpret_cast<uintptr_t>(smem_raw) + 127) & ~(uintptr_t)127);
-    uint8_t *aux = smem + W_BYTES + AT_STAGE + AT_Y0;
-    int *s_flag = reinterpret_cast<int *>(aux);
-    struct Scalars {
-        const float *y0, *k0;
-        float *ycand, *kcand;
-        AttOut out;
-        float rtol, atol;
-    };
-    Scalars *s_sc = reinterpret_cast<Scalars *>(aux + 320);
-    static_assert(320 + sizeof(Scalars) <= 512, "aux layout");
-    float *s_cr = reinterpret_cast<float *>(aux + 64);
+__device__ __forceinline__ void attempt_prologue(const TdqCtrl *c, const float *y0, const float *k0, const AttOut &out,
+                                                 bool fold, size_t n_rows_sz, uint8_t *aux, int tid) {
+    float *s_cr = reinterpret_cast<float *>(aux + AUX_CR);
     float *s_ce = s_cr + AT_MAX_S * 8;
-    double *s_red = reinterpret_cast<double *>(aux + 512);
-    const int tid = threadIdx.x, lane = tid & 31;
-    const int warp = __shfl_sync(0xffffffffu, tid >> 5, 0);
-    const int n_rows = (int)n_rows_sz;
-
     if (tid < AT_MAX_S * 8) {
         const int i = tid >> 3, j = tid & 7;
         const unsigned mask = i < S ? (unsigned)((RM >> (8 * i)) & 0xffull) : 0u, below = (1u << j) - 1u;
         s_cr[i * 8 + j] = ((mask >> j) & 1u) ? (float)c->coef[i][__popc(mask & below)] : 0.f;
         if (i == 0) s_ce[j] = j == S ? (float)c->ecoef[__popc(EM)] : ((EM >> j) & 1u) ? (float)c->ecoef[__popc(EM & below)] : 0.f;
     }
-    const bool fold = partials != nullptr;
     if (tid == 0) {
         Scalars sc;
         sc.y0 = tdq_detach(y0 != nullptr ? y0 : reinterpret_cast<const float *>(c->y0_cur), n_rows_sz);
@@ -82,41 +83,51 @@
         sc.out = out;
         sc.rtol = (float)c->rtol;
         sc.atol = (float)c->atol;
-        *s_sc = sc;
-    }
-    load_weights(smem, wt, tid, AT_THREADS);
-    fence_async_smem();
-    __syncthreads();
-
+        *reinterpret_cast<Scalars *>(aux + AUX_SC) = sc;
+    }
+}
+
+__device__ __forceinline__ bool attempt_store(const TdqCtrl *c, int store_always) {
     bool store = store_always != 0 || c->always_fit != 0;
     if (!store) {
         const int cur = c->out_cursor;
         store = cur < c->n_out && !(c->t_out[cur] > c->att_t1);
     }
+    return store;
+}
+
+__device__ __forceinline__ void load_ahi(uint32_t (&ahi)[LD / 16][4], const uint8_t *smem) {
+    const int tid = threadIdx.x, lane = tid & 31, warp = tid >> 5;
+    const int h = warp >> 2, w = warp & 3;
+    const uint32_t wsm_h = smem_u32(smem) + h * 8 * SBO;
+#pragma unroll
+    for (int ks = 0; ks < LD / 16; ++ks) {
+#pragma unroll
+        for (int r = 0; r < 4; ++r) {
+            const int f = 16 * w + (lane >> 2) + 8 * (r & 1), k = 16 * ks + 2 * (lane & 3) + 8 * (r >> 1);
+            asm volatile("ld.shared.b32 %0, [%1];" : "=r"(ahi[ks][r])
+                         : "r"(wsm_h + (f >> 3) * SBO + (k >> 3) * LBO + (f & 7) * 16 + (k & 7) * 2));
+        }
+    }
+}
+
+template <int S, unsigned long long RM, unsigned EM>
+__device__ __forceinline__ void attempt_tiles(uint8_t *smem, const uint32_t (&ahi)[LD / 16][4], bool store, bool fold, int n_rows,
+                                              int tid, double &acc, int &nbad) {
+    const int lane = tid & 31;
+    const int warp = __shfl_sync(0xffffffffu, tid >> 5, 0);
     const int h = warp >> 2, w = warp & 3;
     const uint32_t wsm = smem_u32(smem);
-    const uint32_t ssc = wsm + (uint32_t)(reinterpret_cast<uint8_t *>(s_sc) - smem);
-    const uint32_t scoef = wsm + (uint32_t)(reinterpret_cast<uint8_t *>(s_cr) - smem);
+    const uint32_t ssc = wsm + (uint32_t)(at_aux(smem) - smem) + AUX_SC;
+    const uint32_t scoef = wsm + (uint32_t)(at_aux(smem) - smem) + AUX_CR;
     auto coef = [scoef](int i, int j) { return lds_pinned_f32(scoef + 4 * (8 * i + j)); };
     const uint32_t wsm_h = wsm + h * 8 * SBO;
     const uint32_t stage = wsm + W_BYTES;
     const uint32_t sy0 = stage + AT_STAGE + tid * 4;
     const uint64_t dw = make_desc(wsm_h), dy = make_desc(stage);
-    uint32_t ahi[LD / 16][4];
-#pragma unroll
-    for (int ks = 0; ks < LD / 16; ++ks) {
-#pragma unroll
-        for (int r = 0; r < 4; ++r) {
-            const int f = 16 * w + (lane >> 2) + 8 * (r & 1), k = 16 * ks + 2 * (lane & 3) + 8 * (r >> 1);
-            asm volatile("ld.shared.b32 %0, [%1];" : "=r"(ahi[ks][r])
-                         : "r"(wsm_h + (f >> 3) * SBO + (k >> 3) * LBO + (f & 7) * 16 + (k & 7) * 2));
-        }
-    }
     const int toff = thread_offset(w, lane) + 64 * h;
 
     const int tiles = (n_rows + AT_ROWS - 1) / AT_ROWS;
-    double acc = 0.0;
-    int nbad = 0;
 
     constexpr int KEEP = S < 4 ? S : 4;
     constexpr int NACC = S - KEEP;
@@ -320,20 +331,18 @@
         if (n_rows - t * AT_ROWS >= AT_ROWS) do_tile(std::true_type{}, t);
         else do_tile(std::false_type{}, t);
     }
-    const double bad = (double)nbad;
-
-    if (!fold) return;
+}
+
+__device__ __forceinline__ void cta_partial(double acc, int nbad, double *s_red, double *p_sum, double *p_bad) {
+    const int tid = threadIdx.x, lane = tid & 31, warp = tid >> 5;
     {
-        const double wa = warp_sum(acc), wb = warp_sum(bad);
+        const double wa = warp_sum(acc), wb = warp_sum((double)nbad);
         if (lane == 0) {
             s_red[warp] = wa;
             s_red[32 + warp] = wb;
         }
     }
     __syncthreads();
-    const int P = (int)gridDim.x;
-    double *p_sum = partials + 2, *p_bad = p_sum + P;
-    unsigned int *ticket = reinterpret_cast<unsigned int *>(partials);
     if (tid == 0) {
         double a = 0.0, b = 0.0;
         for (int w_ = 0; w_ < AT_THREADS / 32; ++w_) {
@@ -342,6 +351,49 @@
         }
         p_sum[blockIdx.x] = a;
         p_bad[blockIdx.x] = b;
+    }
+}
+
+__device__ __forceinline__ void sum_partials(const double *p_sum, const double *p_bad, int P, double &a, double &b) {
+    const int lane = threadIdx.x & 31;
+    a = 0.0;
+    b = 0.0;
+    for (int i = lane; i < P; i += 32) {
+        a += __ldcg(&p_sum[i]);
+        b += __ldcg(&p_bad[i]);
+    }
+    a = warp_sum(a);
+    b = warp_sum(b);
+}
+
+template <int S, unsigned long long RM, unsigned EM>
+__global__ void __launch_bounds__(AT_THREADS, 1)
+k_linear_attempt(TdqCtrl *c, const float *y0, const float *k0, AttOut out, const uint32_t *__restrict__ wt,
+                 double *partials, double *norm_out, int store_always, size_t n_rows_sz) {
+    if (c->halt) return;
+    uint8_t *smem = at_smem();
+    uint8_t *aux = at_aux(smem);
+    int *s_flag = reinterpret_cast<int *>(aux);
+    double *s_red = reinterpret_cast<double *>(aux + AUX_RED);
+    const int tid = threadIdx.x;
+    const bool fold = partials != nullptr;
+    attempt_prologue<S, RM, EM>(c, y0, k0, out, fold, n_rows_sz, aux, tid);
+    load_weights(smem, wt, tid, AT_THREADS);
+    fence_async_smem();
+    __syncthreads();
+    const bool store = attempt_store(c, store_always);
+    uint32_t ahi[LD / 16][4];
+    load_ahi(ahi, smem);
+    double acc = 0.0;
+    int nbad = 0;
+    attempt_tiles<S, RM, EM>(smem, ahi, store, fold, (int)n_rows_sz, tid, acc, nbad);
+
+    if (!fold) return;
+    const int P = (int)gridDim.x;
+    double *p_sum = partials + 2, *p_bad = p_sum + P;
+    unsigned int *ticket = reinterpret_cast<unsigned int *>(partials);
+    cta_partial(acc, nbad, s_red, p_sum, p_bad);
+    if (tid == 0) {
         __threadfence();
         const unsigned int tk = atomicAdd(ticket, 1u);
         *s_flag = (tk == gridDim.x - 1) ? 1 : 0;
@@ -349,19 +401,168 @@
     __syncthreads();
     if (!*s_flag) return;
     __threadfence();
-    if (warp == 0) {
-        double a = 0.0, b = 0.0;
-        for (int i = lane; i < P; i += 32) {
-            a += __ldcg(&p_sum[i]);
-            b += __ldcg(&p_bad[i]);
-        }
-        a = warp_sum(a);
-        b = warp_sum(b);
-        if (lane == 0) {
+    if ((tid >> 5) == 0) {
+        double a, b;
+        sum_partials(p_sum, p_bad, P, a, b);
+        if (tid == 0) {
             norm_out[0] = a;
             norm_out[1] = b;
             *ticket = 0;
         }
+    }
+}
+
+enum { BAR_ARRIVE = 0, BAR_RELEASE = 1, BAR_FIT = 2, BAR_ABORT = 3, BAR_WORDS = 4 };
+
+struct SolveAux {
+    double norm[2];
+    double nsm[AT_THREADS / 32 + 1];
+    int attempt, fits, fit_now, halt, was_halted, ok;
+    KPtrs kmid;
+    const float *y1s, *kSs;
+    float *solution;
+    unsigned long long n;
+    unsigned block, blocks;
+};
+static_assert(AUX_SOLVE + sizeof(SolveAux) <= AT_AUX, "aux layout");
+constexpr int SV_CTRL = (AT_SMEM + 15) & ~15;
+constexpr int SV_SMEM = SV_CTRL + (int)sizeof(TdqCtrl);
+
+__device__ __forceinline__ int opaque_tid() {
+    int t;
+    asm volatile("mov.u32 %0, %%tid.x;" : "=r"(t));
+    return t;
+}
+
+__device__ __forceinline__ unsigned ld_acquire_u32(const unsigned *p) {
+    unsigned v;
+    asm volatile("ld.acquire.gpu.global.u32 %0, [%1];" : "=r"(v) : "l"(p) : "memory");
+    return v;
+}
+__device__ __forceinline__ unsigned long long global_ns() {
+    unsigned long long t;
+    asm volatile("mov.u64 %0, %%globaltimer;" : "=l"(t));
+    return t;
+}
+
+__device__ __forceinline__ bool bar_wait(TdqCtrl *c, unsigned *bar, int which, unsigned target) {
+    const unsigned long long t0 = global_ns();
+    for (;;) {
+        if ((int)(ld_acquire_u32(bar + which) - target) >= 0) return true;
+        if (ld_acquire_u32(bar + BAR_ABORT) != 0u) return false;
+        if (global_ns() - t0 > 10000000000ull) break;
+    }
+    if (atomicExch(bar + BAR_ABORT, 1u) == 0u) {
+        c->status = TDQ_RUN_BARRIER_TIMEOUT;
+        c->halt = 1;
+        if (c->mbox) {
+            c->mbox->status = TDQ_RUN_BARRIER_TIMEOUT;
+            __threadfence_system();
+        }
+    }
+    return false;
+}
+
+__device__ __forceinline__ void bar_arrive(unsigned *bar, int which) {
+    __threadfence();
+    atomicAdd(bar + which, 1u);
+}
+
+__device__ __forceinline__ void solve_controller_step(TdqCtrl *c, uint8_t *smem, SolveAux *sx, const int64_t *cnt) {
+    unsigned char *raw = smem + SV_CTRL;
+    ctrl_stage_in(c, raw);
+    ctrl_decide<float, AT_THREADS>(*reinterpret_cast<TdqCtrl *>(raw), sx->norm, cnt, 1, nullptr, true, sx->nsm, &sx->was_halted,
+                                    opaque_tid());
+    ctrl_stage_out(c, raw);
+}
+
+template <int S, unsigned long long RM, unsigned EM, int NK>
+__global__ void __launch_bounds__(AT_THREADS, 1)
+k_linear_solve(TdqCtrl *c, AttOut out, const uint32_t *__restrict__ wt, unsigned *bar, double *part, const int64_t *cnt,
+               KPtrs kmid, const float *y1s, const float *kSs, float *solution, size_t n_rows_sz) {
+    uint8_t *smem = at_smem();
+    uint8_t *aux = at_aux(smem);
+    double *s_red = reinterpret_cast<double *>(aux + AUX_RED);
+    volatile SolveAux *sxv = reinterpret_cast<volatile SolveAux *>(aux + AUX_SOLVE);
+    SolveAux *sx = reinterpret_cast<SolveAux *>(aux + AUX_SOLVE);
+    const int tid = threadIdx.x;
+    const unsigned P = gridDim.x;
+    if (c->halt) {
+        if (blockIdx.x == 0) solve_controller_step(c, smem, sx, cnt);
+        return;
+    }
+    load_weights(smem, wt, tid, AT_THREADS);
+    fence_async_smem();
+    if (tid == 0) {
+        sx->attempt = 0;
+        sx->fits = 0;
+        sx->kmid = kmid;
+        sx->y1s = y1s;
+        sx->kSs = kSs;
+        sx->solution = solution;
+        sx->n = n_rows_sz * LD;
+        sx->block = blockIdx.x;
+        sx->blocks = gridDim.x;
+    }
+    __syncthreads();
+    uint32_t ahi[LD / 16][4];
+    load_ahi(ahi, smem);
+    for (;;) {
+        attempt_prologue<S, RM, EM>(c, nullptr, nullptr, out, true, n_rows_sz, aux, opaque_tid());
+        __syncthreads();
+        const bool store = attempt_store(c, 0);
+        double acc = 0.0;
+        int nbad = 0;
+        attempt_tiles<S, RM, EM>(smem, ahi, store, true, (int)n_rows_sz, opaque_tid(), acc, nbad);
+        const unsigned a = (unsigned)sxv->attempt;
+        double *p_sum = part + (a & 1u) * 2 * P, *p_bad = p_sum + P;
+        cta_partial(acc, nbad, s_red, p_sum, p_bad);
+        if (tid == 0) bar_arrive(bar, BAR_ARRIVE);
+        if (blockIdx.x == 0) {
+            if (tid == 0) sxv->ok = bar_wait(c, bar, BAR_ARRIVE, P * (a + 1u));
+            __syncthreads();
+            if (!sxv->ok) return;
+            if ((tid >> 5) == 0) {
+                double sa, sb;
+                sum_partials(p_sum, p_bad, (int)P, sa, sb);
+                if (tid == 0) {
+                    sxv->norm[0] = sa;
+                    sxv->norm[1] = sb;
+                }
+            }
+            __syncthreads();
+            solve_controller_step(c, smem, sx, cnt);
+            __syncthreads();
+            if (tid == 0) {
+                __threadfence();
+                asm volatile("st.release.gpu.global.u32 [%0], %1;" :: "l"(bar + BAR_RELEASE), "r"(a + 1u) : "memory");
+            }
+        } else if (tid == 0) {
+            sxv->ok = bar_wait(c, bar, BAR_RELEASE, a + 1u);
+        }
+        if (tid == 0) {
+            sxv->fit_now = c->fit_now;
+            sxv->halt = c->halt;
+            sxv->attempt = (int)(a + 1u);
+        }
+        __syncthreads();
+        if (!sxv->ok) return;
+        if (sxv->fit_now) {
+            KPtrs km;
+#pragma unroll
+            for (int m = 0; m < NK; ++m) km.p[m] = sxv->kmid.p[m];
+            fit_eval_body<float, NK, true, false>(c, sxv->y1s, sxv->kSs, km, nullptr, nullptr, nullptr, nullptr, nullptr,
+                                                  sxv->solution, (size_t)sxv->n, sxv->block, sxv->blocks);
+            __syncthreads();
+            if (tid == 0) {
+                bar_arrive(bar, BAR_FIT);
+                sxv->fits = sxv->fits + 1;
+                sxv->ok = bar_wait(c, bar, BAR_FIT, P * (unsigned)sxv->fits);
+            }
+            __syncthreads();
+            if (!sxv->ok) return;
+        }
+        if (sxv->halt) return;
     }
 }
 
@@ -374,6 +575,28 @@
     auto kern = k_linear_attempt<S, RM, EM>;
     if (cudaFuncSetAttribute(kern, cudaFuncAttributeMaxDynamicSharedMemorySize, AT_SMEM) != cudaSuccess) return -2;
     kern<<<tdq_grid(n_rows, AT_ROWS, 1), AT_THREADS, AT_SMEM, st>>>(c, y0, k0, out, wt, partials, norm_out, store_always, n_rows);
+    return 0;
+}
+
+template <int S, unsigned long long RM, unsigned EM, int NK>
+int launch_solve(TdqCtrl *c, const AttOut &out, const uint32_t *wt, unsigned *bar, double *part, const int64_t *cnt,
+                 const KPtrs &kmid, const float *y1, const float *kS, float *solution, size_t n_rows, cudaStream_t st) {
+    auto kern = k_linear_solve<S, RM, EM, NK>;
+    if (cudaFuncSetAttribute(kern, cudaFuncAttributeMaxDynamicSharedMemorySize, SV_SMEM) != cudaSuccess) return -2;
+    cudaLaunchConfig_t cfg = {};
+    cfg.gridDim = dim3(tdq_grid(n_rows, AT_ROWS, 1));
+    cfg.blockDim = dim3(AT_THREADS);
+    cfg.dynamicSmemBytes = SV_SMEM;
+    cfg.stream = st;
+    cudaLaunchAttribute attr[1];
+    attr[0].id = cudaLaunchAttributeCooperative;
+    attr[0].val.cooperative = 1;
+    cfg.attrs = attr;
+    cfg.numAttrs = 1;
+    if (cudaLaunchKernelEx(&cfg, kern, c, out, wt, bar, part, cnt, kmid, y1, kS, solution, n_rows) != cudaSuccess) {
+        (void)cudaGetLastError();
+        return -3;
+    }
     return 0;
 }
 
@@ -453,4 +676,61 @@
     return TDQ_OK;
 }
 
-}
+size_t tdq_linear_solve_scratch_len(void) { return (size_t)(2 + 4 * tdq_sm_count()); }
+
+int tdq_linear_solve(void *ctrl_dev, const tdq_tableau *tab, int32_t dtype, void *const *k_out, void *y1_out, void *err_out,
+                     const void *planes, int32_t width, size_t n, double *scratch, size_t scratch_len,
+                     const int64_t *seg_counts_dev, void *solution, void *stream) {
+    TDQ_REQUIRE(ctrl_dev && tab && k_out && y1_out && err_out && planes && scratch && seg_counts_dev && solution, "null argument");
+    TDQ_REQUIRE(dtype == TDQ_F32 && width == LD, "the fused linear field is float32, width 128");
+    TDQ_REQUIRE(n % (size_t)width == 0 && n > 0, "state size is not a positive multiple of the field width");
+    const size_t n_rows = n / (size_t)width;
+    TDQ_REQUIRE(n_rows < ((size_t)1 << 31) - 64, "too many rows");
+    TDQ_REQUIRE(scratch_len >= tdq_linear_solve_scratch_len(), "scratch is shorter than tdq_linear_solve_scratch_len()");
+    TdqHostShape hs;
+    tdq_shape_from_tableau(tab, &hs);
+    unsigned long long rm = 0;
+    unsigned em = 0;
+    TDQ_REQUIRE(attempt_masks(hs, &rm, &em), "the whole-attempt kernel takes FSAL tableaus of at most 7 stages");
+    const int S = hs.n_stages;
+    AttOut out;
+    memset(&out, 0, sizeof(out));
+    const void *k[TDQ_MAX_K] = {nullptr};
+    for (int i = 1; i <= S; ++i) {
+        TDQ_REQUIRE(k_out[i] != nullptr, "missing stage slot");
+        out.k[i] = (float *)k_out[i];
+        k[i] = k_out[i];
+    }
+    out.y1 = (float *)y1_out;
+    out.err = (float *)err_out;
+    KPtrs kmid;
+    bool vec = tdq_aligned16(y1_out) && tdq_aligned16(k_out[S]) && tdq_aligned16(solution) && (n * 4) % 16 == 0;
+    TDQ_REQUIRE(hs.mid_nnz >= 1 && tdq_plan_terms(hs.mid_idx, hs.mid_nnz, k, kmid.p, vec) == TDQ_PLAN_OK,
+                "missing stage slot for a non-zero mid-point weight");
+    if (!vec) {
+        tdq_set_error("tdq_linear_solve: the stage, y1 and solution buffers must be 16-byte aligned");
+        return TDQ_ERR_UNSUPPORTED;
+    }
+    unsigned *bar = reinterpret_cast<unsigned *>(scratch);
+    cudaStream_t st = (cudaStream_t)stream;
+    TDQ_CHECK_CUDA(cudaMemsetAsync(bar, 0, BAR_WORDS * sizeof(unsigned), st));
+    TdqCtrl *c = (TdqCtrl *)ctrl_dev;
+    const uint32_t *wt = (const uint32_t *)planes;
+    int rc = -1;
+    if (S == 6 && rm == RM_DOPRI5 && em == 0x3du && hs.mid_nnz == 6)
+        rc = launch_solve<6, RM_DOPRI5, 0x3du, 6>(c, out, wt, bar, scratch + 2, seg_counts_dev, kmid, (const float *)y1_out,
+                                                 (const float *)k_out[S], (float *)solution, n_rows, st);
+    else if (S == 3 && rm == RM_BOSH3 && em == 0x07u && hs.mid_nnz == 1)
+        rc = launch_solve<3, RM_BOSH3, 0x07u, 1>(c, out, wt, bar, scratch + 2, seg_counts_dev, kmid, (const float *)y1_out,
+                                                (const float *)k_out[S], (float *)solution, n_rows, st);
+    TDQ_REQUIRE(rc != -1, "no persistent solve kernel for this tableau (tdq_linear_attempt_supported)");
+    TDQ_REQUIRE(rc != -2, "launch configuration failed");
+    if (rc == -3) {
+        tdq_set_error("tdq_linear_solve: the cooperative launch was refused (the CTAs cannot all be resident)");
+        return TDQ_ERR_UNSUPPORTED;
+    }
+    TDQ_CHECK_CUDA(cudaGetLastError());
+    return TDQ_OK;
+}
+
+}
diff --git a/torchdiffeq_b200/csrc/tdq_ctrl.cu b/torchdiffeq_b200/csrc/tdq_ctrl.cu
--- a/torchdiffeq_b200/csrc/tdq_ctrl.cu
+++ b/torchdiffeq_b200/csrc/tdq_ctrl.cu
@@ -1,231 +1,23 @@
 #include "tdq_common.cuh"
 #include "tdq_shape.cuh"
 #include "tdq_step.cuh"
+#include "tdq_ctrl_step.cuh"
 
 namespace {
-
-template <typename T> __device__ __forceinline__ void store_T(unsigned char *raw, int i, T v) {
-    reinterpret_cast<T *>(raw)[i] = v;
-}
-
-template <typename T> __device__ void prepare_scalar(TdqCtrl &c) {
-    if (c.halt) return;
-    if (c.n_steps_interval >= c.max_num_steps) {
-        c.status = TDQ_RUN_MAX_STEPS;
-        c.halt = 1;
-        return;
-    }
-    double dt = tdq_clamp_dt(c.dt, c.min_step, c.max_step);
-    const double t0 = c.t1;
-    double t1 = t0 + dt;
-    c.att_t0 = t0;
-    c.att_dt = dt;
-    if (!(t0 + dt > t0)) {
-        c.status = TDQ_RUN_DT_UNDERFLOW;
-        c.halt = 1;
-        return;
-    }
-    if (c.y0_bad) {
-        c.status = TDQ_RUN_NONFINITE;
-        c.halt = 1;
-        return;
-    }
-    c.on_step_t = 0;
-    if (c.n_step_t > 0) {
-        const double nxt = c.step_t[c.next_step_index];
-        if (t0 < nxt && nxt < t0 + dt) {
-            c.on_step_t = 1;
-            t1 = nxt;
-            dt = t1 - t0;
-        }
-    }
-    c.on_jump_t = 0;
-    if (c.n_jump_t > 0) {
-        const double nxt = c.jump_t[c.next_jump_index];
-        if (t0 < nxt && nxt < t0 + dt) {
-            c.on_jump_t = 1;
-            c.on_step_t = 0;
-            t1 = nxt;
-            dt = t1 - t0;
-        }
-    }
-    c.att_dt = dt;
-    c.att_t1 = t1;
-    c.att_dtT = (double)(T)dt;
-}
-
-template <typename T> __device__ void prepare_tables(TdqCtrl &c, int tid, int nthreads) {
-    if (c.halt) return;
-    const T t0T = (T)c.att_t0, dtT = (T)c.att_dt, t1T = (T)c.att_t1;
-    const T sgn = (T)c.t_sign;
-    const int S = c.n_stages;
-    for (int i = tid; i < S; i += nthreads)
-        store_T<T>(c.tstage, i, tdq_stage_time<T>((T)c.alpha[i], t0T, dtT, t1T, sgn));
-    const int rows = c.fsal ? S : S + 1;
-    for (int e = tid; e < rows * TDQ_MAX_K; e += nthreads) {
-        const int r = e / TDQ_MAX_K, m = e % TDQ_MAX_K;
-        if (m < c.row_nnz[r]) c.coef[r][m] = (double)tdq_coef<T>(sgn, (T)c.beta[r][m], dtT);
-    }
-    for (int m = tid; m < c.err_nnz; m += nthreads)
-        c.ecoef[m] = (double)tdq_coef<T>(sgn, (T)c.c_err[m], dtT);
-}
 
 template <typename T> __device__ void prepare_attempt(TdqCtrl &c) {
     prepare_scalar<T>(c);
     prepare_tables<T>(c, 0, 1);
 }
 
-template <typename T, int THREADS>
-__device__ double block_norm_from_sums(const TdqCtrl &c, const double *sums, const int64_t *counts, int n_seg,
-                                       double *smem ) {
-    double best = 0.0;
-    int nan = 0;
-    for (int s = threadIdx.x; s < n_seg; s += THREADS) {
-        const double cnt = counts ? (double)counts[s] : (double)c.n_global;
-        if (cnt <= 0.0) continue;
-        const double r = tdq_rms<T>(sums[s], cnt, c.ratio_f64);
-        if (r != r) nan = 1;
-        if (r > best) best = r;
-    }
-#pragma unroll
-    for (int o = 16; o > 0; o >>= 1) {
-        const double ob = __shfl_down_sync(0xffffffffu, best, o);
-        const int on = __shfl_down_sync(0xffffffffu, nan, o);
-        if (ob > best) best = ob;
-        nan |= on;
-    }
-    const int lane = threadIdx.x & 31, w = threadIdx.x >> 5;
-    __syncthreads();
-    if (lane == 0) smem[w] = nan ? CUDART_NAN : best;
-    __syncthreads();
-    if (threadIdx.x == 0) {
-        double b = 0.0;
-        bool bn = false;
-        for (int i = 0; i < THREADS / 32; ++i) {
-            const double v = smem[i];
-            if (v != v) bn = true;
-            else if (v > b) b = v;
-        }
-        smem[THREADS / 32] = bn ? CUDART_NAN : b;
-    }
-    __syncthreads();
-    return smem[THREADS / 32];
-}
-
-static __device__ void write_mailbox(TdqCtrl &c, double fin_t0, double fin_dt, int jumped = 0) {
-    c.seq += 1;
-    tdq_mailbox *m = c.mbox;
-    if (!m) return;
-    if (c.loop_handle != 0ull && !c.halt) return;
-    m->status = c.status;
-    m->accept = c.accept;
-    m->done = c.done;
-    m->out_cursor = c.out_cursor;
-    m->n_accept = c.n_accept;
-    m->n_reject = c.n_reject;
-    m->t0 = c.t0;
-    m->t1 = c.t1;
-    m->dt = c.dt;
-    m->ratio = c.ratio;
-    m->att_t0 = fin_t0;
-    m->att_dt = fin_dt;
-    m->next_t0 = c.att_t0;
-    m->next_dt = c.att_dt;
-    m->on_jump_t = jumped;
-    m->par = c.par;
-    __threadfence_system();
-    m->seq = c.seq;
-}
-
-template <typename T>
-__device__ void controller(TdqCtrl &c, const double *norm_in, int n_seg, const void *ratio_dev, double ratio_pre) {
-    if (c.halt) {
-        c.accept = 0;
-        c.fit_now = 0;
-        c.emit_lo = c.emit_hi;
-        write_mailbox(c, c.att_t0, c.att_dt);
-        return;
-    }
-    using A = Ar<T>;
-    double ratio;
-    if (ratio_dev) {
-        ratio = c.ratio_f64 ? *reinterpret_cast<const double *>(ratio_dev)
-                            : (double)*reinterpret_cast<const T *>(ratio_dev);
-        ratio = fabs(ratio);
-    } else {
-        ratio = ratio_pre;
-    }
-    const bool y1_nonfinite = norm_in && norm_in[n_seg] > 0.0;
-    if (y1_nonfinite && !ratio_dev) ratio = CUDART_NAN;
-    c.ratio = ratio;
-
-    const double dt = c.att_dt;
-    const bool accept = tdq_accept(ratio, dt, c.min_step, c.max_step);
-    c.accept = accept ? 1 : 0;
-
-    if (accept) {
-        c.t0 = c.att_t0;
-        c.t1 = c.att_t1;
-        c.n_accept += 1;
-        c.y0_prev = c.y0_cur;
-        c.k0_prev = c.k0_cur;
-        c.par ^= 1;
-        c.y0_cur = c.ybuf[c.par];
-        c.k0_cur = c.kbuf[c.par];
-        if (c.on_step_t && c.next_step_index != c.n_step_t - 1) c.next_step_index += 1;
-        if (c.on_jump_t) {
-            if (c.next_jump_index != c.n_jump_t - 1) c.next_jump_index += 1;
-            store_T<T>(c.taux, 2, A::mul((T)c.t_sign, next_repr<T>((T)c.att_t1)));
-        }
-        const T dtT = (T)c.att_dtT, sgn = (T)c.t_sign;
-        c.fit_sdt = (double)A::mul(sgn, dtT);
-        for (int m = 0; m < c.mid_nnz; ++m)
-            c.fit_mcoef[m] = (double)tdq_coef<T>(sgn, (T)c.c_mid[m], dtT);
-        if (y1_nonfinite) {
-            c.status = TDQ_RUN_NONFINITE;
-            c.halt = 1;
-        }
-    } else {
-        c.t0 = c.att_t0;
-        c.t1 = c.att_t0;
-        c.n_reject += 1;
-    }
-
-    const double dt_next = tdq_next_dt(ratio, dt, c.safety, c.ifactor, c.dfactor, c.order, c.min_step, c.max_step);
-    c.dt = dt_next;
-
-    c.emit_lo = c.out_cursor;
-    c.n_steps_interval += 1;
-    if (accept) {
-        const int cur = tdq_cursor_after(c.t_out, c.n_out, c.out_cursor, c.t1);
-        if (cur != c.out_cursor) c.n_steps_interval = 0;
-        c.out_cursor = cur;
-    }
-    c.emit_hi = c.out_cursor;
-    c.fit_now = (accept && (c.always_fit || c.emit_hi > c.emit_lo)) ? 1 : 0;
-    if (c.out_cursor >= c.n_out) {
-        c.done = 1;
-        c.halt = 1;
-    }
-    const double fin_t0 = c.att_t0, fin_dt = c.att_dt;
-    const int jumped = (accept && c.on_jump_t) ? 1 : 0;
-    prepare_scalar<T>(c);
-    write_mailbox(c, fin_t0, fin_dt, jumped);
-}
-
 constexpr int kCtrlThreads = 256;
-static_assert(sizeof(TdqCtrl) % 8 == 0, "control block must be a whole number of 8-byte words");
 static_assert(sizeof(TdqCtrl) <= 40 * 1024, "control block must fit static shared memory");
 
 template <typename T>
 __global__ void __launch_bounds__(kCtrlThreads)
 k_controller(TdqCtrl *c, const double *norm_in, const int64_t *cnt, int n_seg, const void *ratio_dev) {
     __shared__ __align__(16) unsigned char raw[sizeof(TdqCtrl)];
-    constexpr int kWords = (int)(sizeof(TdqCtrl) / 8);
-    unsigned long long *sw = reinterpret_cast<unsigned long long *>(raw);
-    const unsigned long long *gw = reinterpret_cast<const unsigned long long *>(c);
-    for (int i = threadIdx.x; i < kWords; i += kCtrlThreads) sw[i] = gw[i];
-    __syncthreads();
+    ctrl_stage_in(c, raw);
     TdqCtrl &sc = *reinterpret_cast<TdqCtrl *>(raw);
     __shared__ double xsum[TDQ_MAX_SEGS + 2];
     __shared__ int xfail;
@@ -269,19 +61,9 @@
         norm_in = xsum;
     }
     __shared__ double nsm[kCtrlThreads / 32 + 1];
-    double ratio_pre = 0.0;
-    if (!sc.halt && ratio_dev == nullptr)
-        ratio_pre = block_norm_from_sums<T, kCtrlThreads>(sc, norm_in, cnt, n_seg, nsm);
     __shared__ int was_halted;
-    if (threadIdx.x == 0) {
-        was_halted = sc.halt;
-        controller<T>(sc, norm_in, n_seg, ratio_dev, ratio_pre);
-    }
-    __syncthreads();
-    if (!was_halted) prepare_tables<T>(sc, threadIdx.x, kCtrlThreads);
-    __syncthreads();
-    unsigned long long *go = reinterpret_cast<unsigned long long *>(c);
-    for (int i = threadIdx.x; i < kWords; i += kCtrlThreads) go[i] = sw[i];
+    ctrl_decide<T, kCtrlThreads>(sc, norm_in, cnt, n_seg, ratio_dev, sc.loop_handle != 0ull, nsm, &was_halted, threadIdx.x);
+    ctrl_stage_out(c, raw);
     if (threadIdx.x == 0 && sc.loop_handle != 0ull)
         cudaGraphSetConditional((cudaGraphConditionalHandle)sc.loop_handle, sc.halt ? 0u : 1u);
 }
diff --git a/torchdiffeq_b200/csrc/tdq_ctrl_step.cuh b/torchdiffeq_b200/csrc/tdq_ctrl_step.cuh
--- /dev/null
+++ b/torchdiffeq_b200/csrc/tdq_ctrl_step.cuh
@@ -0,0 +1,245 @@
+#pragma once
+
+#include "tdq_common.cuh"
+#include "tdq_step.cuh"
+
+namespace {
+
+template <typename T> __device__ __forceinline__ void store_T(unsigned char *raw, int i, T v) {
+    reinterpret_cast<T *>(raw)[i] = v;
+}
+
+template <typename T> __device__ __forceinline__ void prepare_scalar(TdqCtrl &c) {
+    if (c.halt) return;
+    if (c.n_steps_interval >= c.max_num_steps) {
+        c.status = TDQ_RUN_MAX_STEPS;
+        c.halt = 1;
+        return;
+    }
+    double dt = tdq_clamp_dt(c.dt, c.min_step, c.max_step);
+    const double t0 = c.t1;
+    double t1 = t0 + dt;
+    c.att_t0 = t0;
+    c.att_dt = dt;
+    if (!(t0 + dt > t0)) {
+        c.status = TDQ_RUN_DT_UNDERFLOW;
+        c.halt = 1;
+        return;
+    }
+    if (c.y0_bad) {
+        c.status = TDQ_RUN_NONFINITE;
+        c.halt = 1;
+        return;
+    }
+    c.on_step_t = 0;
+    if (c.n_step_t > 0) {
+        const double nxt = c.step_t[c.next_step_index];
+        if (t0 < nxt && nxt < t0 + dt) {
+            c.on_step_t = 1;
+            t1 = nxt;
+            dt = t1 - t0;
+        }
+    }
+    c.on_jump_t = 0;
+    if (c.n_jump_t > 0) {
+        const double nxt = c.jump_t[c.next_jump_index];
+        if (t0 < nxt && nxt < t0 + dt) {
+            c.on_jump_t = 1;
+            c.on_step_t = 0;
+            t1 = nxt;
+            dt = t1 - t0;
+        }
+    }
+    c.att_dt = dt;
+    c.att_t1 = t1;
+    c.att_dtT = (double)(T)dt;
+}
+
+template <typename T> __device__ __forceinline__ void prepare_tables(TdqCtrl &c, int tid, int nthreads) {
+    if (c.halt) return;
+    const T t0T = (T)c.att_t0, dtT = (T)c.att_dt, t1T = (T)c.att_t1;
+    const T sgn = (T)c.t_sign;
+    const int S = c.n_stages;
+    for (int i = tid; i < S; i += nthreads)
+        store_T<T>(c.tstage, i, tdq_stage_time<T>((T)c.alpha[i], t0T, dtT, t1T, sgn));
+    const int rows = c.fsal ? S : S + 1;
+    for (int e = tid; e < rows * TDQ_MAX_K; e += nthreads) {
+        const int r = e / TDQ_MAX_K, m = e % TDQ_MAX_K;
+        if (m < c.row_nnz[r]) c.coef[r][m] = (double)tdq_coef<T>(sgn, (T)c.beta[r][m], dtT);
+    }
+    for (int m = tid; m < c.err_nnz; m += nthreads)
+        c.ecoef[m] = (double)tdq_coef<T>(sgn, (T)c.c_err[m], dtT);
+}
+
+template <typename T, int THREADS>
+__device__ __forceinline__ double block_norm_from_sums(const TdqCtrl &c, const double *sums, const int64_t *counts, int n_seg,
+                                       double *smem ) {
+    double best = 0.0;
+    int nan = 0;
+    for (int s = threadIdx.x; s < n_seg; s += THREADS) {
+        const double cnt = counts ? (double)counts[s] : (double)c.n_global;
+        if (cnt <= 0.0) continue;
+        const double r = tdq_rms<T>(sums[s], cnt, c.ratio_f64);
+        if (r != r) nan = 1;
+        if (r > best) best = r;
+    }
+#pragma unroll
+    for (int o = 16; o > 0; o >>= 1) {
+        const double ob = __shfl_down_sync(0xffffffffu, best, o);
+        const int on = __shfl_down_sync(0xffffffffu, nan, o);
+        if (ob > best) best = ob;
+        nan |= on;
+    }
+    const int lane = threadIdx.x & 31, w = threadIdx.x >> 5;
+    __syncthreads();
+    if (lane == 0) smem[w] = nan ? CUDART_NAN : best;
+    __syncthreads();
+    if (threadIdx.x == 0) {
+        double b = 0.0;
+        bool bn = false;
+        for (int i = 0; i < THREADS / 32; ++i) {
+            const double v = smem[i];
+            if (v != v) bn = true;
+            else if (v > b) b = v;
+        }
+        smem[THREADS / 32] = bn ? CUDART_NAN : b;
+    }
+    __syncthreads();
+    return smem[THREADS / 32];
+}
+
+__device__ __forceinline__ void write_mailbox(TdqCtrl &c, bool final_only, double fin_t0, double fin_dt, int jumped = 0) {
+    c.seq += 1;
+    tdq_mailbox *m = c.mbox;
+    if (!m) return;
+    if (final_only && !c.halt) return;
+    m->status = c.status;
+    m->accept = c.accept;
+    m->done = c.done;
+    m->out_cursor = c.out_cursor;
+    m->n_accept = c.n_accept;
+    m->n_reject = c.n_reject;
+    m->t0 = c.t0;
+    m->t1 = c.t1;
+    m->dt = c.dt;
+    m->ratio = c.ratio;
+    m->att_t0 = fin_t0;
+    m->att_dt = fin_dt;
+    m->next_t0 = c.att_t0;
+    m->next_dt = c.att_dt;
+    m->on_jump_t = jumped;
+    m->par = c.par;
+    __threadfence_system();
+    m->seq = c.seq;
+}
+
+template <typename T>
+__device__ __forceinline__ void controller(TdqCtrl &c, const double *norm_in, int n_seg, const void *ratio_dev, double ratio_pre,
+                           bool final_only) {
+    if (c.halt) {
+        c.accept = 0;
+        c.fit_now = 0;
+        c.emit_lo = c.emit_hi;
+        write_mailbox(c, final_only, c.att_t0, c.att_dt);
+        return;
+    }
+    using A = Ar<T>;
+    double ratio;
+    if (ratio_dev) {
+        ratio = c.ratio_f64 ? *reinterpret_cast<const double *>(ratio_dev)
+                            : (double)*reinterpret_cast<const T *>(ratio_dev);
+        ratio = fabs(ratio);
+    } else {
+        ratio = ratio_pre;
+    }
+    const bool y1_nonfinite = norm_in && norm_in[n_seg] > 0.0;
+    if (y1_nonfinite && !ratio_dev) ratio = CUDART_NAN;
+    c.ratio = ratio;
+
+    const double dt = c.att_dt;
+    const bool accept = tdq_accept(ratio, dt, c.min_step, c.max_step);
+    c.accept = accept ? 1 : 0;
+
+    if (accept) {
+        c.t0 = c.att_t0;
+        c.t1 = c.att_t1;
+        c.n_accept += 1;
+        c.y0_prev = c.y0_cur;
+        c.k0_prev = c.k0_cur;
+        c.par ^= 1;
+        c.y0_cur = c.ybuf[c.par];
+        c.k0_cur = c.kbuf[c.par];
+        if (c.on_step_t && c.next_step_index != c.n_step_t - 1) c.next_step_index += 1;
+        if (c.on_jump_t) {
+            if (c.next_jump_index != c.n_jump_t - 1) c.next_jump_index += 1;
+            store_T<T>(c.taux, 2, A::mul((T)c.t_sign, next_repr<T>((T)c.att_t1)));
+        }
+        const T dtT = (T)c.att_dtT, sgn = (T)c.t_sign;
+        c.fit_sdt = (double)A::mul(sgn, dtT);
+        for (int m = 0; m < c.mid_nnz; ++m)
+            c.fit_mcoef[m] = (double)tdq_coef<T>(sgn, (T)c.c_mid[m], dtT);
+        if (y1_nonfinite) {
+            c.status = TDQ_RUN_NONFINITE;
+            c.halt = 1;
+        }
+    } else {
+        c.t0 = c.att_t0;
+        c.t1 = c.att_t0;
+        c.n_reject += 1;
+    }
+
+    const double dt_next = tdq_next_dt(ratio, dt, c.safety, c.ifactor, c.dfactor, c.order, c.min_step, c.max_step);
+    c.dt = dt_next;
+
+    c.emit_lo = c.out_cursor;
+    c.n_steps_interval += 1;
+    if (accept) {
+        const int cur = tdq_cursor_after(c.t_out, c.n_out, c.out_cursor, c.t1);
+        if (cur != c.out_cursor) c.n_steps_interval = 0;
+        c.out_cursor = cur;
+    }
+    c.emit_hi = c.out_cursor;
+    c.fit_now = (accept && (c.always_fit || c.emit_hi > c.emit_lo)) ? 1 : 0;
+    if (c.out_cursor >= c.n_out) {
+        c.done = 1;
+        c.halt = 1;
+    }
+    const double fin_t0 = c.att_t0, fin_dt = c.att_dt;
+    const int jumped = (accept && c.on_jump_t) ? 1 : 0;
+    prepare_scalar<T>(c);
+    write_mailbox(c, final_only, fin_t0, fin_dt, jumped);
+}
+
+static_assert(sizeof(TdqCtrl) % 8 == 0, "control block must be a whole number of 8-byte words");
+
+__device__ __forceinline__ void ctrl_stage_in(const TdqCtrl *c, unsigned char *raw) {
+    constexpr int kWords = (int)(sizeof(TdqCtrl) / 8);
+    unsigned long long *sw = reinterpret_cast<unsigned long long *>(raw);
+    const unsigned long long *gw = reinterpret_cast<const unsigned long long *>(c);
+    for (int i = threadIdx.x; i < kWords; i += blockDim.x) sw[i] = gw[i];
+    __syncthreads();
+}
+
+__device__ __forceinline__ void ctrl_stage_out(TdqCtrl *c, const unsigned char *raw) {
+    constexpr int kWords = (int)(sizeof(TdqCtrl) / 8);
+    const unsigned long long *sw = reinterpret_cast<const unsigned long long *>(raw);
+    unsigned long long *go = reinterpret_cast<unsigned long long *>(c);
+    for (int i = threadIdx.x; i < kWords; i += blockDim.x) go[i] = sw[i];
+}
+
+template <typename T, int THREADS>
+__device__ __forceinline__ void ctrl_decide(TdqCtrl &sc, const double *norm_in, const int64_t *cnt, int n_seg,
+                                            const void *ratio_dev, bool final_only, double *nsm, int *was_halted, int tid) {
+    double ratio_pre = 0.0;
+    if (!sc.halt && ratio_dev == nullptr)
+        ratio_pre = block_norm_from_sums<T, THREADS>(sc, norm_in, cnt, n_seg, nsm);
+    if (threadIdx.x == 0) {
+        *was_halted = sc.halt;
+        controller<T>(sc, norm_in, n_seg, ratio_dev, ratio_pre, final_only);
+    }
+    __syncthreads();
+    if (!*was_halted) prepare_tables<T>(sc, tid, THREADS);
+    __syncthreads();
+}
+
+}
diff --git a/torchdiffeq_b200/csrc/tdq_fit.cuh b/torchdiffeq_b200/csrc/tdq_fit.cuh
--- /dev/null
+++ b/torchdiffeq_b200/csrc/tdq_fit.cuh
@@ -0,0 +1,91 @@
+#pragma once
+
+#include "tdq_common.cuh"
+#include "tdq_step.cuh"
+
+namespace {
+
+constexpr int kFitThreads = 256;
+
+template <typename T, int NK, bool VECTOR, bool STORE>
+__device__ __forceinline__ void fit_eval_body(const TdqCtrl *__restrict__ c, const T *__restrict__ y1p, const T *__restrict__ kSp,
+                                              const KPtrs &kmid, T *__restrict__ ce, T *__restrict__ cd, T *__restrict__ cc,
+                                              T *__restrict__ cb, T *__restrict__ ca, T *__restrict__ solution, size_t n,
+                                              unsigned block, unsigned blocks) {
+    constexpr int kThreads = kFitThreads;
+    using A = Ar<T>;
+    const T *y0p = reinterpret_cast<const T *>(c->y0_prev);
+    const T *k0p = reinterpret_cast<const T *>(c->k0_prev);
+    T mf[NK];
+    const T *km[NK];
+#pragma unroll
+    for (int m = 0; m < NK; ++m) {
+        mf[m] = (T)c->fit_mcoef[m];
+        km[m] = reinterpret_cast<const T *>(kmid.p[m] ? kmid.p[m] : (const void *)k0p);
+    }
+    const T sdt = (T)c->fit_sdt;
+    const T two_sdt = A::mul((T)2, sdt);
+    const int lo = c->emit_lo, hi = c->emit_hi;
+    const double t0 = c->t0, t1 = c->t1;
+
+    auto fit = [&](T y0v, T y1v, T f0, T f1, const T *kv, T &e, T &d, T &cq, T &b, T &a) {
+        tdq_quartic<T>(y0v, y1v, f0, f1, tdq_combine<T, NK>(y0v, kv, mf), sdt, two_sdt, e, d, cq, b, a);
+    };
+    auto xof = [&](int j) -> T { return (T)((c->t_out[j] - t0) / (t1 - t0)); };
+
+    if (VECTOR) {
+        using V = Vec<T>;
+        const size_t nvec = n / V::N;
+        for (size_t v = (size_t)block * kThreads + threadIdx.x; v < nvec; v += (size_t)blocks * kThreads) {
+            const size_t i0 = v * V::N;
+            V a0 = ld_stream<T>(y0p + i0), a1 = ld_stream<T>(y1p + i0);
+            V f0 = ld_stream<T>(k0p + i0), f1 = ld_stream<T>(kSp + i0);
+            V kv[NK];
+#pragma unroll
+            for (int m = 0; m < NK; ++m) kv[m] = ld_stream<T>(km[m] + i0);
+            V re, rd, rc, rb, ra;
+#pragma unroll
+            for (int e = 0; e < V::N; ++e) {
+                T ke[NK];
+#pragma unroll
+                for (int m = 0; m < NK; ++m) ke[m] = kv[m].v[e];
+                fit(a0.v[e], a1.v[e], f0.v[e], f1.v[e], ke, re.v[e], rd.v[e], rc.v[e], rb.v[e], ra.v[e]);
+            }
+            if (STORE) {
+                st_vec<T>(ce + i0, re); st_vec<T>(cd + i0, rd); st_vec<T>(cc + i0, rc);
+                st_vec<T>(cb + i0, rb); st_vec<T>(ca + i0, ra);
+            }
+            for (int j = lo; j < hi; ++j) {
+                const T x = xof(j);
+                V r;
+#pragma unroll
+                for (int l = 0; l < V::N; ++l) r.v[l] = tdq_eval_poly<T>(re.v[l], rd.v[l], rc.v[l], rb.v[l], ra.v[l], x);
+                st_vec<T>(solution + (size_t)j * n + i0, r);
+            }
+        }
+        if (block == blocks - 1) {
+            const size_t i = nvec * V::N + threadIdx.x;
+            if (i < n) {
+                T ke[NK];
+#pragma unroll
+                for (int m = 0; m < NK; ++m) ke[m] = km[m][i];
+                T e, d, cq, b, a;
+                fit(y0p[i], y1p[i], k0p[i], kSp[i], ke, e, d, cq, b, a);
+                if (STORE) { ce[i] = e; cd[i] = d; cc[i] = cq; cb[i] = b; ca[i] = a; }
+                for (int j = lo; j < hi; ++j) solution[(size_t)j * n + i] = tdq_eval_poly<T>(e, d, cq, b, a, xof(j));
+            }
+        }
+    } else {
+        for (size_t i = (size_t)block * kThreads + threadIdx.x; i < n; i += (size_t)blocks * kThreads) {
+            T ke[NK];
+#pragma unroll
+            for (int m = 0; m < NK; ++m) ke[m] = km[m][i];
+            T e, d, cq, b, a;
+            fit(y0p[i], y1p[i], k0p[i], kSp[i], ke, e, d, cq, b, a);
+            if (STORE) { ce[i] = e; cd[i] = d; cc[i] = cq; cb[i] = b; ca[i] = a; }
+            for (int j = lo; j < hi; ++j) solution[(size_t)j * n + i] = tdq_eval_poly<T>(e, d, cq, b, a, xof(j));
+        }
+    }
+}
+
+}
diff --git a/torchdiffeq_b200/csrc/tdq_interp.cu b/torchdiffeq_b200/csrc/tdq_interp.cu
--- a/torchdiffeq_b200/csrc/tdq_interp.cu
+++ b/torchdiffeq_b200/csrc/tdq_interp.cu
@@ -1,10 +1,11 @@
 #include "tdq_common.cuh"
 #include "tdq_shape.cuh"
 #include "tdq_step.cuh"
+#include "tdq_fit.cuh"
 
 namespace {
 
-constexpr int kThreads = 256;
+constexpr int kThreads = kFitThreads;
 
 template <typename T, int NK, bool VECTOR, bool STORE>
 __global__ void __launch_bounds__(kThreads)
@@ -12,79 +13,7 @@
            T *__restrict__ ce, T *__restrict__ cd, T *__restrict__ cc, T *__restrict__ cb, T *__restrict__ ca,
            T *__restrict__ solution, size_t n) {
     if (!c->fit_now) return;
-    using A = Ar<T>;
-    const T *y0p = reinterpret_cast<const T *>(c->y0_prev);
-    const T *k0p = reinterpret_cast<const T *>(c->k0_prev);
-    T mf[NK];
-    const T *km[NK];
-#pragma unroll
-    for (int m = 0; m < NK; ++m) {
-        mf[m] = (T)c->fit_mcoef[m];
-        km[m] = reinterpret_cast<const T *>(kmid.p[m] ? kmid.p[m] : (const void *)k0p);
-    }
-    const T sdt = (T)c->fit_sdt;
-    const T two_sdt = A::mul((T)2, sdt);
-    const int lo = c->emit_lo, hi = c->emit_hi;
-    const double t0 = c->t0, t1 = c->t1;
-
-    auto fit = [&](T y0v, T y1v, T f0, T f1, const T *kv, T &e, T &d, T &cq, T &b, T &a) {
-        tdq_quartic<T>(y0v, y1v, f0, f1, tdq_combine<T, NK>(y0v, kv, mf), sdt, two_sdt, e, d, cq, b, a);
-    };
-    auto xof = [&](int j) -> T { return (T)((c->t_out[j] - t0) / (t1 - t0)); };
-
-    if (VECTOR) {
-        using V = Vec<T>;
-        const size_t nvec = n / V::N;
-        for (size_t v = (size_t)blockIdx.x * kThreads + threadIdx.x; v < nvec; v += (size_t)gridDim.x * kThreads) {
-            const size_t i0 = v * V::N;
-            V a0 = ld_stream<T>(y0p + i0), a1 = ld_stream<T>(y1p + i0);
-            V f0 = ld_stream<T>(k0p + i0), f1 = ld_stream<T>(kSp + i0);
-            V kv[NK];
-#pragma unroll
-            for (int m = 0; m < NK; ++m) kv[m] = ld_stream<T>(km[m] + i0);
-            V re, rd, rc, rb, ra;
-#pragma unroll
-            for (int e = 0; e < V::N; ++e) {
-                T ke[NK];
-#pragma unroll
-                for (int m = 0; m < NK; ++m) ke[m] = kv[m].v[e];
-                fit(a0.v[e], a1.v[e], f0.v[e], f1.v[e], ke, re.v[e], rd.v[e], rc.v[e], rb.v[e], ra.v[e]);
-            }
-            if (STORE) {
-                st_vec<T>(ce + i0, re); st_vec<T>(cd + i0, rd); st_vec<T>(cc + i0, rc);
-                st_vec<T>(cb + i0, rb); st_vec<T>(ca + i0, ra);
-            }
-            for (int j = lo; j < hi; ++j) {
-                const T x = xof(j);
-                V r;
-#pragma unroll
-                for (int l = 0; l < V::N; ++l) r.v[l] = tdq_eval_poly<T>(re.v[l], rd.v[l], rc.v[l], rb.v[l], ra.v[l], x);
-                st_vec<T>(solution + (size_t)j * n + i0, r);
-            }
-        }
-        if (blockIdx.x == gridDim.x - 1) {
-            const size_t i = nvec * V::N + threadIdx.x;
-            if (i < n) {
-                T ke[NK];
-#pragma unroll
-                for (int m = 0; m < NK; ++m) ke[m] = km[m][i];
-                T e, d, cq, b, a;
-                fit(y0p[i], y1p[i], k0p[i], kSp[i], ke, e, d, cq, b, a);
-                if (STORE) { ce[i] = e; cd[i] = d; cc[i] = cq; cb[i] = b; ca[i] = a; }
-                for (int j = lo; j < hi; ++j) solution[(size_t)j * n + i] = tdq_eval_poly<T>(e, d, cq, b, a, xof(j));
-            }
-        }
-    } else {
-        for (size_t i = (size_t)blockIdx.x * kThreads + threadIdx.x; i < n; i += (size_t)gridDim.x * kThreads) {
-            T ke[NK];
-#pragma unroll
-            for (int m = 0; m < NK; ++m) ke[m] = km[m][i];
-            T e, d, cq, b, a;
-            fit(y0p[i], y1p[i], k0p[i], kSp[i], ke, e, d, cq, b, a);
-            if (STORE) { ce[i] = e; cd[i] = d; cc[i] = cq; cb[i] = b; ca[i] = a; }
-            for (int j = lo; j < hi; ++j) solution[(size_t)j * n + i] = tdq_eval_poly<T>(e, d, cq, b, a, xof(j));
-        }
-    }
+    fit_eval_body<T, NK, VECTOR, STORE>(c, y1p, kSp, kmid, ce, cd, cc, cb, ca, solution, n, blockIdx.x, gridDim.x);
 }
 
 template <typename T, int NK>
```

After: 3.953 million, median of 6. +15.4%, better.
